# congliuUvA/Clifford-Group-Equivariant-Simplicial-Message-Passing-Networks

Hardware: AMD Instinct MI355X
Metric: simplicial edges/sec (fwd+bwd) on Cl(3,0) 8-ch multivectors; % HBM roofline (higher is better)
Workload: dtype f32; 1 GPU; S1: EGCL layer fwd+bwd, Cl(1, 1, 1), 8 channels, 10000 nodes, 100000 edges/GPU x 1 GPU, aggr=mean, edge_attr 6ch, node_attr 3ch; aggregation=float atomics, launch=hip-graph replay

## Files before the change

### clifford-group-equivariant-simplicial-message-passing-networks_amd/csmpn_hip/native.py

```python
from __future__ import annotations

import ctypes as C
import os

_HERE = os.path.dirname(os.path.abspath(__file__))
LIB_PATH = os.environ.get("CSMPN_LIB") or os.path.join(_HERE, "libcsmpn_hip.so")

ABI_VERSION = 2
MAX_BLOCKS = 4
FLAG_WEIGHTS_PACKED = 1
FLAG_NO_VALIDATE = 2
FLAG_DETERMINISTIC = 4
FLAG_SAVE_STATE = 8
ERR_UNSUPPORTED, ERR_INVALID, ERR_HIP = 1, 2, 3
LAYER_MVSILU, LAYER_MVNORM, LAYER_MVLAYERNORM, LAYER_WGP = 0, 1, 2, 3

EXPORTS = (
    "csmpn_metric_supported",
    "csmpn_algebra_tables",
    "csmpn_geometric_product_forward",
    "csmpn_geometric_product_backward",
    "csmpn_cemlp_workspace_bytes",
    "csmpn_cemlp_saved_floats_per_row",
    "csmpn_cemlp_saved_floats",
    "csmpn_cemlp_forward",
    "csmpn_cemlp_backward",
    "csmpn_mvlinear_forward",
    "csmpn_mvlinear_backward",
    "csmpn_mvlinear_backward_det_bytes",
    "csmpn_mvlinear_backward_det",
    "csmpn_mvsilu_forward",
    "csmpn_mvsilu_backward",
    "csmpn_mvnorm_forward",
    "csmpn_mvnorm_backward",
    "csmpn_mvlayernorm_forward",
    "csmpn_mvlayernorm_backward",
    "csmpn_wgp_forward",
    "csmpn_wgp_backward",
    "csmpn_small_layer_det_bytes",
    "csmpn_mvsilu_backward_det",
    "csmpn_mvnorm_backward_det",
    "csmpn_mvlayernorm_forward_det",
    "csmpn_mvlayernorm_backward_det",
    "csmpn_wgp_backward_det",
    "csmpn_csr_workspace_bytes",
    "csmpn_csr_build",
    "csmpn_csr_source_order",
    "csmpn_segment_reduce",
    "csmpn_egcl_edge_forward",
    "csmpn_egcl_edge_backward",
    "csmpn_egcl_node_forward",
    "csmpn_egcl_node_backward",
    "csmpn_egcl_backward",
    "csmpn_simplex_rows",
    "csmpn_simplex_tables_workspace_bytes",
    "csmpn_simplex_tables",
    "csmpn_rips_lift_workspace_bytes",
    "csmpn_rips_lift",
    "csmpn_knn_lift_workspace_bytes",
    "csmpn_knn_lift",
    "csmpn_embed_cemlp_forward",
    "csmpn_embed_cemlp_backward",
    "csmpn_type_attr_forward",
    "csmpn_type_attr_backward",
    "csmpn_type_attr_backward_det_bytes",
    "csmpn_type_attr_backward_det",
    "csmpn_readout_mse_forward",
    "csmpn_readout_mse_backward",
    "csmpn_readout_traj_forward",
    "csmpn_readout_traj_backward",
    "csmpn_last_error",
    "csmpn_last_kernel",
    "csmpn_abi_version",
    "csmpn_build_target",
)

PARAM_FIELDS = ("lin_w", "lin_b", "silu_a", "silu_b", "gp_w", "norm_a", "right_w", "left_w", "left_b", "ln_a")


class BlockParams(C.Structure):
    _fields_ = [
        ("in_features", C.c_int32),
        ("out_features", C.c_int32),
        ("lin_subspaces", C.c_int32),
        ("reserved", C.c_int32),
    ] + [(name, C.c_void_p) for name in PARAM_FIELDS]


class BlockGrads(C.Structure):
    _fields_ = [(name, C.c_void_p) for name in PARAM_FIELDS]


class VertexBlock(C.Structure):
    _fields_ = [("data", C.c_void_p), ("channels", C.c_int32), ("grade", C.c_int32)]


class NativeLibraryMissing(RuntimeError):
    pass


def _load():
    if not os.path.exists(LIB_PATH):
        raise NativeLibraryMissing(
            f"{LIB_PATH} not found. This package has no CPU/eager fallback: build the HIP "
            f"library first (python -c 'import __graft_entry__ as g; g.build()' or "
            f"make -C {os.path.join(os.path.dirname(_HERE), 'csrc')})."
        )
    lib = C.CDLL(LIB_PATH)
    lib.csmpn_abi_version.restype = C.c_int
    if lib.csmpn_abi_version() != ABI_VERSION:
        raise NativeLibraryMissing(f"{LIB_PATH} has ABI version {lib.csmpn_abi_version()}, this package binds version "
                                   f"{ABI_VERSION}: rebuild it (make -C {os.path.join(os.path.dirname(_HERE), 'csrc')})")
    vp, i32, i64, sz, u32 = C.c_void_p, C.c_int32, C.c_int64, C.c_size_t, C.c_uint32
    fp = C.POINTER(C.c_float)
    bp, bg = C.POINTER(BlockParams), C.POINTER(BlockGrads)

    def sig(name, res, args):
        fn = getattr(lib, name)
        fn.restype = res
        fn.argtypes = args

    sig("csmpn_metric_supported", C.c_int, [fp, C.c_int])
    sig("csmpn_algebra_tables", C.c_int, [fp, C.c_int, vp, vp, vp, vp, vp, vp])
    sig("csmpn_geometric_product_forward", C.c_int, [fp, C.c_int, vp, vp, vp, i64, vp])
    sig("csmpn_geometric_product_backward", C.c_int, [fp, C.c_int, vp, vp, vp, vp, vp, i64, vp])
    sig("csmpn_cemlp_workspace_bytes", sz, [C.c_int, bp, C.c_int])
    sig("csmpn_cemlp_saved_floats_per_row", sz, [C.c_int, bp, C.c_int])
    sig("csmpn_cemlp_saved_floats", sz, [C.c_int, bp, C.c_int, i64, u32])
    sig("csmpn_cemlp_forward", C.c_int, [fp, C.c_int, bp, C.c_int, vp, i64, vp, vp, vp, sz, u32, vp])
    sig("csmpn_cemlp_backward", C.c_int, [fp, C.c_int, bp, bg, C.c_int, vp, vp, i64, vp, vp, vp, sz, u32, vp])
    sig("csmpn_mvlinear_forward", C.c_int, [C.c_int, vp, vp, vp, i64, i32, i32, i32, vp, vp])
    sig("csmpn_mvlinear_backward", C.c_int, [C.c_int, vp, vp, vp, i64, i32, i32, i32, vp, vp, vp, vp])
    sig("csmpn_mvlinear_backward_det_bytes", sz, [C.c_int, i64, i32, i32, i32])
    sig("csmpn_mvlinear_backward_det", C.c_int, [C.c_int, vp, vp, vp, i64, i32, i32, i32, vp, vp, vp, vp, sz, vp])
    sig("csmpn_mvsilu_forward", C.c_int, [fp, C.c_int, vp, vp, vp, i64, i32, vp, vp])
    sig("csmpn_mvsilu_backward", C.c_int, [fp, C.c_int, vp, vp, vp, vp, i64, i32, vp, vp, vp, vp])
    sig("csmpn_mvnorm_forward", C.c_int, [fp, C.c_int, vp, vp, i64, i32, vp, vp])
    sig("csmpn_mvnorm_backward", C.c_int, [fp, C.c_int, vp, vp, vp, i64, i32, vp, vp, vp])
    sig("csmpn_mvlayernorm_forward", C.c_int, [fp, C.c_int, vp, vp, i64, i32, vp, vp])
    sig("csmpn_mvlayernorm_backward", C.c_int, [fp, C.c_int, vp, vp, vp, i64, i32, vp, vp, vp])
    sig("csmpn_wgp_forward", C.c_int, [fp, C.c_int, vp, vp, vp, i64, i32, vp, vp])
    sig("csmpn_wgp_backward", C.c_int, [fp, C.c_int, vp, vp, vp, vp, i64, i32, vp, vp, vp, vp])
    sig("csmpn_small_layer_det_bytes", sz, [C.c_int, C.c_int, i64, i32])
    sig("csmpn_mvsilu_backward_det", C.c_int, [fp, C.c_int, vp, vp, vp, vp, i64, i32, vp, vp, vp, vp, sz, vp])
    sig("csmpn_mvnorm_backward_det", C.c_int, [fp, C.c_int, vp, vp, vp, i64, i32, vp, vp, vp, sz, vp])
    sig("csmpn_mvlayernorm_forward_det", C.c_int, [fp, C.c_int, vp, vp, i64, i32, vp, vp])
    sig("csmpn_mvlayernorm_backward_det", C.c_int, [fp, C.c_int, vp, vp, vp, i64, i32, vp, vp, vp, sz, vp])
    sig("csmpn_wgp_backward_det", C.c_int, [fp, C.c_int, vp, vp, vp, vp, i64, i32, vp, vp, vp, vp, sz, vp])
    sig("csmpn_csr_workspace_bytes", sz, [i64, i64])
    sig("csmpn_csr_build", C.c_int, [vp, i64, i64, vp, vp, vp, vp, vp, vp, sz, u32, vp])
    sig("csmpn_csr_source_order", C.c_int, [vp, i64, i64, vp, vp, vp, sz, vp])
    sig("csmpn_segment_reduce", C.c_int, [vp, i64, i64, vp, vp, vp, vp, vp, i32, vp])
    sig("csmpn_egcl_edge_forward", C.c_int,
        [fp, C.c_int, bp, C.c_int, vp, i32, vp, i32, vp, vp, vp, i64, i64, vp, vp, vp, sz, u32, vp])
    sig("csmpn_egcl_edge_backward", C.c_int,
        [fp, C.c_int, bp, bg, C.c_int, vp, i32, vp, i32, vp, vp, vp, i64, i64, vp, vp, vp, vp, vp, sz, u32, vp])
    sig("csmpn_egcl_node_forward", C.c_int,
        [fp, C.c_int, bp, C.c_int, vp, i32, vp, i32, vp, i32, vp, i32, i32, i64, vp, vp, vp, sz, u32, vp])
    sig("csmpn_egcl_node_backward", C.c_int,
        [fp, C.c_int, bp, bg, C.c_int, vp, i32, vp, i32, vp, i32, vp, i32, i32, i64, vp, vp, vp, vp, vp, vp, sz, u32, vp])
    sig("csmpn_egcl_backward", C.c_int,
        [fp, C.c_int, bp, bg, C.c_int, bp, bg, C.c_int, vp, i32, vp, i32, vp, i32, vp, i32, vp, vp, vp, vp, i32, i32, i64, i64,
         vp, vp, vp, vp, vp, vp, vp, vp, sz, u32, vp, vp, sz, u32, vp])
    sig("csmpn_simplex_rows", C.c_int, [C.c_int, C.POINTER(VertexBlock), C.c_int, vp, i64, i32, i64, vp, vp])
    sig("csmpn_simplex_tables_workspace_bytes", sz, [i64, i32])
    sig("csmpn_simplex_tables", C.c_int, [vp, i32, vp, vp, vp, i64, i64, i32, vp, vp, vp, vp, vp, vp, vp, vp, vp, sz, vp])
    sig("csmpn_rips_lift_workspace_bytes", sz, [i64, i32, i32])
    sig("csmpn_rips_lift", C.c_int, [vp, i32, i64, i32, C.c_double, i32, vp, i64, vp, i32, vp, vp, vp, vp, vp, vp, vp, vp, vp, vp, sz, vp])
    sig("csmpn_knn_lift_workspace_bytes", sz, [i64, i32, i32])
    sig("csmpn_knn_lift", C.c_int, [vp, i32, i64, i32, i32, i32, vp, i64, vp, i32, vp, vp, vp, vp, vp, vp, vp, vp, vp, vp, sz, vp])
    sig("csmpn_embed_cemlp_forward", C.c_int, [fp, C.c_int, bp, C.c_int, vp, i64, i32, vp, i32, i32, i64, vp, vp, vp, sz, u32, vp])
    sig("csmpn_embed_cemlp_backward", C.c_int, [fp, C.c_int, bp, bg, C.c_int, vp, i64, i32, vp, i32, i32, i64, vp, vp, vp, sz, u32, vp])
    sig("csmpn_type_attr_forward", C.c_int, [C.c_int, vp, i32, i32, vp, i64, vp, vp, i64, vp, vp, vp])
    sig("csmpn_type_attr_backward", C.c_int, [C.c_int, i32, i32, vp, i64, vp, vp, i64, vp, vp, vp, vp])
    sig("csmpn_type_attr_backward_det_bytes", sz, [i32, i32, i64, i64])
    sig("csmpn_type_attr_backward_det", C.c_int, [C.c_int, i32, i32, vp, i64, vp, vp, i64, vp, vp, vp, vp, sz, vp])
    sig("csmpn_readout_mse_forward", C.c_int, [C.c_int, vp, vp, i32, vp, i64, i32, vp, i64, vp, vp, vp, vp, vp])
    sig("csmpn_readout_mse_backward", C.c_int, [C.c_int, vp, i32, i64, i32, vp, i64, vp, vp, vp])
    sig("csmpn_readout_traj_forward", C.c_int, [C.c_int, vp, i32, vp, i64, vp, i32, i32, vp, vp, vp, vp, i64, vp, vp, vp, vp])
    sig("csmpn_readout_traj_backward", C.c_int,
        [C.c_int, vp, i32, i64, vp, vp, i64, vp, i32, i32, vp, vp, vp, vp, vp, vp, vp, vp, vp, vp, vp])
    sig("csmpn_last_error", C.c_char_p, [])
    sig("csmpn_last_kernel", C.c_char_p, [])
    sig("csmpn_abi_version", C.c_int, [])
    sig("csmpn_build_target", C.c_char_p, [])
    return lib


_lib = None


def lib():
    global _lib
    if _lib is None:
        _lib = _load()
    return _lib


class CsmpnError(RuntimeError):
    pass


def check(rc: int):
    if rc != 0:
        raise CsmpnError(f"csmpn_hip error {rc}: {lib().csmpn_last_error().decode()}")


def metric_array(metric):
    arr = (C.c_float * len(metric))(*[float(m) for m in metric])
    return arr
```

### clifford-group-equivariant-simplicial-message-passing-networks_amd/csmpn_hip/ops.py

```python
from __future__ import annotations

import ctypes as C
import os
import warnings
from typing import List, Optional, Sequence

import torch

from . import native
from .native import BlockGrads, BlockParams, PARAM_FIELDS, check

NP = len(PARAM_FIELDS)


def _stream(device) -> int:
    return torch.cuda.current_stream(device).cuda_stream


def _on_device_of(arg_index):
    import functools

    def deco(fn):
        @functools.wraps(fn)
        def wrapped(*args, **kwargs):
# ... 292 lines not shown
def _det_call(call, flags):
    det = deterministic_request()
    rc = call(flags | (native.FLAG_DETERMINISTIC if det else 0))
    if det == "soft" and _soft_fallback(rc):
        rc = call(flags)
    check(rc)


_DET_LAUNCHES = 0


def det_launches() -> int:
    return _DET_LAUNCHES


def _count_det():
    global _DET_LAUNCHES
    _DET_LAUNCHES += 1


def _det_scratch(nbytes, device):
    _count_det()
    return torch.empty(max(int(nbytes), 16), dtype=torch.uint8, device=device)


def _small_det_scratch(op, metric, x):
    return _det_scratch(native.lib().csmpn_small_layer_det_bytes(op, len(metric), x.shape[0], x.shape[1]), x.device)


def _warn_soft_slice():
    global _warned_soft_det
    if not _warned_soft_det:
        _warned_soft_det = True
        warnings.warn("csmpn_hip: torch.use_deterministic_algorithms(True) is set, but this launch covers a slice of "
                      "the adjacency (graph-segment step): using float atomics (ops.set_deterministic(True) makes "
                      "this an error)")


def segment_reduce(rows, out, add=None, sub=None, accumulate=True):
    ap, ao = add if add is not None else (None, None)
    sp, so = sub if sub is not None else (None, None)
    check(native.lib().csmpn_segment_reduce(rows.data_ptr(), rows[0].numel(), out.shape[0], _ptr(ap), _ptr(ao),
                                            _ptr(sp), _ptr(so), out.data_ptr(), 1 if accumulate else 0,
                                            _stream(out.device)))
    return out


class Csr:

    __slots__ = ("perm", "src", "dst", "deg", "row_ptr", "n_edges", "n_nodes", "build_ms", "_src_order", "_ws")

    def source_order(self):
        if self._src_order is None:
            dev = self.src.device
            order = torch.empty(max(self.n_edges, 1), dtype=torch.int32, device=dev)
            rp = torch.empty(self.n_nodes + 1, dtype=torch.int32, device=dev)
            ws = torch.empty(int(native.lib().csmpn_csr_workspace_bytes(self.n_edges, self.n_nodes)),
                             dtype=torch.uint8, device=dev)
            with torch.cuda.device(dev):
                check(native.lib().csmpn_csr_source_order(self.src.data_ptr(), self.n_edges, self.n_nodes,
                                                          order.data_ptr(), rp.data_ptr(), ws.data_ptr(), ws.numel(),
                                                          _stream(dev)))
            self._src_order = (rp, order)
        return self._src_order

    def __init__(self, edge_index: torch.Tensor, n_nodes: int):
        if not edge_index.is_cuda:
            raise RuntimeError("edge_index must live on the GPU (no CPU fallback)")
        if edge_index.dtype != torch.int64 or edge_index.dim() != 2 or edge_index.shape[0] != 2:
            raise RuntimeError("edge_index must be int64 [2, E]")
        ei = edge_index.contiguous()
        dev = ei.device
        E = ei.shape[1]
        i32 = dict(dtype=torch.int32, device=dev)
        self.n_edges, self.n_nodes = E, n_nodes
        self._src_order = None
        self._ws = None
        self.perm = torch.empty(max(E, 1), **i32)
        self.src = torch.empty(max(E, 1), **i32)
        self.dst = torch.empty(max(E, 1), **i32)
        self.deg = torch.empty(n_nodes, **i32)
        self.row_ptr = torch.empty(n_nodes + 1, **i32)
        ws = torch.empty(int(native.lib().csmpn_csr_workspace_bytes(E, n_nodes)), dtype=torch.uint8, device=dev)
        with torch.cuda.device(dev):
            t0, t1 = torch.cuda.Event(enable_timing=True), torch.cuda.Event(enable_timing=True)
            t0.record()
            check(native.lib().csmpn_csr_build(ei.data_ptr(), E, n_nodes, self.perm.data_ptr(), self.src.data_ptr(),
                                               self.dst.data_ptr(), self.deg.data_ptr(), self.row_ptr.data_ptr(),
                                               ws.data_ptr(), ws.numel(), 0, _stream(dev)))
            t1.record()
            t1.synchronize()
            self.build_ms = t0.elapsed_time(t1)


    def rebuild_(self, edge_index: torch.Tensor) -> "Csr":
        if not edge_index.is_cuda or edge_index.device != self.src.device:
            raise RuntimeError("edge_index must live on the device of the CSR (no CPU fallback)")
        if edge_index.dtype != torch.int64 or tuple(edge_index.shape) != (2, self.n_edges) or not edge_index.is_contiguous():
            raise RuntimeError(f"Csr.rebuild_: edge_index must be contiguous int64 [2, {self.n_edges}] (the size it was built for)")
        dev = self.src.device
        lib = native.lib()
        if self._ws is None:
            self._ws = torch.empty(int(lib.csmpn_csr_workspace_bytes(self.n_edges, self.n_nodes)), dtype=torch.uint8, device=dev)
        ws = self._ws
        with torch.cuda.device(dev):
            check(lib.csmpn_csr_build(edge_index.data_ptr(), self.n_edges, self.n_nodes, self.perm.data_ptr(),
                                      self.src.data_ptr(), self.dst.data_ptr(), self.deg.data_ptr(), self.row_ptr.data_ptr(),
                                      ws.data_ptr(), ws.numel(), native.FLAG_NO_VALIDATE, _stream(dev)))
            if self._src_order is not None:
                rp, order = self._src_order
                check(lib.csmpn_csr_source_order(self.src.data_ptr(), self.n_edges, self.n_nodes, order.data_ptr(),
                                                 rp.data_ptr(), ws.data_ptr(), ws.numel(), _stream(dev)))
        try:
            edge_index._csmpn_csr = (edge_index._version, self)
        except Exception:
            pass
        return self


class CsrSlice:

    __slots__ = ("perm", "src", "dst", "n_edges", "n_nodes")

    def __init__(self, csr: Csr, lo: int, hi: int):
        self.perm, self.src, self.dst = csr.perm[lo:hi], csr.src[lo:hi], csr.dst[lo:hi]
        self.n_edges, self.n_nodes = hi - lo, csr.n_nodes


def get_csr(edge_index: torch.Tensor, n_nodes: int) -> Csr:
    cached = getattr(edge_index, "_csmpn_csr", None)
    if cached is not None and cached[0] == edge_index._version and cached[1].n_nodes == n_nodes:
        return cached[1]
    csr = Csr(edge_index, n_nodes)
    try:
        edge_index._csmpn_csr = (edge_index._version, csr)
    except Exception:
        pass
    return csr




class EgclSpec:

    def __init__(self, edge: CemlpBinding, node: CemlpBinding, channels: int, out_channels: int,
                 edge_attr_channels: int, node_attr_channels: int, aggr: str, residual: bool):
        if aggr not in ("mean", "sum", "add"):
            raise native.CsmpnError(f"aggr={aggr!r} not supported by the HIP path (mean | sum | add)")
        self.edge, self.node = edge, node
        self.C, self.O = channels, out_channels
        self.A, self.T = edge_attr_channels, node_attr_channels
        self.mean = 1 if aggr == "mean" else 0
        self.residual = 1 if residual else 0


class HipBackend:

    @staticmethod
    def build_csr(edge_index, n_nodes):
        return get_csr(edge_index, n_nodes)

    @staticmethod
    @_on_device_of(2)
    def edge_forward(spec, csr, h, edge_attr, pe, save=True, agg=None, saved=None):
        e = spec.edge
        e.bind(pe)
        N, D = h.shape[0], e.D
        if agg is None:
            agg = torch.zeros(N, spec.O, D, dtype=torch.float32, device=h.device)
        ws = e.workspace(h.device)
        st_flag = 0
        if saved is None and save:
            saved = e.new_saved(csr.n_edges, h.device, _SAVE_STATE)
            if _SAVE_STATE and saved is not None:
                st_flag = native.FLAG_SAVE_STATE
                saved.csmpn_save_state = True
        det = deterministic_request()
        if det and not isinstance(csr, Csr):
            if det == "hard":
                raise native.CsmpnError("deterministic aggregation needs the whole adjacency (no sliced launches: "
                                        "set CSMPN_SPLIT_FWD=0)")
            _warn_soft_slice()
            det = None
        if det:
            rows = torch.empty(max(csr.n_edges, 1), spec.O, D, dtype=torch.float32, device=h.device)
            rc = native.lib().csmpn_egcl_edge_forward(
                e.metric_arr, e.n, e.params, e.nblk, h.data_ptr(), spec.C, _ptr(edge_attr), spec.A,
                csr.perm.data_ptr(), csr.src.data_ptr(), csr.dst.data_ptr(), csr.n_edges, N, rows.data_ptr(),
                _ptr(saved), ws.data_ptr(), ws.numel(), native.FLAG_DETERMINISTIC | st_flag, _stream(h.device))
            if not (det == "soft" and _soft_fallback(rc)):
                check(rc)
                segment_reduce(rows, agg, add=(csr.row_ptr, None))
                return agg, (ws, saved)
        check(native.lib().csmpn_egcl_edge_forward(
            e.metric_arr, e.n, e.params, e.nblk, h.data_ptr(), spec.C, _ptr(edge_attr), spec.A,
            csr.perm.data_ptr(), csr.src.data_ptr(), csr.dst.data_ptr(), csr.n_edges, N, agg.data_ptr(),
            _ptr(saved), ws.data_ptr(), ws.numel(), st_flag, _stream(h.device)))
        return agg, (ws, saved)

    @staticmethod
    @_on_device_of(2)
    def node_forward(spec, deg, h, agg, node_attr, pn, save=True):
        nd = spec.node
        nd.bind(pn)
        N, D = h.shape[0], nd.D
        out = torch.empty(N, nd.out_features, D, dtype=torch.float32, device=h.device)
        ws = nd.workspace(h.device)
        saved = nd.new_saved(N, h.device, _SAVE_STATE) if save else None
        st_flag = 0
        if _SAVE_STATE and saved is not None:
            st_flag = native.FLAG_SAVE_STATE
            saved.csmpn_save_state = True

        def call(flags):
            return native.lib().csmpn_egcl_node_forward(
                nd.metric_arr, nd.n, nd.params, nd.nblk, h.data_ptr(), spec.C, agg.data_ptr(), spec.O,
                _ptr(node_attr), spec.T, deg.data_ptr(), spec.mean, spec.residual, N, out.data_ptr(),
                _ptr(saved), ws.data_ptr(), ws.numel(), flags, _stream(h.device))

        det = deterministic_request()
        rc = call((native.FLAG_DETERMINISTIC if det else 0) | st_flag)
        if det == "soft" and _soft_fallback(rc):
            rc = call(st_flag)
        check(rc)
        return out, (ws, saved)

    @staticmethod
    @_on_device_of(2)
    def node_backward(spec, deg, h, agg, node_attr, pn, gout, want_gna, state=None, gflat=None, fused_into=None):
        nd = spec.node
        nd.bind(pn)
        N, D, dev = h.shape[0], nd.D, h.device
        _flat, views = nd.new_grads(pn, dev, gflat, fused_into=fused_into)
        gh = torch.empty_like(h)
        g_agg = torch.empty(N, spec.O, D, dtype=torch.float32, device=dev)
        g_na = torch.empty_like(node_attr) if (node_attr is not None and want_gna) else None
        ws, saved = state if state is not None else (nd.workspace(dev), None)
        flags = native.FLAG_WEIGHTS_PACKED if state is not None else 0
        if getattr(saved, "csmpn_save_state", False):
            flags |= native.FLAG_SAVE_STATE

        def call(fl):
            return native.lib().csmpn_egcl_node_backward(
                nd.metric_arr, nd.n, nd.params, nd.grads, nd.nblk, h.data_ptr(), spec.C, agg.data_ptr(), spec.O,
                _ptr(node_attr), spec.T, deg.data_ptr(), spec.mean, spec.residual, N, gout.data_ptr(),
                gh.data_ptr(), g_agg.data_ptr(), _ptr(g_na), _ptr(saved), ws.data_ptr(), ws.numel(), fl, _stream(dev))

        det = deterministic_request()
        rc = call(flags | (native.FLAG_DETERMINISTIC if det else 0))
        if det == "soft" and _soft_fallback(rc):
            rc = call(flags)
        check(rc)
        return gh, g_agg, g_na, views

    @staticmethod
    @_on_device_of(2)
    def edge_backward(spec, csr, h, edge_attr, pe, g_agg, gh, want_gea, state=None, gflat=None, fused_into=None):
        e = spec.edge
        e.bind(pe)
        N, dev = h.shape[0], h.device
        _flat, views = e.new_grads(pe, dev, gflat, fused_into=fused_into)
        g_ea = torch.empty_like(edge_attr) if (edge_attr is not None and want_gea) else None
        ws, saved = state if state is not None else (e.workspace(dev), None)
        flags = native.FLAG_WEIGHTS_PACKED if state is not None else 0
        if getattr(saved, "csmpn_save_state", False):
            flags |= native.FLAG_SAVE_STATE
        det = deterministic_request()
        if det and not isinstance(csr, Csr):
            if det == "hard":
                raise native.CsmpnError("deterministic aggregation needs the whole adjacency (no sliced launches)")
            _warn_soft_slice()
            det = None
        if det:
            rows = torch.empty(max(csr.n_edges, 1), spec.C, e.D, dtype=torch.float32, device=dev)
            rc = native.lib().csmpn_egcl_edge_backward(
                e.metric_arr, e.n, e.params, e.grads, e.nblk, h.data_ptr(), spec.C, _ptr(edge_attr), spec.A,
                csr.perm.data_ptr(), csr.src.data_ptr(), csr.dst.data_ptr(), csr.n_edges, N, g_agg.data_ptr(),
                rows.data_ptr(), _ptr(g_ea), _ptr(saved), ws.data_ptr(), ws.numel(),
                flags | native.FLAG_DETERMINISTIC, _stream(dev))
            if not (det == "soft" and _soft_fallback(rc)):
                check(rc)
                segment_reduce(rows, gh, add=(csr.row_ptr, None), sub=csr.source_order())
                return g_ea, views
        check(native.lib().csmpn_egcl_edge_backward(
            e.metric_arr, e.n, e.params, e.grads, e.nblk, h.data_ptr(), spec.C, _ptr(edge_attr), spec.A,
            csr.perm.data_ptr(), csr.src.data_ptr(), csr.dst.data_ptr(), csr.n_edges, N, g_agg.data_ptr(),
            gh.data_ptr(), _ptr(g_ea), _ptr(saved), ws.data_ptr(), ws.numel(), flags, _stream(dev)))
        return g_ea, views

    @staticmethod
    @_on_device_of(2)
    def layer_backward(spec, csr, h, agg, edge_attr, node_attr, pe, pn, gout, want_gea, want_gna, state_e=None, state_n=None,
                       gflat_e=None, gflat_n=None, fused_e=None, fused_n=None):
        e, nd = spec.edge, spec.node
        e.bind(pe)
        nd.bind(pn)
        N, D, dev = h.shape[0], nd.D, h.device
        _fe, views_e = e.new_grads(pe, dev, gflat_e, fused_into=fused_e)
        _fn, views_n = nd.new_grads(pn, dev, gflat_n, fused_into=fused_n)
        gh = torch.empty_like(h)
        g_agg = torch.empty(N, spec.O, D, dtype=torch.float32, device=dev)
        g_na = torch.empty_like(node_attr) if (node_attr is not None and want_gna) else None
        g_ea = torch.empty_like(edge_attr) if (edge_attr is not None and want_gea) else None

        def stage(binding, state):
            ws, saved = state if state is not None else (binding.workspace(dev), None)
            flags = native.FLAG_WEIGHTS_PACKED if state is not None else 0
            if getattr(saved, "csmpn_save_state", False):
                flags |= native.FLAG_SAVE_STATE
            return ws, saved, flags

        ws_e, saved_e, fl_e = stage(e, state_e)
        ws_n, saved_n, fl_n = stage(nd, state_n)
        check(native.lib().csmpn_egcl_backward(
            e.metric_arr, e.n, e.params, e.grads, e.nblk, nd.params, nd.grads, nd.nblk, h.data_ptr(), spec.C,
            agg.data_ptr(), spec.O, _ptr(edge_attr), spec.A, _ptr(node_attr), spec.T, csr.perm.data_ptr(),
            csr.src.data_ptr(), csr.dst.data_ptr(), csr.deg.data_ptr(), spec.mean, spec.residual, csr.n_edges, N,
            gout.data_ptr(), gh.data_ptr(), g_agg.data_ptr(), _ptr(g_ea), _ptr(g_na), None, _ptr(saved_e),
            ws_e.data_ptr(), ws_e.numel(), fl_e, _ptr(saved_n), ws_n.data_ptr(), ws_n.numel(), fl_n, _stream(dev)))
        return gh, g_ea, g_na, views_e, views_n


_SAVE_STATE = os.environ.get("CSMPN_SAVE_STATE", "1") not in ("0", "")


def _check_egcl_inputs(spec, csr, h, edge_attr, node_attr, n_edges):
    D = spec.edge.D
    if h.dim() != 3 or h.shape[1] != spec.C or h.shape[2] != D:
        raise RuntimeError(f"h must be [N, {spec.C}, {D}], got {tuple(h.shape)}")
    if (edge_attr is None) != (spec.A == 0) or (node_attr is None) != (spec.T == 0):
        raise RuntimeError("edge_attr/node_attr presence does not match edge_attr_features/node_attr_features")
    if edge_attr is not None and tuple(edge_attr.shape) != (n_edges, spec.A, D):
        raise RuntimeError(f"edge_attr must be [{n_edges}, {spec.A}, {D}], got {tuple(edge_attr.shape)}")
    if node_attr is not None and tuple(node_attr.shape) != (h.shape[0], spec.T, D):
        raise RuntimeError(f"node_attr must be [{h.shape[0]}, {spec.T}, {D}], got {tuple(node_attr.shape)}")


class _EgclFn(torch.autograd.Function):
    @staticmethod
    def forward(ctx, h, edge_attr, node_attr, spec: EgclSpec, csr: Csr, *params):
        _require_device(h, "EGCL input h")
        _check_egcl_inputs(spec, csr, h, edge_attr, node_attr, csr.n_edges)
        h = h.contiguous()
        if edge_attr is not None:
            _require_device(edge_attr, "edge_attr")
            edge_attr = edge_attr.contiguous()
        if node_attr is not None:
            _require_device(node_attr, "node_attr")
            node_attr = node_attr.contiguous()
        ne = spec.edge.nblk * NP
        pe, pn = params[:ne], params[ne:]
        spec.edge.bind(pe); spec.node.bind(pn)
        n_agg = h.shape[0] * spec.O * spec.edge.D
        ctx.param_refs = params
        fuse = _fusable(params, h.device)
        n_ge, n_gn = (spec.edge.grad_floats(pe), spec.node.grad_floats(pn)) if (any(ctx.needs_input_grad) and not fuse) else (0, 0)
        zeros = torch.zeros(n_agg + n_ge + n_gn, dtype=torch.float32, device=h.device)
        agg = zeros[:n_agg].view(h.shape[0], spec.O, spec.edge.D)
        ctx.gflats = (zeros[n_agg:n_agg + n_ge], zeros[n_agg + n_ge:]) if n_ge else None
        agg, st_e = HipBackend.edge_forward(spec, csr, h, edge_attr, pe, agg=agg)
        out, st_n = HipBackend.node_forward(spec, csr.deg, h, agg, node_attr, pn)
        ctx.spec, ctx.csr, ctx.st_e, ctx.st_n = spec, csr, st_e, st_n
        ctx.has_ea, ctx.has_na = edge_attr is not None, node_attr is not None
        ctx.mask = [p is not None for p in params]
        saved = [h, agg]
        if ctx.has_ea:
            saved.append(edge_attr)
        if ctx.has_na:
            saved.append(node_attr)
        ctx.save_for_backward(*saved, *[p for p in params if p is not None])
        return out

    @staticmethod
    def backward(ctx, gout):
        spec, csr = ctx.spec, ctx.csr
        saved = list(ctx.saved_tensors)
        h, agg = saved[0], saved[1]
        pos = 2
        edge_attr = node_attr = None
        if ctx.has_ea:
            edge_attr = saved[pos]; pos += 1
        if ctx.has_na:
            node_attr = saved[pos]; pos += 1
        it = iter(saved[pos:])
        params = [next(it) if m else None for m in ctx.mask]
        ne = spec.edge.nblk * NP
        pe, pn = params[:ne], params[ne:]
        gout = gout.contiguous()
        gfe, gfn = ctx.gflats if ctx.gflats is not None else (None, None)
        ctx.gflats = None
        refs = ctx.param_refs
        fuse = _fusable(refs, h.device)
        if isinstance(csr, Csr) and not deterministic_request():
            gh, g_ea, g_na, views_e, views_n = HipBackend.layer_backward(
                spec, csr, h, agg, edge_attr, node_attr, pe, pn, gout, ctx.needs_input_grad[1], ctx.needs_input_grad[2],
                ctx.st_e, ctx.st_n, gfe, gfn, refs[:ne] if fuse else None, refs[ne:] if fuse else None)
            return (gh, g_ea, g_na, None, None, *views_e, *views_n)
        gh, g_agg, g_na, views_n = HipBackend.node_backward(spec, csr.deg, h, agg, node_attr, pn, gout,
                                                            ctx.needs_input_grad[2], ctx.st_n, gfn,
                                                            fused_into=refs[ne:] if fuse else None)
        g_ea, views_e = HipBackend.edge_backward(spec, csr, h, edge_attr, pe, g_agg, gh, ctx.needs_input_grad[1],
                                                 ctx.st_e, gfe, fused_into=refs[:ne] if fuse else None)
        return (gh, g_ea, g_na, None, None, *views_e, *views_n)


def egcl_apply(h, edge_attr, node_attr, spec: EgclSpec, csr: Csr, params):
    return _EgclFn.apply(h, edge_attr, node_attr, spec, csr, *params)




class _GpFn(torch.autograd.Function):
    @staticmethod
    @_on_device_of(1)
    def forward(ctx, a, b, metric):
        _require_device(a, "geometric_product operand")
        _require_device(b, "geometric_product operand")
        shape = torch.broadcast_shapes(a.shape, b.shape)
        a2 = a.expand(shape).contiguous()
        b2 = b.expand(shape).contiguous()
        n = len(metric)
        D = 1 << n
        rows = a2.numel() // D
        out = torch.empty_like(a2)
        check(native.lib().csmpn_geometric_product_forward(native.metric_array(metric), n, a2.data_ptr(),
                                                           b2.data_ptr(), out.data_ptr(), rows, _stream(a.device)))
        ctx.save_for_backward(a2, b2)
        ctx.metric, ctx.shapes = metric, (a.shape, b.shape)
        return out

    @staticmethod
    @_on_device_of(1)
    def backward(ctx, gout):
        a2, b2 = ctx.saved_tensors
        metric = ctx.metric
        n = len(metric)
        D = 1 << n
        gout = gout.contiguous()
        ga, gb = torch.zeros_like(a2), torch.zeros_like(b2)
        check(native.lib().csmpn_geometric_product_backward(native.metric_array(metric), n, a2.data_ptr(),
                                                            b2.data_ptr(), gout.data_ptr(), ga.data_ptr(),
                                                            gb.data_ptr(), a2.numel() // D, _stream(a2.device)))
        sa, sb = ctx.shapes
        return ga.sum_to_size(sa), gb.sum_to_size(sb), None




class _MVLinearFn(torch.autograd.Function):

    @staticmethod
    @_on_device_of(1)
    def forward(ctx, x, weight, bias, n):
        _require_device(x, "MVLinear input")
        for name, t in (("weight", weight), ("bias", bias)):
            if t is not None and (t.device != x.device or t.dtype != torch.float32):
                raise RuntimeError(f"MVLinear {name} must be float32 on {x.device}, got {t.dtype} on {t.device}")
        x = x.contiguous()
        w = weight.contiguous()
        b = bias.contiguous() if bias is not None else None
        rows, I, D = x.shape
        O = w.shape[0]
        if D != (1 << n) or w.shape[1] != I:
            raise RuntimeError(f"MVLinear: input {tuple(x.shape)} does not match weight {tuple(w.shape)} (n={n})")
        y = torch.empty(rows, O, D, dtype=torch.float32, device=x.device)
        check(native.lib().csmpn_mvlinear_forward(n, x.data_ptr(), w.data_ptr(), _ptr(b), rows, I, O,
                                                  1 if w.dim() == 3 else 0, y.data_ptr(), _stream(x.device)))
        ctx.save_for_backward(x, w)
        ctx.n, ctx.has_bias = n, bias is not None
        ctx.param_refs = (weight if weight.is_contiguous() else None, bias if (bias is None or bias.is_contiguous()) else False)
        return y

    @staticmethod
    @_on_device_of(1)
    def backward(ctx, gy):
        x, w = ctx.saved_tensors
        gy = gy.contiguous()
        rows, I, D = x.shape
        O = w.shape[0]
        gx = torch.empty_like(x) if ctx.needs_input_grad[0] else None
        need_w, need_b = ctx.needs_input_grad[1], ctx.has_bias and ctx.needs_input_grad[2]
        pw, pb = ctx.param_refs
        sub = 1 if w.dim() == 3 else 0

        def run(gw_ptr, gb_ptr):
            if deterministic_request() and (gw_ptr is not None or gb_ptr is not None):
                ws = _det_scratch(native.lib().csmpn_mvlinear_backward_det_bytes(ctx.n, rows, I, O, sub), x.device)
                check(native.lib().csmpn_mvlinear_backward_det(ctx.n, x.data_ptr(), w.data_ptr(), gy.data_ptr(), rows, I, O, sub,
                                                               _ptr(gx), gw_ptr, gb_ptr, ws.data_ptr(), ws.numel(),
                                                               _stream(x.device)))
            else:
                check(native.lib().csmpn_mvlinear_backward(ctx.n, x.data_ptr(), w.data_ptr(), gy.data_ptr(), rows, I, O, sub,
                                                           _ptr(gx), gw_ptr, gb_ptr, _stream(x.device)))

        if (pw is not None and pb is not False and (need_w or need_b)
                and _fusable([pw if need_w else None, pb if need_b else None], x.device)
                and (not need_b or pb.grad.numel() == O)):
            run(pw.grad.data_ptr() if need_w else None, pb.grad.data_ptr() if need_b else None)
            return gx, None, None, None
        gw = torch.zeros_like(w) if need_w else None
        gb = torch.zeros(1, O, 1, dtype=torch.float32, device=x.device) if need_b else None
        run(_ptr(gw), _ptr(gb))
        return gx, gw, gb, None



_SMALL_LAUNCHES = 0


def small_layer_launches() -> int:
    return _SMALL_LAUNCHES


def _small_args(x, what, params):
    _require_device(x, f"{what} input")
    if x.dim() != 3:
        raise RuntimeError(f"{what}: the HIP path takes [rows, channels, D] inputs, got {tuple(x.shape)}")
    for t in params:
        if t.device != x.device or t.dtype != torch.float32:
            raise RuntimeError(f"{what} parameters must be float32 on {x.device}, got {t.dtype} on {t.device}")
    return x.contiguous()


def _count():
    global _SMALL_LAUNCHES
    _SMALL_LAUNCHES += 1


class _MVSiLUFn(torch.autograd.Function):

    @staticmethod
    @_on_device_of(1)
    def forward(ctx, x, a, b, metric):
        x = _small_args(x, "MVSiLU", (a, b))
        a2, b2 = a.contiguous(), b.contiguous()
        y = torch.empty_like(x)
        check(native.lib().csmpn_mvsilu_forward(native.metric_array(metric), len(metric), x.data_ptr(), a2.data_ptr(),
                                                b2.data_ptr(), x.shape[0], x.shape[1], y.data_ptr(), _stream(x.device)))
        _count()
        ctx.save_for_backward(x, a2, b2)
        ctx.metric = metric
        return y

    @staticmethod
    @_on_device_of(1)
    def backward(ctx, gy):
        x, a, b = ctx.saved_tensors
        gy = gy.contiguous()
        gx, ga, gb = torch.empty_like(x), torch.zeros_like(a), torch.zeros_like(b)
# ... 472 lines not shown
```

### clifford-group-equivariant-simplicial-message-passing-networks_amd/csrc/capi.hip

```cpp
#include <mutex>
#include <hip/hip_runtime.h>

#include <cstdarg>
#include <cstdio>
#include <cstdlib>
#include <cstring>
#include <vector>

#include "plan.hpp"

using namespace csmpn;

thread_local char g_csmpn_err[512] = "";

int csmpn_fail(int code, const char* fmt, ...) {
    va_list ap;
    va_start(ap, fmt);
    vsnprintf(g_csmpn_err, sizeof(g_csmpn_err), fmt, ap);
    va_end(ap);
    return code;
}


namespace csmpn {
// ... 102 lines not shown

size_t csmpn_cemlp_saved_floats(int n, const csmpn_block_params* blocks, int n_blocks, int64_t rows, uint32_t flags) {
    if (rows <= 0 || !blocks || n_blocks < 1 || n_blocks > CSMPN_MAX_BLOCKS || n < 1 || n > 8) return 0;
    return saved_layout(n, blocks, n_blocks, rows, flags).total;
}

size_t csmpn_cemlp_saved_floats_per_row(int n, const csmpn_block_params* blocks, int n_blocks) {
    if (!blocks || n_blocks < 1 || n_blocks > CSMPN_MAX_BLOCKS || n < 1 || n > 8) return 0;
    return saved_layout(n, blocks, n_blocks, -1, CSMPN_FLAG_SAVE_STATE).total;
}

size_t csmpn_cemlp_workspace_bytes(int n, const csmpn_block_params* blocks, int n_blocks) {
    if (!blocks || n_blocks < 1 || n_blocks > CSMPN_MAX_BLOCKS || n < 1 || n > 8) return 0;
    const size_t tail = family_tail_bytes(n, blocks, n_blocks), det = det_slice_bytes(n, blocks, n_blocks);
    return plan_front_bytes(n, blocks, n_blocks) + (tail > det ? tail : det) + kTailSlack;
}

int csmpn_cemlp_forward(const float* metric, int n, const csmpn_block_params* blocks, int n_blocks, const float* x,
                        int64_t rows, float* y, float* save_inputs, void* workspace, size_t workspace_bytes, uint32_t flags, void* stream) {
    const AlgId id = alg_id(metric, n);
    if (id == ALG_NONE) return fail(CSMPN_ERR_UNSUPPORTED, "metric not supported by the HIP path");
    Plan plan;
    int rc = make_plan(id, blocks, nullptr, n_blocks, workspace, workspace_bytes, false, 0, false, rows, plan,
                       (flags & CSMPN_FLAG_DETERMINISTIC) != 0);
    if (rc) return rc;
    const bool need_pack = !(flags & CSMPN_FLAG_WEIGHTS_PACKED);
    RowIO io;
    memset(&io, 0, sizeof(io));
    io.rows = rows; io.nseg = 1;
    io.seg[0].a = x; io.seg[0].ch = blocks[0].in_features; io.seg[0].off = 0;
    io.y = y; io.save = save_inputs;
    io.save_state = ((flags & CSMPN_FLAG_SAVE_STATE) && pq_plain_shape(n, blocks, n_blocks)) ? 1 : 0;
    return run_rows(plan, MODE_PLAIN, false, io, (hipStream_t)stream, need_pack);
}

int csmpn_cemlp_backward(const float* metric, int n, const csmpn_block_params* blocks, const csmpn_block_grads* grads,
                         int n_blocks, const float* x, const float* gy, int64_t rows, float* gx, const float* saved_inputs, void* workspace,
                         size_t workspace_bytes, uint32_t flags, void* stream) {
    const AlgId id = alg_id(metric, n);
    if (id == ALG_NONE) return fail(CSMPN_ERR_UNSUPPORTED, "metric not supported by the HIP path");
    Plan plan;
    int rc = make_plan(id, blocks, grads, n_blocks, workspace, workspace_bytes, true, 0, saved_inputs != nullptr, rows, plan,
                       (flags & CSMPN_FLAG_DETERMINISTIC) != 0);
    if (rc) return rc;
    const bool need_pack = true;
    RowIO io;
    memset(&io, 0, sizeof(io));
    io.rows = rows; io.nseg = 1;
    io.seg[0].a = x; io.seg[0].ch = blocks[0].in_features; io.seg[0].off = 0;
    io.gy = gy; io.gx[0] = gx; io.saved = saved_inputs;
    io.row_store = (flags & CSMPN_FLAG_DETERMINISTIC) ? 1 : 0;
    io.save_state = ((flags & CSMPN_FLAG_SAVE_STATE) && pq_plain_shape(n, blocks, n_blocks)) ? 1 : 0;
    const bool tables_ready = io.save_state && (flags & CSMPN_FLAG_WEIGHTS_PACKED) != 0;
    return run_rows(plan, MODE_PLAIN, true, io, (hipStream_t)stream, need_pack, tables_ready);
}

__global__ void index_range_kernel(const int* __restrict__ idx, long n, int hi, int* __restrict__ flag) {
    const long i = (long)blockIdx.x * blockDim.x + threadIdx.x;
    if (i < n && (idx[i] < 0 || idx[i] >= hi)) atomicOr(flag, 1);
}
__device__ int g_range_flag;
static std::mutex g_range_mutex;

static int check_index_range(const int32_t* idx, int64_t n, int64_t hi, hipStream_t st, const char* what) {
    if (n <= 0) return CSMPN_OK;
    std::lock_guard<std::mutex> lock(g_range_mutex);
    int* flag = nullptr;
    hipError_t e = hipGetSymbolAddress(reinterpret_cast<void**>(&flag), HIP_SYMBOL(g_range_flag));
    if (e == hipSuccess) e = hipMemsetAsync(flag, 0, sizeof(int), st);
    if (e != hipSuccess) return fail(CSMPN_ERR_HIP, "%s validation: %s", what, hipGetErrorString(e));
    hipLaunchKernelGGL(index_range_kernel, dim3((unsigned)((n + 255) / 256)), dim3(256), 0, st, idx, (long)n,
                       (int)(hi > 0x7fffffff ? 0x7fffffff : hi), flag);
    int host_flag = 0;
    e = hipMemcpyAsync(&host_flag, flag, sizeof(int), hipMemcpyDeviceToHost, st);
    if (e == hipSuccess) e = hipStreamSynchronize(st);
    if (e != hipSuccess) return fail(CSMPN_ERR_HIP, "%s validation: %s", what, hipGetErrorString(e));
    if (host_flag) return fail(CSMPN_ERR_INVALID, "%s has entries outside [0, %lld)", what, (long long)hi);
    return CSMPN_OK;
}

static int embed_io(const AlgId id, const csmpn_block_params* blocks, const float* vertex_feat, int64_t n_vertex_rows, int32_t kpv,
                    const int32_t* verts, int32_t nv, int32_t n_orders, int64_t n_rows, uint32_t flags, hipStream_t st, RowIO& io) {
    if (id != ALG_N5 && id != ALG_N5M) return fail(CSMPN_ERR_UNSUPPORTED, "fused embedding: Cl(5,0) / Cl(4,1) only");
    if (n_orders != 1 && n_orders != 2 && n_orders != 6) return fail(CSMPN_ERR_UNSUPPORTED, "fused embedding: 1, 2 or 6 vertex orders");
    if (!vertex_feat || !verts || kpv < 1 || nv < 1 || nv * kpv != blocks[0].in_features || nv * kpv > 8)
        return fail(CSMPN_ERR_UNSUPPORTED, "fused embedding: verts_per_row * channels_per_vertex must equal in_features (<= 8)");
    if (n_rows % n_orders) return fail(CSMPN_ERR_INVALID, "fused embedding: n_rows %ld is not a multiple of n_orders %d", (long)n_rows, n_orders);
    if (n_vertex_rows < 1 || n_vertex_rows > 0x7fffffff)
        return fail(CSMPN_ERR_INVALID, "fused embedding: n_vertex_rows %lld not in [1, 2^31)", (long long)n_vertex_rows);
    if (!(flags & CSMPN_FLAG_NO_VALIDATE)) {
        const int rc = check_index_range(verts, n_rows * nv, n_vertex_rows, st, "fused embedding: verts");
        if (rc) return rc;
    }
    memset(&io, 0, sizeof(io));
    io.rows = n_rows; io.nseg = 1;
    io.seg[0].a = vertex_feat; io.seg[0].ch = blocks[0].in_features; io.seg[0].off = 0;
    io.emb_verts = verts; io.emb_nperm = n_orders; io.emb_nv = nv; io.emb_k = kpv; io.emb_nrows = (int)n_vertex_rows;
    return CSMPN_OK;
}

int csmpn_embed_cemlp_forward(const float* metric, int n, const csmpn_block_params* blocks, int n_blocks, const float* vertex_feat,
                              int64_t n_vertex_rows, int32_t channels_per_vertex, const int32_t* verts, int32_t verts_per_row, int32_t n_orders,
                              int64_t n_rows, float* out, float* save_inputs, void* workspace, size_t workspace_bytes,
                              uint32_t flags, void* stream) {
    const AlgId id = alg_id(metric, n);
    if (id == ALG_NONE) return fail(CSMPN_ERR_UNSUPPORTED, "metric not supported by the HIP path");
    RowIO io;
    int rc = embed_io(id, blocks, vertex_feat, n_vertex_rows, channels_per_vertex, verts, verts_per_row, n_orders, n_rows, flags,
                      (hipStream_t)stream, io);
    if (rc) return rc;
    Plan plan;
    if ((rc = make_plan(id, blocks, nullptr, n_blocks, workspace, workspace_bytes, false, 0, false, n_rows, plan))) return rc;
    io.y = out; io.save = save_inputs;
    if (!plw_serves(plan, MODE_PLAIN, false, io))
        return fail(CSMPN_ERR_UNSUPPORTED, "fused embedding: shape not served by the wide parity-lane kernels");
    io.save_state = (flags & CSMPN_FLAG_SAVE_STATE) ? 1 : 0;
    return run_rows(plan, MODE_PLAIN, false, io, (hipStream_t)stream, false);
}

int csmpn_embed_cemlp_backward(const float* metric, int n, const csmpn_block_params* blocks, const csmpn_block_grads* grads,
                               int n_blocks, const float* vertex_feat, int64_t n_vertex_rows, int32_t channels_per_vertex,
                               const int32_t* verts, int32_t verts_per_row, int32_t n_orders, int64_t n_rows, const float* g_out,
                               const float* saved_inputs, void* workspace, size_t workspace_bytes, uint32_t flags, void* stream) {
    const AlgId id = alg_id(metric, n);
    if (id == ALG_NONE) return fail(CSMPN_ERR_UNSUPPORTED, "metric not supported by the HIP path");
    RowIO io;
    int rc = embed_io(id, blocks, vertex_feat, n_vertex_rows, channels_per_vertex, verts, verts_per_row, n_orders, n_rows, flags,
                      (hipStream_t)stream, io);
    if (rc) return rc;
    Plan plan;
    if ((rc = make_plan(id, blocks, grads, n_blocks, workspace, workspace_bytes, true, 0, saved_inputs != nullptr, n_rows, plan))) return rc;
    io.gy = g_out; io.saved = saved_inputs;
    if (!plw_serves(plan, MODE_PLAIN, true, io))
        return fail(CSMPN_ERR_UNSUPPORTED, "fused embedding: shape not served by the wide parity-lane kernels (two blocks need saved inputs)");
    io.save_state = (flags & CSMPN_FLAG_SAVE_STATE) ? 1 : 0;
    return run_rows(plan, MODE_PLAIN, true, io, (hipStream_t)stream, false);
}

static int edge_io(const csmpn_block_params* blocks, const float* h, int channels, const float* edge_attr, int attr_channels,
                   const int32_t* perm, const int32_t* src_sorted, const int32_t* dst_sorted, int64_t E, uint32_t flags, RowIO& io) {
    if (attr_channels > 0 && !edge_attr && E > 0) return fail(CSMPN_ERR_INVALID, "edge_attr is null");
    if (channels + attr_channels != blocks[0].in_features)
        return fail(CSMPN_ERR_INVALID, "edge model in_features %d != %d + %d", blocks[0].in_features, channels, attr_channels);
    memset(&io, 0, sizeof(io));
    io.rows = E; io.nseg = attr_channels > 0 ? 2 : 1;
    io.seg[0].a = h; io.seg[0].ia = dst_sorted; io.seg[0].b = h; io.seg[0].ib = src_sorted; io.seg[0].ch = channels;
    io.seg[1].a = edge_attr; io.seg[1].ia = perm; io.seg[1].ch = attr_channels; io.seg[1].off = channels;
    io.dst = dst_sorted; io.src = src_sorted; io.perm = perm;
    io.row_store = (flags & CSMPN_FLAG_DETERMINISTIC) ? 1 : 0;
    io.save_state = (flags & CSMPN_FLAG_SAVE_STATE) ? 1 : 0;
    return CSMPN_OK;
}

int csmpn_egcl_edge_forward(const float* metric, int n, const csmpn_block_params* blocks, int n_blocks, const float* h,
                            int32_t channels, const float* edge_attr, int32_t attr_channels, const int32_t* perm,
                            const int32_t* src_sorted, const int32_t* dst_sorted, int64_t E, int64_t N, float* agg,
                            float* save_inputs, void* workspace, size_t workspace_bytes, uint32_t flags, void* stream) {
    const AlgId id = alg_id(metric, n);
    if (id == ALG_NONE) return fail(CSMPN_ERR_UNSUPPORTED, "metric not supported by the HIP path");
    RowIO io;
    int rc = edge_io(blocks, h, channels, edge_attr, attr_channels, perm, src_sorted, dst_sorted, E, flags, io);
    if (rc) return rc;
    Plan plan;
    if ((rc = make_plan(id, blocks, nullptr, n_blocks, workspace, workspace_bytes, false, blocks[n_blocks - 1].out_features << n, false,
                        E, plan, (flags & CSMPN_FLAG_DETERMINISTIC) != 0))) return rc;
    const bool need_pack = !(flags & CSMPN_FLAG_WEIGHTS_PACKED);
    io.agg = agg; io.save = save_inputs;
    io.gather_rows = N;
    return run_rows(plan, MODE_EDGE, false, io, (hipStream_t)stream, need_pack);
}

static int edge_backward(const float* metric, int n, const csmpn_block_params* blocks,
                         const csmpn_block_grads* grads, int n_blocks, const float* h, int32_t channels,
                         const float* edge_attr, int32_t attr_channels, const int32_t* perm,
                         const int32_t* src_sorted, const int32_t* dst_sorted, int64_t E, int64_t N,
                         const float* g_agg, float* gh, float* g_edge_attr, const float* saved_inputs, void* workspace,
                         size_t workspace_bytes, uint32_t flags, void* stream, SliceSet* deferred) {
    const AlgId id = alg_id(metric, n);
    if (id == ALG_NONE) return fail(CSMPN_ERR_UNSUPPORTED, "metric not supported by the HIP path");
    RowIO io;
    int rc = edge_io(blocks, h, channels, edge_attr, attr_channels, perm, src_sorted, dst_sorted, E, flags, io);
    if (rc) return rc;
    Plan plan;
    if ((rc = make_plan(id, blocks, grads, n_blocks, workspace, workspace_bytes, true, 0, saved_inputs != nullptr, E, plan,
                        (flags & CSMPN_FLAG_DETERMINISTIC) != 0))) return rc;
    const bool need_pack = true;
    io.gy = g_agg; io.gx[0] = gh; io.gx[1] = g_edge_attr; io.saved = saved_inputs;
    io.gather_rows = N;
    return run_rows(plan, MODE_EDGE, true, io, (hipStream_t)stream, need_pack, (flags & CSMPN_FLAG_WEIGHTS_PACKED) != 0, deferred);
}

int csmpn_egcl_edge_backward(const float* metric, int n, const csmpn_block_params* blocks,
                             const csmpn_block_grads* grads, int n_blocks, const float* h, int32_t channels,
                             const float* edge_attr, int32_t attr_channels, const int32_t* perm,
                             const int32_t* src_sorted, const int32_t* dst_sorted, int64_t E, int64_t N,
                             const float* g_agg, float* gh, float* g_edge_attr, const float* saved_inputs, void* workspace,
                             size_t workspace_bytes, uint32_t flags, void* stream) {
    return edge_backward(metric, n, blocks, grads, n_blocks, h, channels, edge_attr, attr_channels, perm, src_sorted, dst_sorted, E, N,
                         g_agg, gh, g_edge_attr, saved_inputs, workspace, workspace_bytes, flags, stream, nullptr);
}

static int node_io(const csmpn_block_params* blocks, int n_blocks, const float* h, int channels, const float* agg,
                   int agg_channels, const float* node_attr, int attr_channels, const int32_t* in_degree,
                   int mean_aggr, int residual, int64_t N, RowIO& io) {
    if (attr_channels > 0 && !node_attr) return fail(CSMPN_ERR_INVALID, "node_attr is null");
    if (channels + agg_channels + attr_channels != blocks[0].in_features)
        return fail(CSMPN_ERR_INVALID, "node model in_features %d != %d + %d + %d", blocks[0].in_features, channels,
                    agg_channels, attr_channels);
    if (residual && blocks[n_blocks - 1].out_features != channels)
        return fail(CSMPN_ERR_INVALID, "residual needs out_features == channels");
    if (mean_aggr && !in_degree) return fail(CSMPN_ERR_INVALID, "in_degree is null");
    memset(&io, 0, sizeof(io));
    io.rows = N; io.nseg = attr_channels > 0 ? 3 : 2;
    io.seg[0].a = h; io.seg[0].ch = channels; io.seg[0].off = 0;
    io.seg[1].a = agg; io.seg[1].ch = agg_channels; io.seg[1].off = channels;
    io.seg[1].deg = mean_aggr ? in_degree : nullptr;
    io.seg[2].a = node_attr; io.seg[2].ch = attr_channels; io.seg[2].off = channels + agg_channels;
    return CSMPN_OK;
}

int csmpn_egcl_node_forward(const float* metric, int n, const csmpn_block_params* blocks, int n_blocks, const float* h,
                            int32_t channels, const float* agg, int32_t agg_channels, const float* node_attr,
                            int32_t attr_channels, const int32_t* in_degree, int32_t mean_aggr, int32_t residual,
                            int64_t N, float* out, float* save_inputs, void* workspace, size_t workspace_bytes, uint32_t flags, void* stream) {
    const AlgId id = alg_id(metric, n);
    if (id == ALG_NONE) return fail(CSMPN_ERR_UNSUPPORTED, "metric not supported by the HIP path");
    RowIO io;
    int rc = node_io(blocks, n_blocks, h, channels, agg, agg_channels, node_attr, attr_channels, in_degree, mean_aggr,
                     residual, N, io);
    if (rc) return rc;
    Plan plan;
    if ((rc = make_plan(id, blocks, nullptr, n_blocks, workspace, workspace_bytes, false, 0, false, N, plan,
                        (flags & CSMPN_FLAG_DETERMINISTIC) != 0))) return rc;
    const bool need_pack = !(flags & CSMPN_FLAG_WEIGHTS_PACKED);
    io.y = out; io.resid = residual ? h : nullptr; io.save = save_inputs;
    io.row_store = (flags & CSMPN_FLAG_DETERMINISTIC) ? 1 : 0;
    io.save_state = (flags & CSMPN_FLAG_SAVE_STATE) ? 1 : 0;
    return run_rows(plan, MODE_NODE, false, io, (hipStream_t)stream, need_pack);
}

static int node_backward(const float* metric, int n, const csmpn_block_params* blocks,
                         const csmpn_block_grads* grads, int n_blocks, const float* h, int32_t channels,
                         const float* agg, int32_t agg_channels, const float* node_attr, int32_t attr_channels,
                         const int32_t* in_degree, int32_t mean_aggr, int32_t residual, int64_t N,
                         const float* g_out, float* gh, float* g_agg, float* g_node_attr, const float* saved_inputs, void* workspace,
                         size_t workspace_bytes, uint32_t flags, void* stream, SliceSet* deferred) {
    const AlgId id = alg_id(metric, n);
    if (id == ALG_NONE) return fail(CSMPN_ERR_UNSUPPORTED, "metric not supported by the HIP path");
    RowIO io;
    int rc = node_io(blocks, n_blocks, h, channels, agg, agg_channels, node_attr, attr_channels, in_degree, mean_aggr,
                     residual, N, io);
    if (rc) return rc;
    Plan plan;
    if ((rc = make_plan(id, blocks, grads, n_blocks, workspace, workspace_bytes, true, 0, saved_inputs != nullptr, N, plan,
                        (flags & CSMPN_FLAG_DETERMINISTIC) != 0))) return rc;
    const bool need_pack = true;
    io.gy = g_out; io.gx[0] = gh; io.gx[1] = g_agg; io.gx[2] = g_node_attr;
    io.resid_bwd = residual ? 1 : 0; io.saved = saved_inputs;
    io.row_store = (flags & CSMPN_FLAG_DETERMINISTIC) ? 1 : 0;
    io.save_state = (flags & CSMPN_FLAG_SAVE_STATE) ? 1 : 0;
    return run_rows(plan, MODE_NODE, true, io, (hipStream_t)stream, need_pack, (flags & CSMPN_FLAG_WEIGHTS_PACKED) != 0, deferred);
}

int csmpn_egcl_node_backward(const float* metric, int n, const csmpn_block_params* blocks,
                             const csmpn_block_grads* grads, int n_blocks, const float* h, int32_t channels,
                             const float* agg, int32_t agg_channels, const float* node_attr, int32_t attr_channels,
                             const int32_t* in_degree, int32_t mean_aggr, int32_t residual, int64_t N,
                             const float* g_out, float* gh, float* g_agg, float* g_node_attr, const float* saved_inputs, void* workspace,
                             size_t workspace_bytes, uint32_t flags, void* stream) {
    return node_backward(metric, n, blocks, grads, n_blocks, h, channels, agg, agg_channels, node_attr, attr_channels, in_degree, mean_aggr,
                         residual, N, g_out, gh, g_agg, g_node_attr, saved_inputs, workspace, workspace_bytes, flags, stream, nullptr);
}

int csmpn_egcl_backward(const float* metric, int n, const csmpn_block_params* edge_blocks, const csmpn_block_grads* edge_grads,
                        int n_edge_blocks, const csmpn_block_params* node_blocks, const csmpn_block_grads* node_grads,
                        int n_node_blocks, const float* h, int32_t channels, const float* agg, int32_t agg_channels,
                        const float* edge_attr, int32_t edge_attr_channels, const float* node_attr, int32_t node_attr_channels,
                        const int32_t* perm, const int32_t* src_sorted, const int32_t* dst_sorted, const int32_t* in_degree,
                        int32_t mean_aggr, int32_t residual, int64_t E, int64_t N, const float* g_out, float* gh, float* g_agg,
                        float* g_edge_attr, float* g_node_attr, float* g_edge_rows, const float* edge_saved, void* edge_workspace,
                        size_t edge_workspace_bytes, uint32_t edge_flags, const float* node_saved, void* node_workspace,
                        size_t node_workspace_bytes, uint32_t node_flags, void* stream) {
    const bool det = ((edge_flags | node_flags) & CSMPN_FLAG_DETERMINISTIC) != 0;
    if ((edge_flags & CSMPN_FLAG_DETERMINISTIC) && !g_edge_rows)
        return fail(CSMPN_ERR_INVALID, "CSMPN_FLAG_DETERMINISTIC: g_edge_rows ([E, C, D], csmpn_egcl_edge_backward's gh) is null");
    const char *we = static_cast<const char*>(edge_workspace), *wn = static_cast<const char*>(node_workspace);
    const bool apart = we && wn && (we + edge_workspace_bytes <= wn || wn + node_workspace_bytes <= we);
    SliceSet node_set, edge_set;
    node_set.unit = edge_set.unit = nullptr;
    const bool defer = !det && apart;
    int rc = node_backward(metric, n, node_blocks, node_grads, n_node_blocks, h, channels, agg, agg_channels, node_attr,
                           node_attr_channels, in_degree, mean_aggr, residual, N, g_out, gh, g_agg, g_node_attr, node_saved,
                           node_workspace, node_workspace_bytes, node_flags, stream, defer ? &node_set : nullptr);
    if (rc) return rc;
    rc = edge_backward(metric, n, edge_blocks, edge_grads, n_edge_blocks, h, channels, edge_attr, edge_attr_channels, perm, src_sorted,
                       dst_sorted, E, N, g_agg, (edge_flags & CSMPN_FLAG_DETERMINISTIC) ? g_edge_rows : gh, g_edge_attr, edge_saved,
                       edge_workspace, edge_workspace_bytes, edge_flags, stream, node_set.unit ? &edge_set : nullptr);
    if (node_set.unit) {
        const SliceSet* const other = (!rc && edge_set.unit == node_set.unit) ? &edge_set : nullptr;
        HIP_TRY(node_set.unit->sum_slices(node_set, other, (hipStream_t)stream));
        if (!rc && edge_set.unit && !other) HIP_TRY(edge_set.unit->sum_slices(edge_set, nullptr, (hipStream_t)stream));
    }
    return rc;
}

}
```

### clifford-group-equivariant-simplicial-message-passing-networks_amd/csrc/cemlp_cl.hpp

```cpp
#pragma once
#include "cemlp_lane.hpp"

namespace csmpn {

constexpr int kClWaves = 4;
constexpr int kClSliceCap = 512;
constexpr int kClParStride = 36;

#define CL_LDS_ORDER() do { asm volatile("" ::: "memory"); __builtin_amdgcn_wave_barrier(); asm volatile("" ::: "memory"); } while (0)

typedef unsigned cl_u4 __attribute__((ext_vector_type(4)));
constexpr unsigned kClNoStore = 0xFF000000u;
constexpr int kClStream = 2;
struct ClBuf {
    __amdgpu_buffer_rsrc_t r;
    CSMPN_DEV ClBuf() : r(__builtin_amdgcn_make_buffer_rsrc(nullptr, 0, 0, 0x00020000)) {}
    CSMPN_DEV ClBuf(const void* base, size_t bytes)
        : r(__builtin_amdgcn_make_buffer_rsrc(const_cast<void*>(base), 0, base ? (int)(unsigned)bytes : 0, 0x00020000)) {}
    template <int AUX = 0>
    CSMPN_DEV f4 ld4(unsigned off) const { return __builtin_bit_cast(f4, __builtin_amdgcn_raw_buffer_load_b128(r, (int)off, 0, AUX)); }
    CSMPN_DEV int ldi(unsigned off) const { return (int)__builtin_amdgcn_raw_buffer_load_b32(r, (int)off, 0, 0); }
    template <int AUX = 0>
    CSMPN_DEV void st4(unsigned off, f4 v) const { __builtin_amdgcn_raw_buffer_store_b128(__builtin_bit_cast(cl_u4, v), r, (int)off, 0, AUX); }
    CSMPN_DEV void st8(unsigned off, const float (&x)[8]) const {
// ... 69 lines not shown
            "v_fmac_f32_dpp %2, %10, %17 row_ror:%20 row_mask:0xf bank_mask:0xf\n\t"
            "v_fmac_f32_dpp %3, %11, %17 row_ror:%20 row_mask:0xf bank_mask:0xf\n\t"
            "v_fmac_f32_dpp %4, %12, %18 row_ror:%20 row_mask:0xf bank_mask:0xf\n\t"
            "v_fmac_f32_dpp %5, %13, %18 row_ror:%20 row_mask:0xf bank_mask:0xf\n\t"
            "v_fmac_f32_dpp %6, %14, %18 row_ror:%20 row_mask:0xf bank_mask:0xf\n\t"
            "v_fmac_f32_dpp %7, %15, %19 row_ror:%20 row_mask:0xf bank_mask:0xf"
            : "+v"(acc[0]), "+v"(acc[1]), "+v"(acc[2]), "+v"(acc[3]), "+v"(acc[4]), "+v"(acc[5]), "+v"(acc[6]), "+v"(acc[7])
            : "v"(x[0]), "v"(x[1]), "v"(x[2]), "v"(x[3]), "v"(x[4]), "v"(x[5]), "v"(x[6]), "v"(x[7]),
              "v"(w.x), "v"(w.y), "v"(w.z), "v"(w.w), "n"(ROT));
    }
}

template <int NK>
CSMPN_DEV void cl_pin(f4 (&w)[NK]) {
    if constexpr (NK == 8) asm volatile("" : "+v"(w[0]), "+v"(w[1]), "+v"(w[2]), "+v"(w[3]), "+v"(w[4]), "+v"(w[5]), "+v"(w[6]), "+v"(w[7]));
    else if constexpr (NK == 4) asm volatile("" : "+v"(w[0]), "+v"(w[1]), "+v"(w[2]), "+v"(w[3]));
    else if constexpr (NK == 2) asm volatile("" : "+v"(w[0]), "+v"(w[1]));
    else static_assert(NK == 1 || NK == 2 || NK == 4 || NK == 8, "batch size");
}
template <int C, int NROT, int TOFF, int BATCH = 4>
CSMPN_DEV void cl_mix(float (&acc)[8], const float (&x)[8], const float* ldsw) {
    static_assert(NROT % BATCH == 0, "whole batches");
    constexpr int NB = NROT / BATCH;
    f4 w[BATCH];
#pragma unroll
    for (int i = 0; i < BATCH; ++i) w[i] = ld4(ldsw + (TOFF + 4 * C * i));
    cl_pin<BATCH>(w);
    static_for<0, NB>([&](auto b) {
        f4 wn[BATCH];
        if constexpr (b + 1 < NB) {
#pragma unroll
            for (int i = 0; i < BATCH; ++i) wn[i] = ld4(ldsw + (TOFF + 4 * C * (BATCH * (b + 1) + i)));
        }
        static_for<0, BATCH>([&](auto i) { cl_fmac8<ClMap<C>::ROTL * (BATCH * b + i)>(acc, x, w[i]); });
        if constexpr (b + 1 < NB) {
            cl_pin<BATCH>(wn);
#pragma unroll
            for (int i = 0; i < BATCH; ++i) w[i] = wn[i];
        }
    });
}

constexpr int cl_pow2_ge(int w) { int p = 1; while (p < w) p <<= 1; return p; }

template <int C, int MODE, int NA, int K, bool BWD>
struct ClTab {
    static constexpr int NSEG = MODE == MODE_EDGE ? 1 : (MODE == MODE_NODE ? 2 : 0);
    static_assert(MODE == MODE_EDGE || MODE == MODE_NODE, "edge or node program");
    static constexpr int NP = K > 0 ? 1 : NSEG + (NA > 0 ? 1 : 0);
    static constexpr int width(int p) { return (K > 0 || p < NSEG) ? C : NA; }
    static constexpr int period(int p) { return (K > 0 || p < NSEG) ? C : cl_pow2_ge(NA); }
    static constexpr int coff(int p) { return C * p; }
    static constexpr int I = K > 0 ? C : NSEG * C + NA;
    static_assert(NA <= C, "attribute segment wider than the layer");
    static constexpr int W1(int p) { int o = 0; for (int q = 0; q < p; ++q) o += 4 * C * period(q); return o; }
    static constexpr int WR = W1(NP), WL = WR + 4 * C * C;
    static constexpr int fwd_end = WL + 4 * C * C;
    static constexpr int W1T(int p) { return fwd_end + 4 * C * C * p; }
    static constexpr int WRT = W1T(NP), WLT = WRT + 4 * C * C;
    static constexpr int par = BWD ? WLT + 4 * C * C : fwd_end;
    static constexpr int total = par + C * kClParStride;
    static constexpr int n_entries = par / 4;
};

constexpr unsigned kClStateTile = 2048, kClStatePiece = 1024;
template <int C>
CSMPN_DEV unsigned cl_state_lane(int r, int c) { return 16u * (unsigned)(r * C + c); }
struct ClFwd {
    float y[8], gate[4], R[8], invden[4], s[8];
    float qs, nl, invMn;
};

CSMPN_DEV float cl_smooth_abs_sqrt(float q) { return sqrt_pos(sqrt_pos(__builtin_fmaf(q, q, kSmooth))); }

template <class ALG, int C, class TB, bool BWD>
struct ClStage {
    static constexpr int G = ALG::G, P = ALG::P, NP = TB::NP;
    static_assert(G == 4, "the weight of one (o, c) pair is one 16-byte vector of 4 grades");
    static_assert(16 + P <= kClParStride && P % 4 == 0, "parameter stride; path weights as 16-byte vectors");
    static_assert(C * C == 64, "a piece is one wave's worth of entries");
    static_assert(kClWaves >= 3, "three waves share the per-channel parameters");
    static_assert(C * P / 4 <= 64, "one wave deals out the path weights, a 16-byte vector per lane");
    static_assert(16 + P == kClParStride, "a channel's parameter row has no padding behind the path weights: every float of it is staged");
    static constexpr int NQ = BWD ? 2 * NP + 4 : NP + 2, NSLOT = (NQ + kClWaves - 1) / kClWaves;
    struct Piece {
        const float* base;
        unsigned bytes;
        int e0, n;
        int stride, coff;
        int pm, width;
        bool transposed;
    };
    template <int Q>
    static CSMPN_DEV Piece piece(const DevBlock& B) {
        static_assert(Q >= 0 && Q < NQ, "piece index");
        constexpr bool T = Q >= NP + 2;
        constexpr int q = T ? Q - (NP + 2) : Q;
        if constexpr (q < NP) {
            return Piece{B.W1, (unsigned)(C * TB::I * G * 4), (T ? TB::W1T(q) : TB::W1(q)) / 4, T ? C * C : TB::period(q) * C, TB::I * G * 4,
                         TB::coff(q) * G * 4, TB::period(q) - 1, TB::width(q), T};
        } else {
            constexpr int e0 = (q == NP ? (T ? TB::WRT : TB::WR) : (T ? TB::WLT : TB::WL)) / 4;
            return Piece{q == NP ? B.WR : B.WL, (unsigned)(C * C * G * 4), e0, C * C, C * G * 4, 0, C - 1, C, T};
        }
    }
    f4 v[NSLOT], pw, psa, psb, pan;
    float pb1, pbL, pla;
    int dst[NSLOT];
    __device__ void load(const DevBlock& B, int wave, int lane, int dir) {
        const int o = lane % C, k = lane / C, t = o + dir * k, t7 = t & (C - 1);
        static_for<0, NSLOT>([&](auto s) {
            Piece d{B.W1, 0u, 0, 0, 0, 0, 0, 0, false};
            static_for<0, kClWaves>([&](auto j) {
                constexpr int Q = kClWaves * decltype(s)::value + decltype(j)::value;
                if constexpr (Q < NQ) {
                    if (wave == j) d = piece<Q>(B);
                }
            });
            const int row = d.transposed ? t7 : o, col = (d.transposed ? o : t) & d.pm;
            const bool in_piece = lane < d.n;
            const unsigned off = in_piece && col < d.width ? (unsigned)(row * d.stride + d.coff + col * (G * 4)) : kClNoStore;
            v[s] = ClBuf(d.base, d.bytes).ld4(off);
            dst[s] = in_piece ? d.e0 + lane : -1;
        });
        constexpr int NW = C * P / 4;
        const unsigned ow = wave == 0 && lane < NW ? 16u * lane : kClNoStore;
        const unsigned ov = wave == 1 && lane < C ? 16u * lane : kClNoStore;
        const unsigned os = wave == 2 && lane < C ? 4u * lane : kClNoStore;
        pw = ClBuf(B.w, C * P * 4).ld4(ow);
        psa = ClBuf(B.sa, C * G * 4).ld4(ov);
        psb = ClBuf(B.sb, C * G * 4).ld4(ov);
        pan = ClBuf(B.an, C * G * 4).ld4(ov);
        pb1 = __builtin_bit_cast(float, ClBuf(B.has_b1 ? B.b1 : nullptr, C * 4).ldi(os));
        pbL = __builtin_bit_cast(float, ClBuf(B.bL, C * 4).ldi(os));
        pla = __builtin_bit_cast(float, ClBuf(B.la, C * 4).ldi(os));
    }
    __device__ void store(float* base, int wave, int lane) {
#pragma unroll
        for (int s = 0; s < NSLOT; ++s) {
            if (dst[s] >= 0) st4(base + 4 * dst[s], v[s]);
        }
        float* par = base + TB::par;
        constexpr int NW = C * P / 4;
        if (wave == 0 && lane < NW) st4(par + (lane / (P / 4)) * kClParStride + 16 + 4 * (lane % (P / 4)), pw);
        if (wave == 1 && lane < C) {
            float* p = par + lane * kClParStride;
            st4(p + 4, psa);
            st4(p + 8, psb);
            st4(p + 12, f4{sigmoidf(pan.x), sigmoidf(pan.y), sigmoidf(pan.z), sigmoidf(pan.w)});
        }
        if (wave == 2 && lane < C) st4(par + lane * kClParStride, f4{pb1, pbL, pla, 0.f});
    }
};

template <class ALG>
CSMPN_DEV void cl_weighted_gp(float (&out)[8], const float (&z)[8], const float (&r)[8], const float* wp) {
    constexpr int P = ALG::P;
    f4 wv[(P + 3) / 4];
#pragma unroll
    for (int q = 0; q < (P + 3) / 4; ++q) wv[q] = ld4(wp + 4 * q);
    static_for<0, P>([&](auto p) {
        constexpr int gi = ALG::t.path_g[p][0], gj = ALG::t.path_g[p][1], gk = ALG::t.path_g[p][2];
        constexpr int i0 = ALG::gstart(gi), ni = ALG::gsize(gi);
        constexpr int j0 = ALG::gstart(gj), nj = ALG::gsize(gj);
        constexpr int k0 = ALG::gstart(gk), nk = ALG::gsize(gk);
        const float w = wv[p / 4][p % 4];
        float tmp[nj];
#pragma unroll
        for (int t = 0; t < nj; ++t) tmp[t] = 0.f;
        static_for<0, ni>([&](auto ii) {
            static_for<0, nk>([&](auto kk) {
                constexpr int i = i0 + ii, k = k0 + kk;
                constexpr int j = ALG::t.out[i][k];
                if constexpr (j >= j0 && j < j0 + nj) {
                    constexpr float sg = float(ALG::t.sign[i][k]);
                    tmp[j - j0] += (sg * z[i]) * r[k];
                }
            });
        });
#pragma unroll
        for (int t = 0; t < nj; ++t) out[j0 + t] = __builtin_fmaf(w, tmp[t], out[j0 + t]);
    });
}

template <class ALG, int C, class TB, int BATCH>
CSMPN_DEV void cl_block_tail(const float* ldsw, const float* ldsp, ClFwd& S, float (&out)[8], ClStamp& stamp, int sid, bool have_s = false) {
    constexpr int D = ALG::D, G = ALG::G;
    static_assert(D == 8 && G == 4, "Cl(3,0)-shaped algebra");
    const f4 p0 = ld4(ldsp + TB::par);
    const f4 sa = ld4(ldsp + (TB::par + 4)), sb = ld4(ldsp + (TB::par + 8));
    S.y[0] += p0.x;
    float z[D];
    static_for<0, G>([&](auto g) {
        constexpr int d0 = ALG::gstart(g), nd = ALG::gsize(g);
        float u;
        if constexpr (g == 0) {
            u = S.y[0];
        } else {
            u = 0.f;
            static_for<0, nd>([&](auto t) {
                constexpr int d = d0 + decltype(t)::value;
                u += qsf<ALG, d> * S.y[d] * S.y[d];
            });
        }
        S.gate[g] = sigmoidf(__builtin_fmaf(sa[int(g)], u, sb[int(g)]));
#pragma unroll
        for (int t = 0; t < nd; ++t) z[d0 + t] = S.gate[g] * S.y[d0 + t];
    });
    stamp(sid);
    float L[D];
#pragma unroll
    for (int d = 0; d < D; ++d) { S.R[d] = 0.f; L[d] = 0.f; }
    cl_mix<C, C, TB::WR, BATCH>(S.R, z, ldsw);
    if (have_s) {
        const f4 sg = ld4(ldsp + (TB::par + 12));
        static_for<0, G>([&](auto g) {
            constexpr int d0 = ALG::gstart(g), nd = ALG::gsize(g);
            float qq = 0.f;
            static_for<0, nd>([&](auto t) {
                constexpr int d = d0 + decltype(t)::value;
                qq += qsf<ALG, d> * S.R[d] * S.R[d];
            });
            const float m = __builtin_fmaf(sg[int(g)], cl_smooth_abs_sqrt(qq) - 1.0f, 1.0f);
            S.invden[g] = fast_rcp(m + kEps);
        });
        float qs = 0.f;
        static_for<0, D>([&](auto dd) {
            constexpr int d = decltype(dd)::value;
            qs += qsf<ALG, d> * S.s[d] * S.s[d];
        });
        S.qs = qs;
        S.nl = cl_smooth_abs_sqrt(qs);
        S.invMn = fast_rcp(__builtin_fmaf(cl_chan_sum<C>(S.nl), 1.0f / float(C), kEps));
        return;
    }
    cl_mix<C, C, TB::WL, BATCH>(L, z, ldsw);
    stamp(sid + 1);
    L[0] += p0.y;
    const f4 sg = ld4(ldsp + (TB::par + 12));
    float r[D];
    static_for<0, G>([&](auto g) {
        constexpr int d0 = ALG::gstart(g), nd = ALG::gsize(g);
        float qq = 0.f;
        static_for<0, nd>([&](auto t) {
            constexpr int d = d0 + decltype(t)::value;
            qq += qsf<ALG, d> * S.R[d] * S.R[d];
        });
        const float m = __builtin_fmaf(sg[int(g)], cl_smooth_abs_sqrt(qq) - 1.0f, 1.0f);
        S.invden[g] = fast_rcp(m + kEps);
#pragma unroll
        for (int t = 0; t < nd; ++t) r[d0 + t] = S.R[d0 + t] * S.invden[g];
    });
    stamp(sid + 2);
    cl_weighted_gp<ALG>(L, z, r, ldsp + (TB::par + 16));
    stamp(sid + 3);
#pragma unroll
    for (int d = 0; d < D; ++d) S.s[d] = L[d] * kInvSqrt2;
    float qs = 0.f;
    static_for<0, D>([&](auto dd) {
        constexpr int d = decltype(dd)::value;
        qs += qsf<ALG, d> * S.s[d] * S.s[d];
    });
    S.qs = qs;
    S.nl = cl_smooth_abs_sqrt(qs);
    S.invMn = fast_rcp(__builtin_fmaf(cl_chan_sum<C>(S.nl), 1.0f / float(C), kEps));
    const float k = p0.z * S.invMn;
#pragma unroll
    for (int d = 0; d < D; ++d) out[d] = k * S.s[d];
    stamp(sid + 4);
}


template <class ALG>
struct ClRed {
    static constexpr int G = ALG::G, P = ALG::P;
    static constexpr int i_la = 0, i_bL = 1, i_w = 2, i_an = 2 + P, i_sa = 2 + P + G, i_b1 = 2 + P + 3 * G, n = 3 + 3 * G + P;
};
template <class ALG, int C, int I>
struct ClPart {
    static constexpr int G = ALG::G, P = ALG::P;
    static constexpr int pWR = C * I * G, pWL = pWR + C * C * G, pS = pWL + C * C * G;
    static constexpr int qb1 = 0, qsa = qb1 + C, qsb = qsa + C * G, qw = qsb + C * G, qan = qw + C * P, qbL = qan + C * G, qla = qbL + C;
    static constexpr int m_small = C * (3 + 3 * G + P);
    static constexpr int total = pS + m_small;
    using RM = ClRed<ALG>;
    static constexpr int off(int idx) {
        if (idx == RM::i_la) return qla;
        if (idx == RM::i_bL) return qbL;
        if (idx < RM::i_an) return qw + (idx - RM::i_w);
        if (idx < RM::i_sa) return qan + (idx - RM::i_an);
        if (idx < RM::i_b1) return ((idx - RM::i_sa) & 1 ? qsb : qsa) + (idx - RM::i_sa) / 2;
        return qb1;
    }
    static constexpr int stride(int idx) {
        if (idx == RM::i_la || idx == RM::i_bL) return 1;
        if (idx < RM::i_an) return P;
        if (idx < RM::i_b1) return G;
        return 1;
    }
};

template <int N>
struct ClSums {
    static constexpr int kGroups = (N + 3) / 4;
    static constexpr int floats_per_wg = kGroups * 4 * 64 * kClWaves;
    float* base;
// ... 188 lines not shown
            acc += val[rr];
        });
        flush(cur, acc);
        if constexpr (SUB) {
            static_for<0, RPW>([&](auto rr) { flush(__builtin_amdgcn_readlane(t_sub, MP::lane_of_row(rr)), -val[rr]); });
        }
    });
}

template <class ALG, int C, int MODE, int NA>
struct ClIn {
    static constexpr int D = ALG::D, RB = C * D * 4, AB = NA * D * 4;
    ClBuf a, b, at;
    ClBuf i0, i1, i2;
    unsigned rows;
    unsigned lo, la;
    bool in_attr;
    const float* attr;
    CSMPN_DEV ClIn(const RowIO& io, int c) {
        rows = (unsigned)io.rows;
        lo = (unsigned)c * (D * 4);
        const int ca = c & (cl_pow2_ge(NA > 0 ? NA : 1) - 1);
        la = (unsigned)(ca < NA ? ca : NA - 1) * (D * 4);
        in_attr = c < NA;
        const size_t rb = (size_t)rows * RB, ib = (size_t)rows * 4;
        if constexpr (MODE == MODE_EDGE) {
            const size_t tb = (size_t)io.gather_rows * RB;
            a = ClBuf(io.seg[0].a, tb); b = ClBuf(io.seg[0].b, tb);
            i0 = ClBuf(io.seg[0].ia, ib); i1 = ClBuf(io.seg[0].ib, ib);
            if constexpr (NA > 0) { attr = io.seg[1].a; i2 = ClBuf(io.seg[1].ia, ib); }
        } else {
            attr = nullptr;
            a = ClBuf(io.seg[0].a, rb); b = ClBuf(io.seg[1].a, rb);
            i0 = ClBuf(io.seg[1].deg, ib);
            if constexpr (NA > 0) at = ClBuf(io.seg[2].a, (size_t)rows * AB);
        }
    }
    CSMPN_DEV unsigned row_off(unsigned row) const { return row * RB + lo; }
};

template <int C, int MODE>
struct ClTile {
    unsigned row, lrow;
    bool valid;
    int i_dst, i_src, i_perm, deg;
    CSMPN_DEV float scale() const { return 1.0f / float(deg > 1 ? deg : 1); }
    template <class ALG, int NA>
    CSMPN_DEV void load(const ClIn<ALG, C, MODE, NA>& in, unsigned tile, int r) {
        row = tile * ClMap<C>::RPW + r;
        valid = row < in.rows;
        lrow = valid ? row : 0;
        i_dst = i_src = i_perm = 0;
        deg = 1;
        if constexpr (MODE == MODE_EDGE) {
            i_dst = in.i0.ldi(4 * lrow);
            i_src = in.i1.ldi(4 * lrow);
            if constexpr (NA > 0) i_perm = in.i2.ldi(4 * lrow);
        }
        if constexpr (MODE == MODE_NODE) deg = in.i0.ldi(4 * lrow);
    }
};

template <class ALG, int C, int MODE, int NA>
struct ClRaw {
    static constexpr int NSEG = MODE == MODE_EDGE ? 2 : 2;
    using IN = ClIn<ALG, C, MODE, NA>;
    f4 v[2 * (NSEG + (NA > 0 ? 1 : 0))];
    CSMPN_DEV void issue(const IN& in, const ClTile<C, MODE>& T) {
        unsigned o0, o1, o2 = 0;
        if constexpr (MODE == MODE_EDGE) {
            o0 = (unsigned)T.i_dst * IN::RB + in.lo;
            o1 = (unsigned)T.i_src * IN::RB + in.lo;
        } else {
            o0 = o1 = in.row_off(T.lrow);
            if constexpr (NA > 0) o2 = T.lrow * IN::AB + in.la;
        }
        v[0] = in.a.ld4(o0); v[1] = in.a.ld4(o0 + 16);
        v[2] = in.b.ld4(o1); v[3] = in.b.ld4(o1 + 16);
        if constexpr (NA > 0 && MODE == MODE_EDGE) {
            const float* p2 = in.attr + ((size_t)(unsigned)T.i_perm * (IN::AB / 4) + in.la / 4);
            v[4] = ld4(p2); v[5] = ld4(p2 + 4);
        } else if constexpr (NA > 0) {
            v[4] = in.at.ld4(o2); v[5] = in.at.ld4(o2 + 16);
        }
    }
    CSMPN_DEV void pin() {
        if constexpr (NA > 0) asm volatile("" : "+v"(v[0]), "+v"(v[1]), "+v"(v[2]), "+v"(v[3]), "+v"(v[4]), "+v"(v[5]));
        else asm volatile("" : "+v"(v[0]), "+v"(v[1]), "+v"(v[2]), "+v"(v[3]));
    }
    template <class TB>
    CSMPN_DEV void finish(float (&x)[TB::NP][8], const ClTile<C, MODE>& T) const {
        auto unpack = [&](float (&t)[8], const f4& a, const f4& b) {
            t[0] = a.x; t[1] = a.y; t[2] = a.z; t[3] = a.w; t[4] = b.x; t[5] = b.y; t[6] = b.z; t[7] = b.w;
        };
        if constexpr (MODE == MODE_EDGE) {
            const f4 a = v[0] - v[2], b = v[1] - v[3];
            unpack(x[0], a, b);
            if constexpr (NA > 0) unpack(x[1], v[4], v[5]);
        } else {
            unpack(x[0], v[0], v[1]);
            const float sc_ = T.scale();
            unpack(x[1], v[2] * sc_, v[3] * sc_);
            if constexpr (NA > 0) unpack(x[2], v[4], v[5]);
        }
    }
};

template <int C>
CSMPN_DEV int cl_probe_dir(int c) {
    const int probe = cl_dpp_i<0x120 + ClMap<C>::ROTL>(c);
    return (((probe - c) & (C - 1)) == 1) ? 1 : -1;
}

template <class ALG, int C, int MODE, int NBLK, int NA>
__global__ void __launch_bounds__(64 * kClWaves, 4) cemlp_cl_fwd_kernel(const DevCemlp C_arg, const RowIO io_arg) {
    CSMPN_KERNEL_ARGS(Cd);
    using MP = ClMap<C>;
    using T0 = ClTab<C, MODE, NA, 0, false>;
    using T1 = ClTab<C, MODE, NA, 1, false>;
    constexpr int D = ALG::D, ROW = C * D, RPW = MP::RPW, SS = ROW + 4;
    static_assert(NBLK == 1 || NBLK == 2, "one or two blocks");
    constexpr int tab_floats = T0::total + (NBLK > 1 ? T1::total : 0);
    constexpr int kBatch = 4;
    extern __shared__ __attribute__((aligned(16))) float smem[];
    float* lds = smem;
    const int wave = __builtin_amdgcn_readfirstlane(threadIdx.x >> 6), lane = threadIdx.x & 63;
    const int c = MP::chan(lane), r = MP::row(lane);
    float* sc = lds + tab_floats + wave * (RPW * SS);
    ClStamp stamp(0);
    using IN = ClIn<ALG, C, MODE, NA>;
    constexpr int RB = IN::RB;
    const IN in(io, c);
    const float* ldsw0 = lds + 4 * c;
    const float* ldsp0 = lds + kClParStride * c;
    const float* ldsw1 = ldsw0 + T0::total;
    const float* ldsp1 = ldsp0 + T0::total;

    const unsigned ntiles = (in.rows + RPW - 1) / RPW;
    const unsigned tstride = gridDim.x * kClWaves;
    const bool save_s = NBLK > 1 && io.save_state != 0 && io.save != nullptr;
    const size_t row_bytes = (size_t)in.rows * RB, state_bytes = state_rows(io.rows) * (size_t)RB;
    const ClBuf b_save(io.save, row_bytes);
    const ClBuf b_s0(save_s ? io.save + state_region<ROW, ROW>(io.rows, 0, 0) : nullptr, state_bytes);
    const ClBuf b_s1(save_s ? io.save + state_region<ROW, ROW>(io.rows, 0, 1) : nullptr, state_bytes);
    const ClBuf b_out(MODE == MODE_EDGE ? (io.row_store ? io.agg : nullptr) : io.y, row_bytes);
    const ClBuf b_res(MODE == MODE_NODE ? io.resid : nullptr, row_bytes);
    const unsigned st_lane = cl_state_lane<C>(r, c);
    const unsigned tile0 = blockIdx.x * kClWaves + wave;
    ClTile<C, MODE> T, Tn;
    T.load(in, tile0, r);
    ClRaw<ALG, C, MODE, NA> raw;
    raw.issue(in, T);
    Tn.load(in, tile0 + tstride, r);
    {
        const int dir = cl_probe_dir<C>(c);
        ClStage<ALG, C, T0, false> st0;
        ClStage<ALG, C, T1, false> st1;
        st0.load(Cd.b[0], wave, lane, dir);
        if constexpr (NBLK > 1) st1.load(Cd.b[1], wave, lane, dir);
        st0.store(lds, wave, lane);
        if constexpr (NBLK > 1) st1.store(lds + T0::total, wave, lane);
    }
    __syncthreads();
    stamp(0);
    for (unsigned tile = tile0; tile < ntiles; tile += tstride) {
        raw.pin();
        stamp(1);
        f4 res0, res1;
        if constexpr (MODE == MODE_NODE) {
            if (io.resid) {
                const unsigned o = in.row_off(T.lrow);
                res0 = b_res.ld4(o); res1 = b_res.ld4(o + 16);
            }
        }
        const unsigned st_off = T.valid ? tile * kClStateTile + st_lane : kClNoStore;
        float out[D], in1[D];
        {
            float x[T0::NP][D];
            raw.template finish<T0>(x, T);
            ClFwd S;
#pragma unroll
            for (int d = 0; d < D; ++d) S.y[d] = 0.f;
            static_for<0, T0::NP>([&](auto p) { cl_mix<C, T0::period(p), T0::W1(p), kBatch>(S.y, x[p], ldsw0); });
            stamp(2);
            cl_block_tail<ALG, C, T0, kBatch>(ldsw0, ldsp0, S, out, stamp, 3);
            if (save_s) {
                b_s0.template st4<kClStream>(st_off, f4{S.s[0], S.s[1], S.s[2], S.s[3]});
                b_s0.template st4<kClStream>(st_off + kClStatePiece, f4{S.s[4], S.s[5], S.s[6], S.s[7]});
            }
        }
        if constexpr (NBLK > 1) {
#pragma unroll
            for (int d = 0; d < D; ++d) in1[d] = out[d];
            ClFwd S;
#pragma unroll
            for (int d = 0; d < D; ++d) S.y[d] = 0.f;
            cl_mix<C, C, T1::W1(0), kBatch>(S.y, in1, ldsw1);
            stamp(8);
            cl_block_tail<ALG, C, T1, kBatch>(ldsw1, ldsp1, S, out, stamp, 9);
            if (save_s) {
                b_s1.template st4<kClStream>(st_off, f4{S.s[0], S.s[1], S.s[2], S.s[3]});
                b_s1.template st4<kClStream>(st_off + kClStatePiece, f4{S.s[4], S.s[5], S.s[6], S.s[7]});
            }
        }
        const ClTile<C, MODE> Tc = T;
        T = Tn;
        raw.issue(in, T);
        Tn.load(in, tile + 2 * tstride, r);
        const unsigned o_row = in.row_off(Tc.row);
        if constexpr (NBLK > 1) {
            if (io.save) b_save.st8(o_row, in1);
        }
        if constexpr (MODE == MODE_EDGE) {
            if (io.row_store) {
                b_out.st8(o_row, out);
            } else {
                CL_LDS_ORDER();
                cl_st8(sc + r * SS + c * D, out);
                CL_LDS_ORDER();
                cl_scatter<C, ROW, false>(sc, Tc.valid ? Tc.i_dst : -1, -1, io.agg, lane);
            }
        } else {
            if (io.resid) {
                const float res[D] = {res0.x, res0.y, res0.z, res0.w, res1.x, res1.y, res1.z, res1.w};
#pragma unroll
                for (int d = 0; d < D; ++d) out[d] += res[d];
            }
            b_out.st8(o_row, out);
        }
        stamp(14);
    }
    stamp.flush(io.stamps, lane);
}
template <class ALG, int C, int MODE, int NBLK, int NA>
constexpr size_t cl_fwd_lds_bytes() {
    return sizeof(float) * (ClTab<C, MODE, NA, 0, false>::total + (NBLK > 1 ? ClTab<C, MODE, NA, 1, false>::total : 0) +
                            (MODE == MODE_EDGE ? kClWaves * ClMap<C>::RPW * (C * ALG::D + 4) : 0));
}

struct ClCarry { f4 a, b; };
template <class ALG, int C, int MODE, int NA>
struct ClBwdIn : ClIn<ALG, C, MODE, NA> {
    using IN = ClIn<ALG, C, MODE, NA>;
    static constexpr int ROW = C * ALG::D;
    ClBuf gy, st0, st1;
    unsigned st_lane, st_row0;
    CSMPN_DEV ClBwdIn(const RowIO& io, int c, int r) : IN(io, c) {
        const size_t rb = (size_t)this->rows * IN::RB, sb = state_rows(io.rows) * (size_t)IN::RB;
        gy = ClBuf(io.gy, MODE == MODE_EDGE ? (size_t)io.gather_rows * IN::RB : rb);
        st0 = ClBuf(io.saved + state_region<ROW, ROW>(io.rows, 0, 0), io.save_state ? sb : 0);
        st1 = ClBuf(io.saved + state_region<ROW, ROW>(io.rows, 0, 1), io.save_state ? sb : 0);
        st_lane = cl_state_lane<C>(r, c);
        st_row0 = cl_state_lane<C>(0, c);
    }
    CSMPN_DEV unsigned gy_off(const ClTile<C, MODE>& T) const {
        if constexpr (MODE == MODE_EDGE) return T.valid ? (unsigned)T.i_dst * IN::RB + this->lo : kClNoStore;
        else return this->row_off(T.row);
    }
    template <int K>
    CSMPN_DEV const ClBuf& state() const { if constexpr (K == 0) return st0; else return st1; }
    CSMPN_DEV unsigned state_off(const ClTile<C, MODE>& T) const {
        return T.valid ? (T.row / ClMap<C>::RPW) * kClStateTile + st_lane : st_row0;
    }
};
template <class ALG, int C, int MODE, int NBLK, int NA, bool SAVES>
struct ClBwdReq {
    f4 g0, g1, s0, s1, t0, t1;
    ClRaw<ALG, C, MODE, NA> raw;
    template <int K>
    CSMPN_DEV void request(const RowIO& io, const ClBwdIn<ALG, C, MODE, NA>& in, const ClTile<C, MODE>& Tl) {
        if constexpr (K == NBLK - 1) {
            const unsigned o = in.gy_off(Tl);
            g0 = in.gy.ld4(o); g1 = in.gy.ld4(o + 16);
        }
        if constexpr (K == 0) {
            raw.issue(in, Tl);
        } else {
            const ClBuf saved(io.saved, (size_t)in.rows * ClBwdIn<ALG, C, MODE, NA>::RB);
            const unsigned o = in.row_off(Tl.lrow);
            s0 = saved.ld4(o); s1 = saved.ld4(o + 16);
        }
        if constexpr (SAVES) {
            const unsigned o = in.state_off(Tl);
            t0 = in.template state<K>().template ld4<kClStream>(o);
            t1 = in.template state<K>().template ld4<kClStream>(o + kClStatePiece);
        }
    }
    CSMPN_DEV void arrived0() {
        raw.pin();
        if constexpr (SAVES) asm volatile("" : "+v"(t0), "+v"(t1));
    }
};
template <class ALG, int C, int MODE, int NBLK, int NA, int K, bool SAVES, bool SINGLE>
CSMPN_DEV ClCarry cl_bwd_block(const RowIO& io, const ClBwdIn<ALG, C, MODE, NA>& in, float* tab, float* work, const ClTile<C, MODE>& T0,
                               ClBwdReq<ALG, C, MODE, NBLK, NA, SAVES>& cur,
                               ClBwdReq<ALG, C, MODE, NBLK, NA, SAVES>& next, const ClCarry carry_in, ClStamp& stamp) {
    constexpr bool single = SINGLE, have_pre = SINGLE || K == NBLK - 1;
    f4 carry_a = carry_in.a, carry_b = carry_in.b;
    using MP = ClMap<C>;
    using TB = ClTab<C, MODE, NA, K, true>;
    using PT = ClPart<ALG, C, TB::I>;
    using RM = ClRed<ALG>;
    constexpr int D = ALG::D, G = ALG::G, ROW = C * D, RPW = MP::RPW, SS = ROW + 4, NP = TB::NP;
    static_assert(K >= 0 && K < NBLK && NBLK <= 2, "block index");
    constexpr bool kLast = K == NBLK - 1;
    constexpr int img_max = NBLK > 1 && ClPart<ALG, C, C>::total > ClPart<ALG, C, ClTab<C, MODE, NA, 0, true>::I>::total
                                ? ClPart<ALG, C, C>::total : ClPart<ALG, C, ClTab<C, MODE, NA, 0, true>::I>::total;
// ... 160 lines not shown
            if (io.gx[1]) {
                float gx[D];
#pragma unroll
                for (int d = 0; d < D; ++d) gx[d] = 0.f;
                cl_mix<C, C, TB::W1T(1)>(gx, gy, ldsw);
#pragma unroll
                for (int d = 0; d < D; ++d) gx[d] *= Tc.scale();
                b_gx1.st8(o_row, gx);
            }
            if constexpr (NA > 0) {
                if (io.gx[2]) {
                    float gx[D];
#pragma unroll
                    for (int d = 0; d < D; ++d) gx[d] = 0.f;
                    cl_mix<C, C, TB::W1T(2)>(gx, gy, ldsw);
                    b_gx2.st8(in.in_attr ? Tc.row * IN::AB + in.lo : kClNoStore, gx);
                }
            }
        }
        stamp(16);
        if constexpr (single) break;
    }
    if constexpr (K > 0 && single) next.template request<K - 1>(io, in, T0);

    {
        float* img = sc;
        const int j = lane & 15, q = lane >> 4;
        constexpr int NM = NP + 2;
        f4 lo[NM], hi[NM];
        auto pair_tile = [&](const f4 (&acc)[G], int m) {
            if constexpr (C == 8) {
#pragma unroll
                for (int g = 0; g < G; ++g) {
                    lo[m][g] = acc[g][0] + dpp_mov<0xB1>(acc[g][1]);
                    hi[m][g] = acc[g][2] + dpp_mov<0xB1>(acc[g][3]);
                }
            }
        };
        auto put_tile = [&](const f4 (&acc)[G], int m, int base, int I, int coff, int width) {
            if constexpr (C == 8) {
                const int cc = j >> 1;
                if ((j & 1) == 0 && cc < width) {
                    float* p0 = img + base + ((2 * q) * I + coff + cc) * G;
                    st4(p0, lo[m]);
                    st4(p0 + I * G, hi[m]);
                }
            } else {
                if (j < width) {
#pragma unroll
                    for (int v = 0; v < 4; ++v) {
                        float* p0 = img + base + ((4 * q + v) * I + coff + j) * G;
                        st4(p0, f4{acc[0][v], acc[1][v], acc[2][v], acc[3][v]});
                    }
                }
            }
        };
        static_for<0, NP>([&](auto p) { pair_tile(accW1[p], p); });
        pair_tile(accR, NP);
        pair_tile(accL, NP + 1);
        if constexpr (C == 8) {
#pragma unroll
            for (int m = 0; m < NM; ++m) asm volatile("" : "+v"(lo[m]), "+v"(hi[m]) : : "memory");
        }
        static_for<0, NP>([&](auto p) { put_tile(accW1[p], p, 0, TB::I, TB::coff(p), TB::width(p)); });
        put_tile(accR, NP, PT::pWR, C, 0, C);
        put_tile(accL, NP + 1, PT::pWL, C, 0, C);
        stamp(21);
        __syncthreads();
        stamp(22);
        float* part = io.rl_partials + (K == 0 ? 0 : (size_t)kClSliceCap * ClPart<ALG, C, ClTab<C, MODE, NA, 0, true>::I>::total) +
                      (size_t)blockIdx.x * PT::total;
        constexpr int KG = ClSums<RM::n>::kGroups, GS = 4 * 64 * kClWaves, HR = RPW / 2;
        static_assert(2 * C * KG <= 64 * kClWaves, "one pair of owner threads per (channel, group of four sums)");
        const int par = threadIdx.x & 1, own = threadIdx.x >> 1, oc = own % C, og = own / C;
        f4 s = f4{0.f, 0.f, 0.f, 0.f};
        if (own < C * KG) {
            const float* src = work + kClWaves * scratch + og * GS + 4 * (MP::lane_of_row(par) + oc * MP::ROTL);
            f4 v[kClWaves * HR];
#pragma unroll
            for (int w = 0; w < kClWaves; ++w) {
#pragma unroll
                for (int rh = 0; rh < HR; ++rh) v[w * HR + rh] = ld4(src + 4 * (w * 64 + MP::lane_of_row(2 * rh)));
            }
            s = v[0];
#pragma unroll
            for (int i = 1; i < kClWaves * HR; ++i) s += v[i];
#pragma unroll
            for (int i = 0; i < 4; ++i) s[i] += dpp_mov<0xB1>(s[i]);
        }
        if constexpr (K == 1 && single) next.arrived0();
        if (own < C * KG) {
#pragma unroll
            for (int i = 0; i < 2; ++i) {
                const int idx = 4 * og + 2 * par + i;
                const float val = par ? s[2 + i] : s[i];
                if (idx < RM::n) part[PT::pS + PT::off(idx) + oc * PT::stride(idx)] = val;
            }
        }
        const float* img0 = work;
        static_assert(PT::pS % 4 == 0, "matrix part of the slice");
        for (int e = 4 * threadIdx.x; e < PT::pS; e += 4 * 64 * kClWaves) {
            f4 v = ld4(img0 + e);
#pragma unroll
            for (int w = 1; w < kClWaves; ++w) v += ld4(img0 + w * scratch + e);
            st4(part + e, v);
        }
    }
    stamp(17);
    return ClCarry{carry_a, carry_b};
}
template <class ALG, int C, int MODE, int NBLK, int NA>
constexpr size_t cl_bwd_lds_bytes() {
    using TB0 = ClTab<C, MODE, NA, 0, true>;
    using TB1 = ClTab<C, MODE, NA, 1, true>;
    constexpr int tile = ClMap<C>::RPW * (C * ALG::D + 4);
    int img = ClPart<ALG, C, TB0::I>::total;
    if (NBLK > 1 && ClPart<ALG, C, C>::total > img) img = ClPart<ALG, C, C>::total;
    return sizeof(float) * (TB0::total + (NBLK > 1 ? TB1::total : 0) + kClWaves * (tile > img ? tile : img) +
                            ClSums<ClRed<ALG>::n>::floats_per_wg);
}
template <class ALG, int C, int MODE, int NBLK, int NA, bool SAVES, bool SINGLE>
CSMPN_DEV void cl_bwd_blocks(const RowIO& io, const ClBwdIn<ALG, C, MODE, NA>& in, float* smem, const ClTile<C, MODE>& T0, ClBwdReq<ALG, C, MODE, NBLK, NA, SAVES>& req,
                             ClStamp& stamp) {
    using TB0 = ClTab<C, MODE, NA, 0, true>;
    using TB1 = ClTab<C, MODE, NA, 1, true>;
    constexpr int tabs = TB0::total + (NBLK > 1 ? TB1::total : 0);
    ClCarry carry{f4{0.f, 0.f, 0.f, 0.f}, f4{0.f, 0.f, 0.f, 0.f}};
    if constexpr (NBLK > 1) {
        ClBwdReq<ALG, C, MODE, NBLK, NA, SAVES> req0;
        carry = cl_bwd_block<ALG, C, MODE, NBLK, NA, 1, SAVES, SINGLE>(io, in, smem + TB0::total, smem + tabs, T0, req, req0, carry, stamp);
        if constexpr (!SINGLE) asm volatile("s_waitcnt vmcnt(0)" ::: "memory");
        stamp(18);
        __syncthreads();
        stamp(19);
        cl_bwd_block<ALG, C, MODE, NBLK, NA, 0, SAVES, SINGLE>(io, in, smem, smem + tabs, T0, req0, req, carry, stamp);
    } else {
        cl_bwd_block<ALG, C, MODE, NBLK, NA, 0, SAVES, SINGLE>(io, in, smem, smem + tabs, T0, req, req, carry, stamp);
    }
}
template <class ALG, int C, int MODE, int NBLK, int NA, bool SAVES = false>
__global__ void __launch_bounds__(64 * kClWaves, 2) cemlp_cl_bwd_kernel(const DevCemlp C_arg, const RowIO io_arg) {
    CSMPN_KERNEL_ARGS(Cd);
    extern __shared__ __attribute__((aligned(16))) float smem[];
    ClStamp stamp(0);
    using TB0 = ClTab<C, MODE, NA, 0, true>;
    using TB1 = ClTab<C, MODE, NA, 1, true>;
    constexpr int tabs = TB0::total + (NBLK > 1 ? TB1::total : 0);
    const int lane = threadIdx.x & 63;
    const ClBwdIn<ALG, C, MODE, NA> in(io, ClMap<C>::chan(lane), ClMap<C>::row(lane));
    ClTile<C, MODE> T0;
    ClBwdReq<ALG, C, MODE, NBLK, NA, SAVES> req;
    T0.load(in, blockIdx.x * kClWaves + __builtin_amdgcn_readfirstlane(threadIdx.x >> 6), ClMap<C>::row(lane));
    req.template request<NBLK - 1>(io, in, T0);
    {
        const int wave = __builtin_amdgcn_readfirstlane(threadIdx.x >> 6);
        const int dir = cl_probe_dir<C>(ClMap<C>::chan(lane));
        ClStage<ALG, C, TB0, true> st0;
        ClStage<ALG, C, TB1, true> st1;
        st0.load(Cd.b[0], wave, lane, dir);
        if constexpr (NBLK > 1) st1.load(Cd.b[1], wave, lane, dir);
        st0.store(smem, wave, lane);
        if constexpr (NBLK > 1) st1.store(smem + TB0::total, wave, lane);
    }
    __syncthreads();
    stamp(0);
    const unsigned ntiles = (in.rows + ClMap<C>::RPW - 1) / ClMap<C>::RPW;
    if (ntiles <= gridDim.x * kClWaves) cl_bwd_blocks<ALG, C, MODE, NBLK, NA, SAVES, true>(io, in, smem, T0, req, stamp);
    else cl_bwd_blocks<ALG, C, MODE, NBLK, NA, SAVES, false>(io, in, smem, T0, req, stamp);
    stamp.flush(io.stamps, threadIdx.x & 63);
}

template <class ALG, int C, int I0, int NBLK>
CSMPN_DEV void cl_reduce_group(const DevCemlp& Cd, const float* part, int nslices, int slice_cap, int group, float (*red)[17]) {
    constexpr int G = ALG::G;
    using P0 = ClPart<ALG, C, I0>;
    using P1 = ClPart<ALG, C, C>;
    constexpr int total = P0::total + (NBLK > 1 ? P1::total : 0);
    const int j = threadIdx.x & 15, w = threadIdx.x >> 4;
    int e = group * 16 + j;
    const bool live = e < total;
    if (!live) e = 0;
    const int k = (NBLK > 1 && e >= P0::total) ? 1 : 0;
    const int len = k == 0 ? P0::total : P1::total;
    const float* p = part + (k == 0 ? 0 : (size_t)slice_cap * P0::total);
    if (k == 1) e -= P0::total;
    float s = 0.f;
    for (int s0 = w; s0 < nslices; s0 += 256) {
        float v[16];
#pragma unroll
        for (int i = 0; i < 16; ++i) {
            const int sl = s0 + 16 * i;
            v[i] = sl < nslices ? p[(size_t)sl * len + e] : 0.f;
        }
#pragma unroll
        for (int i = 0; i < 16; ++i) s += v[i];
    }
    red[w][j] = s;
    __syncthreads();
    if (w != 0 || !live) return;
#pragma unroll
    for (int i = 1; i < 16; ++i) s += red[i][j];
    const DevBlock& B = Cd.b[k];
    const int I = k == 0 ? I0 : C;
    int f = e;
    float* dst = nullptr;
    const int nW1 = C * I * G, nWC = C * C * G;
    if (f < nW1) dst = B.gW1 + f;
    else if ((f -= nW1) < nWC) dst = B.gWR + f;
    else if ((f -= nWC) < nWC) dst = B.gWL + f;
    else {
        f -= nWC;
        if (f < P0::qsa) dst = B.has_b1 ? B.gb1 + f : nullptr;
        else if (f < P0::qsb) dst = B.gsa + (f - P0::qsa);
        else if (f < P0::qw) dst = B.gsb + (f - P0::qsb);
        else if (f < P0::qan) dst = B.gw + (f - P0::qw);
        else if (f < P0::qbL) dst = B.gan + (f - P0::qan);
        else if (f < P0::qla) dst = B.gbL + (f - P0::qbL);
        else dst = B.gla + (f - P0::qla);
    }
    if (dst) *dst += s;
}
template <class ALG, int C, int I0, int NBLK>
constexpr int cl_reduce_groups() { return (ClPart<ALG, C, I0>::total + (NBLK > 1 ? ClPart<ALG, C, C>::total : 0) + 15) / 16; }
template <class ALG, int C, int I0, int NBLK>
__global__ void __launch_bounds__(256) cl_reduce_kernel(const DevCemlp Cd, const float* part, int nslices, int slice_cap) {
    __shared__ float red[16][17];
    cl_reduce_group<ALG, C, I0, NBLK>(Cd, part, nslices, slice_cap, blockIdx.x, red);
}
template <class ALG, int C, int I0A, int NBLKA, int I0B, int NBLKB>
__global__ void __launch_bounds__(256) cl_reduce2_kernel(const DevCemlp CdA, const float* partA, int nslicesA, const DevCemlp CdB,
                                                         const float* partB, int nslicesB, int slice_cap) {
    __shared__ float red[16][17];
    constexpr int groupsA = cl_reduce_groups<ALG, C, I0A, NBLKA>();
    if ((int)blockIdx.x < groupsA) cl_reduce_group<ALG, C, I0A, NBLKA>(CdA, partA, nslicesA, slice_cap, blockIdx.x, red);
    else cl_reduce_group<ALG, C, I0B, NBLKB>(CdB, partB, nslicesB, slice_cap, (int)blockIdx.x - groupsA, red);
}

}
```

### clifford-group-equivariant-simplicial-message-passing-networks_amd/csrc/dispatch.hip

```cpp
#include <atomic>
#include <cstdio>

#include "plan.hpp"

namespace csmpn {
namespace {

struct SizeKey { int n, nblk, ch, i0; bool uniform; };
SizeKey size_key(int n, const csmpn_block_params* blocks, int nblk) {
    SizeKey k{n, nblk, nblk > 0 ? blocks[0].out_features : 0, nblk > 0 ? blocks[0].in_features : 0, nblk > 0};
    for (int j = 1; j < nblk; ++j)
        if (blocks[j].out_features != k.ch || blocks[j].in_features != k.ch) k.uniform = false;
    return k;
}
LaneShape shape_of(int mode, const SizeKey& k) {
    return LaneShape{mode, k.nblk, k.ch, mode == MODE_EDGE ? k.i0 - k.ch : (mode == MODE_NODE ? k.i0 - 2 * k.ch : k.i0)};
}
constexpr int kModes[] = {MODE_EDGE, MODE_NODE, MODE_PLAIN};
bool n3_shape(const SizeKey& k) { return k.n == 3 && k.nblk <= 2 && k.uniform; }
bool d32_shape(const SizeKey& k) { return k.n == 5 && k.nblk <= 2 && k.uniform && k.ch >= 8 && k.ch <= 32; }
bool egcl_slices(const LaneUnit& u, const SizeKey& k) {
    return u.slice_floats(shape_of(MODE_EDGE, k)) || u.slice_floats(shape_of(MODE_NODE, k));
}

struct TailNeed {
    size_t table_bytes, slice_bytes, pad, align, slack;
    size_t bytes() const { return table_bytes + slice_bytes; }
    size_t asks() const { return bytes() + slack; }
};
TailNeed padded(size_t table_bytes, size_t slice_bytes, bool exact) {
    return TailNeed{table_bytes, slice_bytes, kTailPad, kTailAlign, exact ? kAdmitSlack : kBoundSlack};
}
float* carve(const Plan& plan, const TailNeed& t, float** tabs) {
    if (!t.table_bytes) return reinterpret_cast<float*>(tail_region(plan, t.slice_bytes + t.pad, t.align));
    char* const tb = tail_region(plan, t.table_bytes + t.pad, t.align);
    *tabs = reinterpret_cast<float*>(tb);
    return reinterpret_cast<float*>(tb - t.slice_bytes);
}

struct SavedNeed { bool claimed; size_t handover_ch, state_ch; };

struct StageShape {
    bool ok;
    int ch, na, i0, nblk;
    bool uniform_width;
    bool all_w1_sub;
};
StageShape stage_shape(const DevCemlp& C, const SizeKey& k, int mode, const RowIO& io) {
    StageShape S{true, k.ch, k.i0, k.i0, k.nblk, k.uniform, true};
    const int ch = S.ch;
    for (int j = 0; j < C.nblk; ++j)
        if (!C.b[j].w1_sub) S.all_w1_sub = false;
    if (mode == MODE_EDGE) {
        S.na = io.nseg > 1 ? io.seg[1].ch : 0;
        if (io.seg[0].ch != ch || S.i0 != ch + S.na) S.ok = false;
    } else if (mode == MODE_NODE) {
        S.na = io.nseg > 2 ? io.seg[2].ch : 0;
        if (io.seg[0].ch != ch || io.seg[1].ch != ch || S.i0 != 2 * ch + S.na) S.ok = false;
    }
    return S;
}

struct Launch {
    const Plan& plan;
    const AlgOps& A;
    int mode;
    bool bwd, tables_ready;
    SizeKey key;
    StageShape S;
    float* handover;
};
LaneShape lane_shape(const Launch& x) { return LaneShape{x.mode, x.S.nblk, x.S.ch, x.S.na}; }
bool egcl(const Launch& x) { return x.mode != MODE_PLAIN && x.S.ok; }
bool two_uniform_blocks(const Launch& x) { return x.S.nblk == 2 && x.S.uniform_width && x.S.all_w1_sub; }
bool fits(const Plan& plan, size_t bytes) { return plan.workspace && plan.workspace_bytes >= bytes; }
unsigned capped(long groups, long cap) { return (unsigned)(groups < cap ? groups : cap); }

enum DebugFields { kChannelsAttr, kChannelsI0, kI0 };
struct Family {
    const char* name;
    DebugFields debug_fields;
    bool (*eligible)(const Launch& x, const RowIO& io);
    unsigned (*grid)(const Launch& x, long rows);
    const LaneUnit* (*unit)(const AlgOps* A);
    TailNeed (*tail)(const LaneUnit* u, const LaneShape& s, bool bwd);
    float* RowIO::*slices;
    const char* too_small;
    bool (*reserves)(const SizeKey& k);
    SavedNeed (*saved)(const SizeKey& k);
    int handover_blocks;
    void (*kernel_label)(const Launch& x, const RowIO& io);
};

bool pq_on() { return !sw().no_pq && !sw().no_cm; }
bool pq_eligible(const Launch& x, const RowIO& io) {
    const StageShape& S = x.S;
    if (!pq_on() || x.plan.id != ALG_N3) return false;
    if (S.nblk != 2 && !(S.nblk == 1 && x.mode == MODE_PLAIN)) return false;
    if (S.ch != 32 || !S.uniform_width || !S.all_w1_sub || !S.ok) return false;
    if (x.mode == MODE_PLAIN && (io.nseg != 1 || io.emb_nperm != 0 || io.seg[0].ch != S.i0)) return false;
    if (!cemlp_pq_n3().table_floats(lane_shape(x))) return false;
    return !x.bwd || (io.saved && io.save_state);
}
unsigned pq_grid(const Launch&, long rows) {
    return capped((rows + 15) / 16, kPqGridCap);
}
TailNeed pq_tail(const LaneUnit* u, const LaneShape& s, bool) {
    const size_t tf = u->table_floats(s);
    return tf ? padded(tf * sizeof(float), u->slice_floats(s) * sizeof(float) * kPqGridCap, true) : TailNeed{};
}
SavedNeed pq_saved(const SizeKey& k) {
    if (!pq_on() || sw().no_cm_bwd || !n3_shape(k) || k.ch != 32 || !cemlp_pq_n3().table_floats(shape_of(MODE_PLAIN, k))) return {};
    return {true, 0, (size_t)3 * k.nblk * 32};
}
void pq_label(const Launch& x, const RowIO&) {
    note_kernel("csmpn::cemlp_pq_%s_kernel<%s, ...> (mode %d, %d channels, %d %s channels, %d block%s)", x.bwd ? "bwd" : "fwd", x.A.name,
                x.mode, x.S.ch, x.S.na, x.mode == MODE_PLAIN ? "input" : "attribute", x.S.nblk, x.S.nblk > 1 ? "s" : "");
}

bool pg_eligible(const Launch& x, const RowIO& io) {
    const StageShape& S = x.S;
    if (sw().no_pg || !x.A.pg || !two_uniform_blocks(x) || S.ch <= 16 || S.ch > 32 || !egcl(x)) return false;
    if (!x.A.pg->table_floats(lane_shape(x))) return false;
    return !x.bwd || (io.saved && io.save_state);
}
unsigned pg_grid(const Launch&, long rows) { return capped((rows + 15) / 16, kPgGridCap); }
TailNeed pg_tail(const LaneUnit* u, const LaneShape& s, bool) {
    return padded(u ? u->table_floats(s) * sizeof(float) : pg_tables_bytes(s.channels), pg_part_bytes(s.channels), u != nullptr);
}
bool pg_reserves(const SizeKey& k) { return d32_shape(k) && k.ch > 16; }
SavedNeed pg_saved(const SizeKey& k) { return pg_reserves(k) && k.nblk == 2 ? SavedNeed{true, (size_t)k.ch, 3 * 2 * 32} : SavedNeed{}; }
void pg_label(const Launch& x, const RowIO&) {
    note_kernel("csmpn::cemlp_pg_%s_kernel<%s, ...> (mode %d, %d channels, %d attribute channels)", x.bwd ? "bwd" : "fwd", x.A.name, x.mode,
                x.S.ch, x.S.na);
}

bool plw_eligible(const Launch& x, const RowIO& io) {
    const StageShape& S = x.S;
    if (sw().no_plw || !x.A.plw || S.nblk < 1 || S.nblk > 2) return false;
    if ((S.ch <= 8 && !(S.ch == 8 && sw().plw8)) || S.ch > 32 || !S.uniform_width || !S.all_w1_sub || !S.ok) return false;
    if (x.mode == MODE_PLAIN && (S.na < 1 || S.na > 8 || io.nseg != 1)) return false;
    if (!x.A.plw->table_floats(lane_shape(x))) return false;
    return !(x.bwd && S.nblk > 1 && !io.saved);
}
unsigned plw_grid(const Launch& x, long rows) {
    const long per_cu = 4 / ((x.S.ch + 7) / 8) > 0 ? 4 / ((x.S.ch + 7) / 8) : 1;
    return capped((rows + 3) / 4, (x.bwd ? kPlwMaxGroups : 2 * kPlwMaxGroups) * per_cu);
}
TailNeed plw_tail(const LaneUnit* u, const LaneShape& s, bool) {
    return padded(u ? u->table_floats(s) * sizeof(float) : plw_tables_bytes(s.channels), plw_part_bytes(s.channels), u != nullptr);
}
bool plw_reserves(const SizeKey& k) { return d32_shape(k); }
SavedNeed plw_saved(const SizeKey& k) {
    return d32_shape(k) && k.nblk == 2 ? SavedNeed{true, (size_t)k.ch, (size_t)3 * 2 * ((k.ch + 7) / 8 * 8)} : SavedNeed{};
}
void plw_label(const Launch& x, const RowIO&) {
    note_kernel("csmpn::cemlp_plw_%s_kernel<%s, ...> (mode %d, %d channels, %d attribute channels, %d blocks)", x.bwd ? "bwd" : "fwd",
                x.A.name, x.mode, x.S.ch, x.S.na, x.S.nblk);
}

bool pl_eligible(const Launch& x, const RowIO& io) {
    if (sw().no_pl || !x.A.pl || !two_uniform_blocks(x) || x.S.ch != 8 || !egcl(x)) return false;
    if (x.bwd && !io.saved) return false;
    return serves(*x.A.pl, lane_shape(x));
}
unsigned pl_grid(const Launch& x, long rows) {
    const long tiles = (rows + 3) / 4;
    return capped((tiles + 3) / 4, x.bwd ? kPlMaxBwdGroups : 512);
}
TailNeed pl_tail(const LaneUnit* u, const LaneShape&, bool bwd) { return bwd ? padded(0, pl_part_bytes(), u != nullptr) : TailNeed{}; }
bool pl_reserves(const SizeKey& k) { return d32_shape(k) && k.nblk == 2 && k.ch == 8; }
void pl_label(const Launch& x, const RowIO& io) {
    note_kernel("csmpn::cemlp_pl_kernel<%s, %d, %d, %d, %s, %s>", x.A.name, x.mode, x.S.nblk, x.S.i0, x.bwd ? "true" : "false",
                x.bwd && io.save_state ? "true" : "false");
}

bool cl_eligible(const Launch& x, const RowIO& io) {
    const StageShape& S = x.S;
    if (sw().no_cl || x.plan.id != ALG_N3 || !two_uniform_blocks(x) || !egcl(x)) return false;
    if (x.bwd && !io.saved) return false;
    if (!serves(cemlp_cl_n3(), lane_shape(x))) return false;
    const int row_floats = S.ch * x.A.D;
    if (!cl_array_fits(io.rows + 16, row_floats)) return false;
    return x.mode != MODE_EDGE || (io.gather_rows > 0 && cl_array_fits(io.gather_rows, row_floats));
}
unsigned cl_grid(const Launch& x, long rows) {
    const long rows_per_wave = 64 / x.S.ch;
    const long tiles = (rows + rows_per_wave - 1) / rows_per_wave;
    long cap = x.bwd ? kClMaxBwdGroups : kClMaxFwdGroups;
    const long cap_f = sw().cl_cap_fwd, cap_b = sw().cl_cap_bwd;
    if (!x.bwd && cap_f > 0 && cap_f < 4096) cap = cap_f;
    if (x.bwd && cap_b > 0 && cap_b < cap) cap = cap_b;
    return capped((tiles + 3) / 4, cap);
}
TailNeed cl_tail(const LaneUnit* u, const LaneShape& s, bool bwd) {
    return bwd ? TailNeed{0, u->slice_floats(s) * sizeof(float) * kClMaxBwdGroups, 0, 16, 0} : TailNeed{};
}
SavedNeed cl_saved(const SizeKey& k) {
    return n3_shape(k) && k.nblk == 2 && egcl_slices(cemlp_cl_n3(), k) ? SavedNeed{true, (size_t)k.ch, (size_t)2 * k.ch} : SavedNeed{};
}
void cl_label(const Launch& x, const RowIO& io) {
    note_kernel("csmpn::cemlp_cl_%s_kernel<%s, %d, %d, %d, %d%s>", x.bwd ? "bwd" : "fwd", x.A.name, x.S.ch, x.mode, x.S.nblk, x.S.na,
                !x.bwd ? "" : (io.save_state ? ", true" : ", false"));
}

SavedNeed cm_saved(const SizeKey& k) {
    if (sw().no_cm_bwd || !n3_shape(k) || k.nblk != 2 || !egcl_slices(cemlp_cm_n3(), k)) return {};
    return {true, (size_t)k.ch, k.ch == 32 ? (size_t)3 * 2 * 32 : 0};
}
bool cm_eligible(const Launch& x, const RowIO& io) {
    if (sw().no_cm || x.plan.id != ALG_N3 || !two_uniform_blocks(x) || !egcl(x)) return false;
    if (x.bwd && !io.saved) return false;
    if (!serves(cemlp_cm_n3(), lane_shape(x))) return false;
    return !x.bwd || cm_saved(x.key).claimed;
}
unsigned cm_grid(const Launch& x, long rows) {
    const long tiles = (rows + 15) / 16;
    const long cap = x.bwd ? kCmMaxBwdGroups : (x.S.ch == 16 ? kCmMaxFwdGroups : 256);
    const long per_group = !x.bwd ? 4 : (x.S.ch == 32 ? 2 : 4);
    return capped((tiles + per_group - 1) / per_group, cap);
}
void cm_label(const Launch& x, const RowIO& io) {
    note_kernel("csmpn::cemlp_%s_kernel<%s, %d, %d, %d, %d%s>", !x.bwd ? "cm_fwd" : (x.S.ch == 32 ? "cmp" : "cmb"), x.A.name, x.S.ch, x.mode,
                x.S.nblk, x.S.na, x.bwd && x.S.ch == 32 ? (io.save_state && x.S.nblk > 1 ? ", true" : ", false") : "");
}

const Family kFamilies[] = {
    {"pq", kChannelsAttr, pq_eligible, pq_grid, [](const AlgOps*) { return &cemlp_pq_n3(); }, pq_tail, &RowIO::slices, nullptr, n3_shape,
     pq_saved, 1, pq_label},
    {"pg", kChannelsAttr, pg_eligible, pg_grid, [](const AlgOps* A) { return A ? A->pg : nullptr; }, pg_tail, &RowIO::slices, nullptr,
     pg_reserves, pg_saved, 1, pg_label},
    {"plw", kChannelsAttr, plw_eligible, plw_grid, [](const AlgOps* A) { return A ? A->plw : nullptr; }, plw_tail, &RowIO::slices, nullptr,
     plw_reserves, plw_saved, 2, plw_label},
    {"pl", kI0, pl_eligible, pl_grid, [](const AlgOps* A) { return A ? A->pl : nullptr; }, pl_tail, &RowIO::slices,
     "workspace too small for the parity-lane backward", pl_reserves, nullptr, 0, pl_label},
    {"cl", kChannelsI0, cl_eligible, cl_grid, [](const AlgOps*) { return &cemlp_cl_n3(); }, cl_tail, &RowIO::rl_partials, nullptr, n3_shape,
     cl_saved, 1, cl_label},
    {"cm", kChannelsI0, cm_eligible, cm_grid, [](const AlgOps*) { return &cemlp_cm_n3(); }, cl_tail, &RowIO::rl_partials, nullptr, n3_shape,
     cm_saved, 1, cm_label},
};

SavedNeed family_saved(const SizeKey& k) {
    for (const Family& F : kFamilies) {
        const SavedNeed s = F.saved ? F.saved(k) : SavedNeed{};
        if (s.claimed) return s;
    }
    return {};
}
}

size_t family_tail_bytes(int n, const csmpn_block_params* blocks, int nblk) {
    const SizeKey k = size_key(n, blocks, nblk);
    size_t best = 0;
    for (const Family& F : kFamilies)
        for (int mode : kModes) {
            const size_t b = F.reserves(k) ? F.tail(F.unit(nullptr), shape_of(mode, k), true).asks() : 0;
            best = b > best ? b : best;
        }
    return best;
}

bool pq_plain_shape(int n, const csmpn_block_params* blocks, int nblk) { return nblk >= 1 && pq_saved(size_key(n, blocks, nblk)).claimed; }

bool general_phased_shape(int n, const csmpn_block_params* blocks, int nblk) {
    if (n > 3 || nblk < 2 || nblk > CSMPN_MAX_BLOCKS) return false;
    for (int k = 0; k < nblk; ++k)
        if (blocks[k].out_features > 64) return false;
    return !family_saved(size_key(n, blocks, nblk)).handover_ch;
}

SavedLayout saved_layout(int n, const csmpn_block_params* blocks, int nblk, int64_t rows, uint32_t flags) {
    SavedLayout L{};
    for (int k = 0; k + 1 < nblk; ++k) L.inputs_ch += (size_t)blocks[k].out_features;
    const SavedNeed s = family_saved(size_key(n, blocks, nblk));
    if (s.handover_ch) L.handover_ch = s.handover_ch;
    else if (general_phased_shape(n, blocks, nblk) && (rows < 0 || rows >= sw().phased_min_rows || s.claimed)) L.handover_ch = L.inputs_ch;
    if (rows < 0 || (flags & CSMPN_FLAG_SAVE_STATE)) L.state_ch = s.state_ch;
    if (rows < 0) {
        L.total = (L.inputs_ch + L.handover_ch + L.state_ch) << n;
        return L;
    }
    const size_t state_rows = (size_t)((rows + 15) & ~(int64_t)15);
    L.handover_off = (L.inputs_ch * (size_t)rows) << n;
    L.state_off = ((L.inputs_ch + L.handover_ch) * (size_t)rows) << n;
    L.total = L.state_off + ((L.state_ch * state_rows) << n);
    return L;
}

namespace {
void debug_line(const Family& F, const Launch& x, unsigned grid, long rows) {
    char shape[64];
    if (F.debug_fields == kI0) snprintf(shape, sizeof(shape), "i0=%d", x.S.i0);
    else snprintf(shape, sizeof(shape), "channels=%d %s=%d", x.S.ch, F.debug_fields == kChannelsAttr ? "attr" : "i0",
                  F.debug_fields == kChannelsAttr ? x.S.na : x.S.i0);
    fprintf(stderr, "[csmpn] %s mode=%d bwd=%d %s grid=%u rows=%ld\n", F.name, x.mode, (int)x.bwd, shape, grid, rows);
}

Launch make_launch(const Plan& plan, int mode, bool bwd, bool tables_ready, const RowIO& io, float* handover) {
    const AlgOps& A = alg_ops(plan.id);
    const SizeKey k = size_key(A.n, plan.blocks, plan.C.nblk);
    return Launch{plan, A, mode, bwd, tables_ready, k, stage_shape(plan.C, k, mode, io), handover};
}
}

bool plw_serves(const Plan& plan, int mode, bool bwd, const RowIO& io) {
    const Launch x = make_launch(plan, mode, bwd, false, io, nullptr);
    return plw_eligible(x, io) && fits(plan, plw_tail(x.A.plw, lane_shape(x), bwd).asks());
}

int run_rows(const Plan& plan, int mode, bool bwd, const RowIO& io_in, hipStream_t st, bool need_pack, bool tables_ready,
             SliceSet* deferred) {
    if (deferred) deferred->unit = nullptr;
    if (io_in.rows <= 0) return CSMPN_OK;
    const AlgOps& A = alg_ops(plan.id);
    RowIO io = io_in;
    io.stamps = g_stamps;
    const SavedLayout SL = saved_layout(A.n, plan.blocks, plan.C.nblk, io.rows, io.save_state ? CSMPN_FLAG_SAVE_STATE : 0);
    if (!SL.state_ch) io.save_state = 0;
    float* const handover = io.saved ? const_cast<float*>(io.saved) + SL.handover_off : nullptr;
    const Launch x = make_launch(plan, mode, bwd, tables_ready, io, handover);
    for (const Family& F : kFamilies) {
        if (!F.eligible(x, io)) continue;
        const LaneUnit* const unit = F.unit(&A);
        const TailNeed t = F.tail(unit, lane_shape(x), bwd);
        if (t.bytes() && !fits(plan, t.asks())) {
            if (!F.too_small) continue;
            return fail(CSMPN_ERR_INVALID, "%s", F.too_small);
        }
        const unsigned grid = F.grid(x, io.rows);
        float* tabs = nullptr;
        if (t.bytes()) io.*F.slices = carve(plan, t, &tabs);
        if (bwd && F.handover_blocks && x.S.nblk >= F.handover_blocks) io.handover = handover;
        if (sw().debug) debug_line(F, x, grid, io.rows);
        bool handled = false;
        io.defer_sum = (bwd && deferred && unit->sum_slices && io.rl_partials) ? 1 : 0;
        HIP_TRY(unit->launch(lane_shape(x), bwd, !(bwd && tables_ready), grid, st, plan.C, io, tabs, &handled));
        if (handled) {
            if (io.defer_sum) *deferred = SliceSet{unit, lane_shape(x), plan.C, io.rl_partials, grid};
            F.kernel_label(x, io);
            return CSMPN_OK;
        }
    }
    if (A.D == 32 && bwd && mode != MODE_PLAIN && io.rows >= 4096 && !sw().quiet) {
        static std::atomic<bool> warned{false};
        if (!warned.exchange(true))
            fprintf(stderr, "[csmpn] note: Cl(5,0) / Cl(4,1) layer with %d channels runs on the general row-tile kernels (slow path: "
                            "their backward spills registers). The parity-lane kernels serve two-block EGCL layers of 8, 16, 24, 28 "
                            "or 32 channels. (CSMPN_QUIET=1 silences this note.)\n", plan.C.b[0].O);
    }
    if (io.row_store && !plan.det_general)
        return fail(CSMPN_ERR_UNSUPPORTED,
                    "CSMPN_FLAG_DETERMINISTIC: this shape is served neither by the lane kernels (Cl(3,0) 8 / 16 channels, "
                    "Cl(5,0) / Cl(4,1) 8 / 16 / 24 / 28 / 32 channels; two blocks with saved block inputs) nor by the deterministic "
                    "form of the general kernels (n <= 3, tiles and gradient mirror resident in LDS)");
    DetSlices det{nullptr, 0, kDetGroups};
    if (bwd && (io.row_store || (!sw().no_sliced && (plan.id == ALG_N2 || plan.id == ALG_N3) && !plan.ps && plan.var != VAR_GLOBAL && !plan.wide))) {
        const int rc = det_slices(plan, io.row_store != 0, det);
        if (rc) return rc;
    }
    if (bwd && plan.C.phased) io.handover = handover;
    if (need_pack) {
        const int rcp = run_pack(plan, st);
        if (rcp) return rcp;
    }
    const long R = 16 * plan.H;
    const long ntiles = (io.rows + R - 1) / R;
    DevCemlp Cd = plan.C;
    unsigned threads = plan.threads;
    size_t lds_bytes = plan.lds_bytes;
    if (plan.var != VAR_GLOBAL && Cd.RT > 1 && !bwd) {
        long rt = (ntiles + 255) / 256;
        if (rt < 1) rt = 1;
        if (rt < Cd.RT) {
            lds_bytes -= (size_t)(Cd.RT - rt) * Cd.tile_floats * 4;
            Cd.RT = (int)rt;
            threads = (unsigned)(Cd.RT * Cd.MT * 64);
        }
    }
    long grid = (ntiles + Cd.RT - 1) / Cd.RT;
    if (grid > (long)plan.grid_cap) grid = plan.grid_cap;
    if (det.base && grid > det.groups) grid = det.groups;
    if (sw().debug && plan.wide)
        fprintf(stderr, "[csmpn] wide mode=%d bwd=%d CT=%d MT=%d threads=%u lds=%zu grid=%ld tile_floats=%d rows=%ld\n", mode, (int)bwd,
                Cd.CT, Cd.MT, threads, lds_bytes, grid, Cd.tile_floats, io.rows);
    else if (sw().debug)
        fprintf(stderr, "[csmpn] mode=%d bwd=%d var=%d ps=%d share=%d phased=%d H=%d MT=%d RT=%d threads=%u lds=%zu grid=%ld tile_floats=%d mirror=%d rows=%ld\n",
                mode, (int)bwd, plan.var, (int)plan.ps, Cd.share_inz, (int)(bwd && Cd.phased), plan.H, Cd.MT, Cd.RT, threads, lds_bytes, grid,
                Cd.tile_floats, Cd.mirror_floats, io.rows);
    if (det.base) {
        const int rc = det_launch_begin(plan, det, grid, Cd, st);
        if (rc) return rc;
    }
    const char* const dir = bwd ? "true" : "false";
    if (plan.wide) {
        HIP_TRY(A.launch_cemlp_wide(mode, bwd, (unsigned)grid, threads, lds_bytes, st, Cd, io));
        note_kernel("csmpn::cemlp_wide_kernel<%s, %d, %s> (%d channel tiles on %d waves, tiles in %s)", A.name, mode, dir, Cd.CT, Cd.MT,
                    Cd.gtiles ? "global scratch" : "LDS");
    } else if (plan.ps) {
        HIP_TRY(A.launch_cemlp_ps(mode, bwd, (unsigned)grid, threads, lds_bytes, st, Cd, io));
        note_kernel("csmpn::cemlp_ps_kernel<%s, %d, %s>", A.name, mode, dir);
    } else {
        HIP_TRY(A.launch_cemlp(mode, plan.var, plan.H, bwd, (unsigned)grid, threads, lds_bytes, st, Cd, io));
        note_kernel("csmpn::cemlp_kernel<%s, %d, %d, %d, %s>", A.name, mode, plan.var, plan.H, dir);
    }
    return det.base ? det_reduce(plan, det, grid, st) : CSMPN_OK;
}

}
```

### clifford-group-equivariant-simplicial-message-passing-networks_amd/csrc/launch.hpp

```cpp
#pragma once
#include <hip/hip_runtime.h>

#include "cemlp_device.hpp"

namespace csmpn {
constexpr int kMaxLdsBytes = 160 * 1024;

#define CSMPN_DECLARE_ALG(tag)                                                                                  \
    bool has_h2_##tag();                                                                                        \
    bool has_ps_##tag();                                                                                        \
    hipError_t launch_cemlp_ps_##tag(int mode, bool bwd, unsigned grid, unsigned block, size_t lds,            \
                                     hipStream_t st, const DevCemlp& C, const RowIO& io);                      \
    hipError_t launch_cemlp_##tag(int mode, int var, int h, bool bwd, unsigned grid, unsigned block, size_t lds,   \
                                  hipStream_t st, const DevCemlp& C, const RowIO& io);                          \
    hipError_t launch_cemlp_wide_##tag(int mode, bool bwd, unsigned grid, unsigned block, size_t lds, hipStream_t st, \
                                       const DevCemlp& C, const RowIO& io);                                    \
    hipError_t launch_gp_##tag(bool bwd, const float* a, const float* b, const float* gout, float* out,        \
                               float* ga, float* gb, long rows, hipStream_t st);

CSMPN_DECLARE_ALG(n2)
CSMPN_DECLARE_ALG(n3)
CSMPN_DECLARE_ALG(n4)
CSMPN_DECLARE_ALG(n5)
CSMPN_DECLARE_ALG(n5m)
CSMPN_DECLARE_ALG(n4m)

struct LaneShape { int mode, nblk, channels, attr; };
struct LaneUnit;
struct SliceSet {
    const LaneUnit* unit;
    LaneShape shape;
    DevCemlp C;
    const float* part;
    unsigned nslices;
};
struct LaneUnit {
    size_t (*table_floats)(const LaneShape&);
    size_t (*slice_floats)(const LaneShape&);
    hipError_t (*launch)(const LaneShape&, bool bwd, bool pack, unsigned grid, hipStream_t st, const DevCemlp& C, const RowIO& io,
                         float* tabs, bool* handled);
    hipError_t (*sum_slices)(const SliceSet& a, const SliceSet* b, hipStream_t st);
};
inline bool serves(const LaneUnit& u, const LaneShape& s) { return u.table_floats(s) != 0 || u.slice_floats(s) != 0; }
#define CSMPN_DECLARE_LANE_UNIT(family, tag) const LaneUnit& cemlp_##family##_##tag();

constexpr int kClMaxFwdGroups = 1024;
constexpr int kClMaxBwdGroups = 512;
constexpr unsigned long long kClMaxArrayBytes = 0xFF000000ull;
constexpr bool cl_array_fits(long rows, int row_floats) {
    return rows >= 0 && (unsigned long long)rows * (unsigned long long)row_floats * 4ull <= kClMaxArrayBytes;
}
static_assert(cl_array_fits(16711680, 64) && !cl_array_fits(16711681, 64), "8 channels of Cl(3,0): 256-byte rows, 16 711 680 of them");
static_assert(cl_array_fits(0, 64) && !cl_array_fits(-1, 64) && !cl_array_fits(1L << 40, 64), "no wrap in the check itself");
CSMPN_DECLARE_LANE_UNIT(cl, n3)

constexpr int kCmMaxFwdGroups = 768;
constexpr int kCmMaxBwdGroups = 256;
CSMPN_DECLARE_LANE_UNIT(cm, n3)

constexpr int kPlMaxBwdGroups = 256;
CSMPN_DECLARE_LANE_UNIT(pl, n5)
CSMPN_DECLARE_LANE_UNIT(pl, n5m)

constexpr int kPlwMaxGroups = 256;
CSMPN_DECLARE_LANE_UNIT(plw, n5)
CSMPN_DECLARE_LANE_UNIT(plw, n5m)

constexpr int kPgGridCap = 256;
CSMPN_DECLARE_LANE_UNIT(pg, n5)
CSMPN_DECLARE_LANE_UNIT(pg, n5m)

constexpr unsigned kPqGridCap = 768;
CSMPN_DECLARE_LANE_UNIT(pq, n3)

constexpr size_t pl_part_bytes() { return (size_t)(8 * 768 + 2 * 640) * sizeof(float) * 4 * kPlMaxBwdGroups + 256; }
constexpr size_t plw_part_bytes(int ch) {
    const size_t NG = (ch + 7) / 8, nch0 = 2 * NG + 1;
    const size_t image = 8 * NG * (3 + 3 * 6 + 64) + 16;
    const size_t per_cu = 4 / NG > 0 ? 4 / NG : 1;
    const size_t bytes = ((nch0 + 2 * NG) * 12 * 64 * NG + image) * sizeof(float) * kPlwMaxGroups * per_cu + 256;
    return ch == 8 && pl_part_bytes() > bytes ? pl_part_bytes() : bytes;
}
constexpr size_t plw_tables_bytes(int ch) {
    const size_t NG = (ch + 7) / 8, nch0 = 2 * NG + 1;
    return ((2 * NG * nch0 + 4 * NG * NG) + (2 * NG * NG + 4 * NG * NG)) * 384 * sizeof(float);
}
constexpr size_t pg_part_bytes(int ch) { return plw_part_bytes(ch); }
constexpr size_t pg_tables_bytes(int ch) { return plw_tables_bytes(ch) + 65536; }
constexpr size_t pg_tables_overshoot(int ch) { return ch == 24 ? 100352 : 0; }
}
```

### clifford-group-equivariant-simplicial-message-passing-networks_amd/csrc/plan.hpp

```cpp
#pragma once
#include <hip/hip_runtime.h>

#include <cstddef>

#include "../../include/csmpn_hip.h"
#include "capi_common.hpp"
#include "cemlp_kernel.hpp"
#include "launch.hpp"

#define fail csmpn_fail

#define HIP_TRY(expr)                                                                         \
    do {                                                                                      \
        hipError_t e_ = (expr);                                                               \
        if (e_ != hipSuccess) return fail(CSMPN_ERR_HIP, "%s: %s", #expr, hipGetErrorString(e_)); \
    } while (0)

namespace csmpn {

inline int cdiv(int a, int b) { return (a + b - 1) / b; }
inline int rup(int a, int b) { return cdiv(a, b) * b; }

struct Switches {
    bool no_cl;
    bool no_cm;
    bool no_cm_bwd;
    bool no_pl;
    bool no_plw;
    bool plw8;
    bool no_pg;
    bool no_pq;
    bool no_share;
    bool no_phased;
    bool no_sliced;
    bool debug;
    bool quiet;
    int force_ps;
    int force_h;
    int min_lds_tiles;
    long phased_min_rows;
    long cl_cap_fwd, cl_cap_bwd;
};
const Switches& sw();
void note_kernel(const char* fmt, ...);
extern unsigned long long* g_stamps;

enum AlgId { ALG_NONE = -1, ALG_N2, ALG_N3, ALG_N4, ALG_N5, ALG_N5M, ALG_N4M, ALG_COUNT };
AlgId alg_id(const float* metric, int n);

struct AlgOps {
    int n, D, paths;
    bool h2, ps;
    const char* name;
    hipError_t (*launch_cemlp)(int mode, int var, int h, bool bwd, unsigned grid, unsigned block, size_t lds, hipStream_t st,
                               const DevCemlp& C, const RowIO& io);
    hipError_t (*launch_cemlp_ps)(int mode, bool bwd, unsigned grid, unsigned block, size_t lds, hipStream_t st, const DevCemlp& C,
                                  const RowIO& io);
    hipError_t (*launch_cemlp_wide)(int mode, bool bwd, unsigned grid, unsigned block, size_t lds, hipStream_t st, const DevCemlp& C,
                                    const RowIO& io);
    hipError_t (*launch_gp)(bool bwd, const float* a, const float* b, const float* gout, float* out, float* ga, float* gb, long rows,
                            hipStream_t st);
    const LaneUnit *pl, *plw, *pg;
};
const AlgOps& alg_ops(AlgId id);

struct Plan {
    AlgId id;
    const csmpn_block_params* blocks;
    DevCemlp C;
    PackDesc P;
    size_t pack_f4;
    unsigned threads;
    size_t lds_bytes;
    unsigned grid_cap;
    int var;
    int H;
    bool ps;
    bool det_general;
    bool wide;
    void* workspace;
    size_t workspace_bytes;
};
int make_plan(AlgId id, const csmpn_block_params* blocks, const csmpn_block_grads* grads, int nblk, void* workspace,
              size_t workspace_bytes, bool bwd, int stage_rowlen, bool use_saved, long rows, Plan& plan, bool deterministic = false);
int run_pack(const Plan& plan, hipStream_t st);
size_t plan_front_bytes(int n, const csmpn_block_params* blocks, int nblk);

inline char* tail_region(const Plan& plan, size_t bytes, size_t align) {
    return static_cast<char*>(plan.workspace) + ((plan.workspace_bytes - bytes) & ~(align - 1));
}
constexpr size_t kTailPad = 16, kTailAlign = 256;
constexpr size_t kTailSlack = kTailPad + kTailAlign;
constexpr size_t kAdmitSlack = 1024;
constexpr size_t kBoundSlack = kTailAlign;

template <class Block, class F>
inline void for_each_grad_tensor(Block& B, int G, int P, F&& f) {
    f(B.gW1, (B.w1_sub ? G : 1) * B.O * B.I, true); f(B.gWR, G * B.O * B.O, true); f(B.gWL, G * B.O * B.O, true);
    f(B.gb1, B.O, B.has_b1 != 0); f(B.gsa, B.O * G, true); f(B.gsb, B.O * G, true); f(B.gw, B.O * P, true);
    f(B.gan, B.O * G, true); f(B.gbL, B.O, true); f(B.gla, B.O, true);
}
int mirror_total(int G, int P, const csmpn_block_params* blocks, int nblk);

constexpr int kDetGroups = 512;
struct DetSlices {
    float* base;
    int floats;
    int groups;
};
size_t det_slice_bytes(int n, const csmpn_block_params* blocks, int nblk);
int det_slices(const Plan& plan, bool required, DetSlices& S);
int det_launch_begin(const Plan& plan, const DetSlices& S, long grid, DevCemlp& Cd, hipStream_t st);
int det_reduce(const Plan& plan, const DetSlices& S, long grid, hipStream_t st);

struct SavedLayout {
    size_t inputs_ch, handover_ch, state_ch;
    size_t handover_off, state_off, total;
};
SavedLayout saved_layout(int n, const csmpn_block_params* blocks, int nblk, int64_t rows, uint32_t flags);
bool pq_plain_shape(int n, const csmpn_block_params* blocks, int nblk);
bool general_phased_shape(int n, const csmpn_block_params* blocks, int nblk);
size_t family_tail_bytes(int n, const csmpn_block_params* blocks, int nblk);

int run_rows(const Plan& plan, int mode, bool bwd, const RowIO& io_in, hipStream_t st, bool need_pack, bool tables_ready = false,
             SliceSet* deferred = nullptr);
bool plw_serves(const Plan& plan, int mode, bool bwd, const RowIO& io);

}
```

### include/csmpn_hip.h

```cpp
#ifndef CSMPN_HIP_H
#define CSMPN_HIP_H

#include <stddef.h>
#include <stdint.h>

#ifdef __cplusplus
extern "C" {
#endif

#define CSMPN_MAX_BLOCKS 4
#define CSMPN_OK 0
#define CSMPN_ERR_UNSUPPORTED 1
#define CSMPN_ERR_INVALID 2
#define CSMPN_ERR_HIP 3

#define CSMPN_FLAG_NO_VALIDATE 2u
#define CSMPN_FLAG_WEIGHTS_PACKED 1u

#define CSMPN_FLAG_DETERMINISTIC 4u
#define CSMPN_FLAG_SAVE_STATE 8u

typedef struct csmpn_block_params {
    int32_t in_features;
    int32_t out_features;
    int32_t lin_subspaces;
    int32_t reserved;
    const float* lin_w;
    const float* lin_b;
    const float* silu_a;
    const float* silu_b;
    const float* gp_w;
    const float* norm_a;
    const float* right_w;
    const float* left_w;
    const float* left_b;
    const float* ln_a;
} csmpn_block_params;

typedef struct csmpn_block_grads {
    float* lin_w;
    float* lin_b;
    float* silu_a;
    float* silu_b;
    float* gp_w;
    float* norm_a;
    float* right_w;
    float* left_w;
    float* left_b;
    float* ln_a;
} csmpn_block_grads;

int csmpn_metric_supported(const float* metric_host, int n);

int csmpn_algebra_tables(const float* metric_host, int n, float* cayley, int64_t* index_to_bitmap,
                         int64_t* bitmap_to_index, int64_t* grades, int64_t* subspaces, uint8_t* paths);

int csmpn_geometric_product_forward(const float* metric_host, int n, const float* a, const float* b,
                                    float* out, int64_t rows, void* stream);
int csmpn_geometric_product_backward(const float* metric_host, int n, const float* a, const float* b,
                                     const float* gout, float* ga, float* gb, int64_t rows, void* stream);

size_t csmpn_cemlp_workspace_bytes(int n, const csmpn_block_params* blocks, int n_blocks);

size_t csmpn_cemlp_saved_floats_per_row(int n, const csmpn_block_params* blocks, int n_blocks);
size_t csmpn_cemlp_saved_floats(int n, const csmpn_block_params* blocks, int n_blocks, int64_t rows, uint32_t flags);

int csmpn_cemlp_forward(const float* metric_host, int n, const csmpn_block_params* blocks, int n_blocks,
                        const float* x, int64_t rows, float* y, float* save_inputs, void* workspace, size_t workspace_bytes,
                        uint32_t flags, void* stream);

int csmpn_cemlp_backward(const float* metric_host, int n, const csmpn_block_params* blocks,
                         const csmpn_block_grads* grads, int n_blocks, const float* x, const float* gy,
                         int64_t rows, float* gx, const float* saved_inputs, void* workspace, size_t workspace_bytes, uint32_t flags, void* stream);

int csmpn_mvlinear_forward(int n, const float* x, const float* weight, const float* bias, int64_t rows,
                           int32_t in_features, int32_t out_features, int32_t subspaces, float* y, void* stream);
int csmpn_mvlinear_backward(int n, const float* x, const float* weight, const float* gy, int64_t rows,
                            int32_t in_features, int32_t out_features, int32_t subspaces, float* gx, float* g_weight,
                            float* g_bias, void* stream);
size_t csmpn_mvlinear_backward_det_bytes(int n, int64_t rows, int32_t in_features, int32_t out_features, int32_t subspaces);
int csmpn_mvlinear_backward_det(int n, const float* x, const float* weight, const float* gy, int64_t rows,
                                int32_t in_features, int32_t out_features, int32_t subspaces, float* gx, float* g_weight,
                                float* g_bias, void* workspace, size_t workspace_bytes, void* stream);

int csmpn_mvsilu_forward(const float* metric_host, int n, const float* x, const float* a, const float* b, int64_t rows,
                         int32_t channels, float* y, void* stream);
int csmpn_mvsilu_backward(const float* metric_host, int n, const float* x, const float* a, const float* b, const float* gy,
                          int64_t rows, int32_t channels, float* gx, float* g_a, float* g_b, void* stream);
int csmpn_mvnorm_forward(const float* metric_host, int n, const float* x, const float* a, int64_t rows, int32_t channels,
                         float* y, void* stream);
int csmpn_mvnorm_backward(const float* metric_host, int n, const float* x, const float* a, const float* gy, int64_t rows,
                          int32_t channels, float* gx, float* g_a, void* stream);
int csmpn_mvlayernorm_forward(const float* metric_host, int n, const float* x, const float* a, int64_t rows,
                              int32_t channels, float* y, void* stream);
int csmpn_mvlayernorm_backward(const float* metric_host, int n, const float* x, const float* a, const float* gy,
                               int64_t rows, int32_t channels, float* gx, float* g_a, void* stream);
int csmpn_wgp_forward(const float* metric_host, int n, const float* z, const float* r, const float* weight, int64_t rows,
                      int32_t channels, float* y, void* stream);
int csmpn_wgp_backward(const float* metric_host, int n, const float* z, const float* r, const float* weight,
                       const float* gy, int64_t rows, int32_t channels, float* gz, float* gr, float* g_weight, void* stream);

#define CSMPN_LAYER_MVSILU 0
#define CSMPN_LAYER_MVNORM 1
#define CSMPN_LAYER_MVLAYERNORM 2
#define CSMPN_LAYER_WGP 3
size_t csmpn_small_layer_det_bytes(int op, int n, int64_t rows, int32_t channels);
int csmpn_mvsilu_backward_det(const float* metric_host, int n, const float* x, const float* a, const float* b, const float* gy,
                              int64_t rows, int32_t channels, float* gx, float* g_a, float* g_b, void* workspace,
                              size_t workspace_bytes, void* stream);
int csmpn_mvnorm_backward_det(const float* metric_host, int n, const float* x, const float* a, const float* gy, int64_t rows,
                              int32_t channels, float* gx, float* g_a, void* workspace, size_t workspace_bytes, void* stream);
int csmpn_mvlayernorm_forward_det(const float* metric_host, int n, const float* x, const float* a, int64_t rows,
                                  int32_t channels, float* y, void* stream);
int csmpn_mvlayernorm_backward_det(const float* metric_host, int n, const float* x, const float* a, const float* gy,
                                   int64_t rows, int32_t channels, float* gx, float* g_a, void* workspace, size_t workspace_bytes,
                                   void* stream);
int csmpn_wgp_backward_det(const float* metric_host, int n, const float* z, const float* r, const float* weight, const float* gy,
                           int64_t rows, int32_t channels, float* gz, float* gr, float* g_weight, void* workspace,
                           size_t workspace_bytes, void* stream);

size_t csmpn_csr_workspace_bytes(int64_t n_edges, int64_t n_nodes);
int csmpn_csr_build(const int64_t* edge_index, int64_t n_edges, int64_t n_nodes, int32_t* perm,
                    int32_t* src_sorted, int32_t* dst_sorted, int32_t* in_degree, int32_t* row_ptr,
                    void* workspace, size_t workspace_bytes, uint32_t flags, void* stream);

int csmpn_csr_source_order(const int32_t* src_sorted, int64_t n_edges, int64_t n_nodes, int32_t* order,
                           int32_t* row_ptr_src, void* workspace, size_t workspace_bytes, void* stream);

int csmpn_segment_reduce(const float* rows, int64_t row_floats, int64_t n_nodes, const int32_t* add_ptr,
                         const int32_t* add_order, const int32_t* sub_ptr, const int32_t* sub_order, float* out,
                         int32_t accumulate, void* stream);

int csmpn_egcl_edge_forward(const float* metric_host, int n, const csmpn_block_params* blocks, int n_blocks,
                            const float* h, int32_t channels, const float* edge_attr, int32_t attr_channels,
                            const int32_t* perm, const int32_t* src_sorted, const int32_t* dst_sorted,
                            int64_t n_edges, int64_t n_nodes, float* agg, float* save_inputs, void* workspace,
                            size_t workspace_bytes, uint32_t flags, void* stream);

int csmpn_egcl_edge_backward(const float* metric_host, int n, const csmpn_block_params* blocks,
                             const csmpn_block_grads* grads, int n_blocks, const float* h, int32_t channels,
                             const float* edge_attr, int32_t attr_channels, const int32_t* perm,
                             const int32_t* src_sorted, const int32_t* dst_sorted, int64_t n_edges,
                             int64_t n_nodes, const float* g_agg, float* gh, float* g_edge_attr,
                             const float* saved_inputs, void* workspace, size_t workspace_bytes, uint32_t flags, void* stream);

int csmpn_egcl_node_forward(const float* metric_host, int n, const csmpn_block_params* blocks, int n_blocks,
                            const float* h, int32_t channels, const float* agg, int32_t agg_channels,
                            const float* node_attr, int32_t attr_channels, const int32_t* in_degree,
                            int32_t mean_aggr, int32_t residual, int64_t n_nodes, float* out,
                            float* save_inputs, void* workspace, size_t workspace_bytes, uint32_t flags, void* stream);

int csmpn_egcl_node_backward(const float* metric_host, int n, const csmpn_block_params* blocks,
                             const csmpn_block_grads* grads, int n_blocks, const float* h, int32_t channels,
                             const float* agg, int32_t agg_channels, const float* node_attr,
                             int32_t attr_channels, const int32_t* in_degree, int32_t mean_aggr,
                             int32_t residual, int64_t n_nodes, const float* g_out, float* gh, float* g_agg,
                             float* g_node_attr, const float* saved_inputs, void* workspace, size_t workspace_bytes, uint32_t flags, void* stream);

int csmpn_egcl_backward(const float* metric_host, int n, const csmpn_block_params* edge_blocks,
                        const csmpn_block_grads* edge_grads, int n_edge_blocks, const csmpn_block_params* node_blocks,
                        const csmpn_block_grads* node_grads, int n_node_blocks, const float* h, int32_t channels,
                        const float* agg, int32_t agg_channels, const float* edge_attr, int32_t edge_attr_channels,
                        const float* node_attr, int32_t node_attr_channels, const int32_t* perm, const int32_t* src_sorted,
                        const int32_t* dst_sorted, const int32_t* in_degree, int32_t mean_aggr, int32_t residual,
                        int64_t n_edges, int64_t n_nodes, const float* g_out, float* gh, float* g_agg, float* g_edge_attr,
                        float* g_node_attr, float* g_edge_rows, const float* edge_saved_inputs, void* edge_workspace,
                        size_t edge_workspace_bytes, uint32_t edge_flags, const float* node_saved_inputs, void* node_workspace,
                        size_t node_workspace_bytes, uint32_t node_flags, void* stream);

typedef struct csmpn_vertex_block {
    const float* data;
    int32_t channels;
    int32_t grade;
} csmpn_vertex_block;
int csmpn_simplex_rows(int n, const csmpn_vertex_block* blocks, int n_blocks, const int64_t* verts, int64_t n_rows,
                       int32_t verts_per_row, int64_t n_feature_rows, float* out, void* stream);

size_t csmpn_simplex_tables_workspace_bytes(int64_t n_rows, int32_t max_dim);
int csmpn_simplex_tables(const int64_t* x_ind, int32_t x_ind_cols, const int64_t* node_types, const int64_t* x_ind_batch,
                         const int64_t* x_ind_ptr, int64_t n_rows, int64_t n_graphs, int32_t max_dim,
                         const int64_t* n_expected, int64_t* const* rows, int64_t* const* verts, int32_t* const* verts_i32,
                         int64_t* graph_of_vertex, int64_t* vertices_per_graph, int32_t* types_i32, uint32_t* status,
                         void* workspace, size_t workspace_bytes, void* stream);

size_t csmpn_rips_lift_workspace_bytes(int64_t n_graphs, int32_t verts_per_graph, int32_t max_dim);
int csmpn_rips_lift(const float* points, int32_t point_dim, int64_t n_graphs, int32_t verts_per_graph, double dis, int32_t max_dim,
                    const int64_t* capacity_rows, int64_t capacity_edges, int64_t* x_ind, int32_t x_ind_cols, int64_t* node_types,
                    int64_t* batch, int64_t* x_ind_batch, int64_t* ptr, int64_t* x_ind_ptr, int64_t* edge_index, int64_t* edge_types,
                    int64_t* counts, uint32_t* status, void* workspace, size_t workspace_bytes, void* stream);

size_t csmpn_knn_lift_workspace_bytes(int64_t n_graphs, int32_t verts_per_graph, int32_t max_dim);
int csmpn_knn_lift(const float* points, int32_t point_dim, int64_t n_graphs, int32_t verts_per_graph, int32_t k, int32_t max_dim,
                   const int64_t* capacity_rows, int64_t capacity_edges, int64_t* x_ind, int32_t x_ind_cols, int64_t* node_types,
                   int64_t* batch, int64_t* x_ind_batch, int64_t* ptr, int64_t* x_ind_ptr, int64_t* edge_index, int64_t* edge_types,
                   int64_t* counts, uint32_t* status, void* workspace, size_t workspace_bytes, void* stream);

int csmpn_embed_cemlp_forward(const float* metric_host, int n, const csmpn_block_params* blocks, int n_blocks,
                              const float* vertex_feat, int64_t n_vertex_rows, int32_t channels_per_vertex, const int32_t* verts,
                              int32_t verts_per_row, int32_t n_orders, int64_t n_rows, float* out, float* save_inputs,
                              void* workspace, size_t workspace_bytes, uint32_t flags, void* stream);
int csmpn_embed_cemlp_backward(const float* metric_host, int n, const csmpn_block_params* blocks, const csmpn_block_grads* grads,
                               int n_blocks, const float* vertex_feat, int64_t n_vertex_rows, int32_t channels_per_vertex,
                               const int32_t* verts, int32_t verts_per_row, int32_t n_orders, int64_t n_rows, const float* g_out,
                               const float* saved_inputs, void* workspace, size_t workspace_bytes, uint32_t flags, void* stream);

int csmpn_readout_traj_forward(int n, const float* x, int32_t channels, const int32_t* vertex_rows, int64_t n_vertices,
                               const float* weight, int32_t out_channels, int32_t weight_stride, const float* loc, const float* target,
                               const int32_t* target_row, const int32_t* vertex_ptr, int64_t n_graphs, float* pred, float* per_graph,
                               float* per_vertex, void* stream);
int csmpn_readout_traj_backward(int n, const float* x, int32_t channels, int64_t n_rows, const int32_t* vertex_rows,
                                const int32_t* vertex_of_row, int64_t n_vertices, const float* weight, int32_t out_channels,
                                int32_t weight_stride, const float* pred, const float* target, const int32_t* target_row,
                                const int32_t* graph_of_vertex, const int32_t* vertex_ptr, const float* g_per_graph,
                                const float* g_per_vertex, float* gpred_scratch, float* gx, float* g_weight, void* stream);

int csmpn_type_attr_forward(int n, const float* table, int32_t n_types, int32_t k, const int32_t* types, int64_t n_nodes,
                            const int32_t* src, const int32_t* dst, int64_t n_edges, float* node_attr, float* edge_attr, void* stream);
int csmpn_type_attr_backward(int n, int32_t n_types, int32_t k, const int32_t* types, int64_t n_nodes, const int32_t* src,
                             const int32_t* dst, int64_t n_edges, const float* g_node_attr, const float* g_edge_attr, float* g_table,
                             void* stream);
size_t csmpn_type_attr_backward_det_bytes(int32_t n_types, int32_t k, int64_t n_nodes, int64_t n_edges);
int csmpn_type_attr_backward_det(int n, int32_t n_types, int32_t k, const int32_t* types, int64_t n_nodes, const int32_t* src,
                                 const int32_t* dst, int64_t n_edges, const float* g_node_attr, const float* g_edge_attr,
                                 float* g_table, void* workspace, size_t workspace_bytes, void* stream);

int csmpn_readout_mse_forward(int n, const float* x, const float* weight, int32_t weight_stride, const float* bias,
                              int64_t n_rows, int32_t channels, const int32_t* graph_ptr, int64_t n_graphs,
                              const float* target, float* pred, float* loss, float* channel_sums, void* stream);
int csmpn_readout_mse_backward(int n, const float* weight, int32_t weight_stride, int64_t n_rows, int32_t channels,
                               const int32_t* graph_ptr, int64_t n_graphs, const float* coef, float* gx, void* stream);

const char* csmpn_last_error(void);

const char* csmpn_last_kernel(void);

int csmpn_abi_version(void);
const char* csmpn_build_target(void);

#ifdef __cplusplus
}
#endif
#endif
```

Measured before the change: 645.5 million edges/s.

## Precompute per-layer weight images once and fuse zero-fill into one prepare kernel

Adds a combined EGCL forward entry point that first runs a prepare kernel. The kernel builds packed weight/table "images" for the edge and node forward and backward programs in one launch and also zero-fills the aggregation and gradient buffers. The row kernels then load these prebuilt images instead of repacking weights in each launch, and the backward reuses the images saved from the forward. This removes repeated per-kernel weight packing and a separate memset launch. In exchange it adds an extra buffer, a new code path restricted to the S1 shape (Cl(3,0)-sized, 8 channels, 2 blocks), and more API surface.

```diff
diff --git a/clifford-group-equivariant-simplicial-message-passing-networks_amd/csmpn_hip/native.py b/clifford-group-equivariant-simplicial-message-passing-networks_amd/csmpn_hip/native.py
--- a/clifford-group-equivariant-simplicial-message-passing-networks_amd/csmpn_hip/native.py
+++ b/clifford-group-equivariant-simplicial-message-passing-networks_amd/csmpn_hip/native.py
@@ -52,6 +52,9 @@
     "csmpn_egcl_node_forward",
     "csmpn_egcl_node_backward",
     "csmpn_egcl_backward",
+    "csmpn_egcl_image_floats",
+    "csmpn_egcl_forward",
+    "csmpn_egcl_backward_images",
     "csmpn_simplex_rows",
     "csmpn_simplex_tables_workspace_bytes",
     "csmpn_simplex_tables",
@@ -162,6 +165,13 @@
     sig("csmpn_egcl_backward", C.c_int,
         [fp, C.c_int, bp, bg, C.c_int, bp, bg, C.c_int, vp, i32, vp, i32, vp, i32, vp, i32, vp, vp, vp, vp, i32, i32, i64, i64,
          vp, vp, vp, vp, vp, vp, vp, vp, sz, u32, vp, vp, sz, u32, vp])
+    sig("csmpn_egcl_image_floats", sz, [C.c_int, bp, C.c_int, bp, C.c_int, C.POINTER(sz)])
+    sig("csmpn_egcl_forward", C.c_int,
+        [fp, C.c_int, bp, C.c_int, bp, C.c_int, vp, i32, vp, i32, vp, i32, vp, vp, vp, vp, i32, i32, i64, i64, vp, i32, vp,
+         vp, vp, sz, u32, vp, vp, sz, u32, vp, sz, vp, i64, vp])
+    sig("csmpn_egcl_backward_images", C.c_int,
+        [fp, C.c_int, bp, bg, C.c_int, bp, bg, C.c_int, vp, i32, vp, i32, vp, i32, vp, i32, vp, vp, vp, vp, i32, i32, i64, i64,
+         vp, vp, vp, vp, vp, vp, vp, vp, sz, u32, vp, vp, sz, u32, vp, sz, vp])
     sig("csmpn_simplex_rows", C.c_int, [C.c_int, C.POINTER(VertexBlock), C.c_int, vp, i64, i32, i64, vp, vp])
     sig("csmpn_simplex_tables_workspace_bytes", sz, [i64, i32])
     sig("csmpn_simplex_tables", C.c_int, [vp, i32, vp, vp, vp, i64, i64, i32, vp, vp, vp, vp, vp, vp, vp, vp, vp, sz, vp])
diff --git a/clifford-group-equivariant-simplicial-message-passing-networks_amd/csmpn_hip/ops.py b/clifford-group-equivariant-simplicial-message-passing-networks_amd/csmpn_hip/ops.py
--- a/clifford-group-equivariant-simplicial-message-passing-networks_amd/csmpn_hip/ops.py
+++ b/clifford-group-equivariant-simplicial-message-passing-networks_amd/csmpn_hip/ops.py
@@ -468,6 +468,13 @@
         self.A, self.T = edge_attr_channels, node_attr_channels
         self.mean = 1 if aggr == "mean" else 0
         self.residual = 1 if residual else 0
+        self._image_floats = None
+
+    def image_floats(self) -> int:
+        if self._image_floats is None:
+            e, nd = self.edge, self.node
+            self._image_floats = int(native.lib().csmpn_egcl_image_floats(e.n, e.params, e.nblk, nd.params, nd.nblk, None))
+        return self._image_floats
 
 
 class HipBackend:
@@ -606,8 +613,35 @@
 
     @staticmethod
     @_on_device_of(2)
+    def layer_forward(spec, csr, h, edge_attr, node_attr, pe, pn, agg, zero, images):
+        e, nd = spec.edge, spec.node
+        e.bind(pe)
+        nd.bind(pn)
+        N, D, dev = h.shape[0], nd.D, h.device
+        out = torch.empty(N, nd.out_features, D, dtype=torch.float32, device=dev)
+
+        def stage(binding, rows):
+            saved = binding.new_saved(rows, dev, _SAVE_STATE)
+            flag = 0
+            if _SAVE_STATE and saved is not None:
+                flag = native.FLAG_SAVE_STATE
+                saved.csmpn_save_state = True
+            return binding.workspace(dev), saved, flag
+
+        ws_e, saved_e, fl_e = stage(e, csr.n_edges)
+        ws_n, saved_n, fl_n = stage(nd, N)
+        check(native.lib().csmpn_egcl_forward(
+            e.metric_arr, e.n, e.params, e.nblk, nd.params, nd.nblk, h.data_ptr(), spec.C, _ptr(edge_attr), spec.A,
+            _ptr(node_attr), spec.T, csr.perm.data_ptr(), csr.src.data_ptr(), csr.dst.data_ptr(), csr.deg.data_ptr(),
+            spec.mean, spec.residual, csr.n_edges, N, agg.data_ptr(), spec.O, out.data_ptr(), _ptr(saved_e), ws_e.data_ptr(),
+            ws_e.numel(), fl_e, _ptr(saved_n), ws_n.data_ptr(), ws_n.numel(), fl_n, images.data_ptr(), images.numel(),
+            zero.data_ptr(), zero.numel(), _stream(dev)))
+        return out, (ws_e, saved_e), (ws_n, saved_n)
+
+    @staticmethod
+    @_on_device_of(2)
     def layer_backward(spec, csr, h, agg, edge_attr, node_attr, pe, pn, gout, want_gea, want_gna, state_e=None, state_n=None,
-                       gflat_e=None, gflat_n=None, fused_e=None, fused_n=None):
+                       gflat_e=None, gflat_n=None, fused_e=None, fused_n=None, images=None):
         e, nd = spec.edge, spec.node
         e.bind(pe)
         nd.bind(pn)
@@ -628,12 +662,15 @@
 
         ws_e, saved_e, fl_e = stage(e, state_e)
         ws_n, saved_n, fl_n = stage(nd, state_n)
-        check(native.lib().csmpn_egcl_backward(
-            e.metric_arr, e.n, e.params, e.grads, e.nblk, nd.params, nd.grads, nd.nblk, h.data_ptr(), spec.C,
-            agg.data_ptr(), spec.O, _ptr(edge_attr), spec.A, _ptr(node_attr), spec.T, csr.perm.data_ptr(),
-            csr.src.data_ptr(), csr.dst.data_ptr(), csr.deg.data_ptr(), spec.mean, spec.residual, csr.n_edges, N,
-            gout.data_ptr(), gh.data_ptr(), g_agg.data_ptr(), _ptr(g_ea), _ptr(g_na), None, _ptr(saved_e),
-            ws_e.data_ptr(), ws_e.numel(), fl_e, _ptr(saved_n), ws_n.data_ptr(), ws_n.numel(), fl_n, _stream(dev)))
+        args = (e.metric_arr, e.n, e.params, e.grads, e.nblk, nd.params, nd.grads, nd.nblk, h.data_ptr(), spec.C,
+                agg.data_ptr(), spec.O, _ptr(edge_attr), spec.A, _ptr(node_attr), spec.T, csr.perm.data_ptr(),
+                csr.src.data_ptr(), csr.dst.data_ptr(), csr.deg.data_ptr(), spec.mean, spec.residual, csr.n_edges, N,
+                gout.data_ptr(), gh.data_ptr(), g_agg.data_ptr(), _ptr(g_ea), _ptr(g_na), None, _ptr(saved_e),
+                ws_e.data_ptr(), ws_e.numel(), fl_e, _ptr(saved_n), ws_n.data_ptr(), ws_n.numel(), fl_n)
+        if images is not None:
+            check(native.lib().csmpn_egcl_backward_images(*args, images.data_ptr(), images.numel(), _stream(dev)))
+        else:
+            check(native.lib().csmpn_egcl_backward(*args, _stream(dev)))
         return gh, g_ea, g_na, views_e, views_n
 
 
@@ -671,11 +708,21 @@
         ctx.param_refs = params
         fuse = _fusable(params, h.device)
         n_ge, n_gn = (spec.edge.grad_floats(pe), spec.node.grad_floats(pn)) if (any(ctx.needs_input_grad) and not fuse) else (0, 0)
-        zeros = torch.zeros(n_agg + n_ge + n_gn, dtype=torch.float32, device=h.device)
+        n_zero = n_agg + n_ge + n_gn
+        n_img = spec.image_floats() if (isinstance(csr, Csr) and n_zero % 4 == 0 and any(ctx.needs_input_grad)
+                                        and not deterministic_request()) else 0
+        if n_img:
+            flat = torch.empty(n_zero + n_img, dtype=torch.float32, device=h.device)
+            zeros, ctx.images = flat[:n_zero], flat[n_zero:]
+        else:
+            zeros, ctx.images = torch.zeros(n_zero, dtype=torch.float32, device=h.device), None
         agg = zeros[:n_agg].view(h.shape[0], spec.O, spec.edge.D)
         ctx.gflats = (zeros[n_agg:n_agg + n_ge], zeros[n_agg + n_ge:]) if n_ge else None
-        agg, st_e = HipBackend.edge_forward(spec, csr, h, edge_attr, pe, agg=agg)
-        out, st_n = HipBackend.node_forward(spec, csr.deg, h, agg, node_attr, pn)
+        if n_img:
+            out, st_e, st_n = HipBackend.layer_forward(spec, csr, h, edge_attr, node_attr, pe, pn, agg, zeros, ctx.images)
+        else:
+            agg, st_e = HipBackend.edge_forward(spec, csr, h, edge_attr, pe, agg=agg)
+            out, st_n = HipBackend.node_forward(spec, csr.deg, h, agg, node_attr, pn)
         ctx.spec, ctx.csr, ctx.st_e, ctx.st_n = spec, csr, st_e, st_n
         ctx.has_ea, ctx.has_na = edge_attr is not None, node_attr is not None
         ctx.mask = [p is not None for p in params]
@@ -710,7 +757,7 @@
         if isinstance(csr, Csr) and not deterministic_request():
             gh, g_ea, g_na, views_e, views_n = HipBackend.layer_backward(
                 spec, csr, h, agg, edge_attr, node_attr, pe, pn, gout, ctx.needs_input_grad[1], ctx.needs_input_grad[2],
-                ctx.st_e, ctx.st_n, gfe, gfn, refs[:ne] if fuse else None, refs[ne:] if fuse else None)
+                ctx.st_e, ctx.st_n, gfe, gfn, refs[:ne] if fuse else None, refs[ne:] if fuse else None, images=ctx.images)
             return (gh, g_ea, g_na, None, None, *views_e, *views_n)
         gh, g_agg, g_na, views_n = HipBackend.node_backward(spec, csr.deg, h, agg, node_attr, pn, gout,
                                                             ctx.needs_input_grad[2], ctx.st_n, gfn,
diff --git a/clifford-group-equivariant-simplicial-message-passing-networks_amd/csrc/capi.hip b/clifford-group-equivariant-simplicial-message-passing-networks_amd/csrc/capi.hip
--- a/clifford-group-equivariant-simplicial-message-passing-networks_amd/csrc/capi.hip
+++ b/clifford-group-equivariant-simplicial-message-passing-networks_amd/csrc/capi.hip
@@ -278,10 +278,10 @@
     return CSMPN_OK;
 }
 
-int csmpn_egcl_edge_forward(const float* metric, int n, const csmpn_block_params* blocks, int n_blocks, const float* h,
-                            int32_t channels, const float* edge_attr, int32_t attr_channels, const int32_t* perm,
-                            const int32_t* src_sorted, const int32_t* dst_sorted, int64_t E, int64_t N, float* agg,
-                            float* save_inputs, void* workspace, size_t workspace_bytes, uint32_t flags, void* stream) {
+static int edge_forward(const float* metric, int n, const csmpn_block_params* blocks, int n_blocks, const float* h,
+                        int32_t channels, const float* edge_attr, int32_t attr_channels, const int32_t* perm,
+                        const int32_t* src_sorted, const int32_t* dst_sorted, int64_t E, int64_t N, float* agg,
+                        float* save_inputs, void* workspace, size_t workspace_bytes, uint32_t flags, void* stream, const float* tab) {
     const AlgId id = alg_id(metric, n);
     if (id == ALG_NONE) return fail(CSMPN_ERR_UNSUPPORTED, "metric not supported by the HIP path");
     RowIO io;
@@ -293,7 +293,15 @@
     const bool need_pack = !(flags & CSMPN_FLAG_WEIGHTS_PACKED);
     io.agg = agg; io.save = save_inputs;
     io.gather_rows = N;
-    return run_rows(plan, MODE_EDGE, false, io, (hipStream_t)stream, need_pack);
+    return run_rows(plan, MODE_EDGE, false, io, (hipStream_t)stream, need_pack, false, nullptr, tab);
+}
+
+int csmpn_egcl_edge_forward(const float* metric, int n, const csmpn_block_params* blocks, int n_blocks, const float* h,
+                            int32_t channels, const float* edge_attr, int32_t attr_channels, const int32_t* perm,
+                            const int32_t* src_sorted, const int32_t* dst_sorted, int64_t E, int64_t N, float* agg,
+                            float* save_inputs, void* workspace, size_t workspace_bytes, uint32_t flags, void* stream) {
+    return edge_forward(metric, n, blocks, n_blocks, h, channels, edge_attr, attr_channels, perm, src_sorted, dst_sorted, E, N, agg,
+                        save_inputs, workspace, workspace_bytes, flags, stream, nullptr);
 }
 
 static int edge_backward(const float* metric, int n, const csmpn_block_params* blocks,
@@ -301,7 +309,7 @@
                          const float* edge_attr, int32_t attr_channels, const int32_t* perm,
                          const int32_t* src_sorted, const int32_t* dst_sorted, int64_t E, int64_t N,
                          const float* g_agg, float* gh, float* g_edge_attr, const float* saved_inputs, void* workspace,
-                         size_t workspace_bytes, uint32_t flags, void* stream, SliceSet* deferred) {
+                         size_t workspace_bytes, uint32_t flags, void* stream, SliceSet* deferred, const float* tab = nullptr) {
     const AlgId id = alg_id(metric, n);
     if (id == ALG_NONE) return fail(CSMPN_ERR_UNSUPPORTED, "metric not supported by the HIP path");
     RowIO io;
@@ -313,7 +321,7 @@
     const bool need_pack = true;
     io.gy = g_agg; io.gx[0] = gh; io.gx[1] = g_edge_attr; io.saved = saved_inputs;
     io.gather_rows = N;
-    return run_rows(plan, MODE_EDGE, true, io, (hipStream_t)stream, need_pack, (flags & CSMPN_FLAG_WEIGHTS_PACKED) != 0, deferred);
+    return run_rows(plan, MODE_EDGE, true, io, (hipStream_t)stream, need_pack, (flags & CSMPN_FLAG_WEIGHTS_PACKED) != 0, deferred, tab);
 }
 
 int csmpn_egcl_edge_backward(const float* metric, int n, const csmpn_block_params* blocks,
@@ -345,10 +353,11 @@
     return CSMPN_OK;
 }
 
-int csmpn_egcl_node_forward(const float* metric, int n, const csmpn_block_params* blocks, int n_blocks, const float* h,
-                            int32_t channels, const float* agg, int32_t agg_channels, const float* node_attr,
-                            int32_t attr_channels, const int32_t* in_degree, int32_t mean_aggr, int32_t residual,
-                            int64_t N, float* out, float* save_inputs, void* workspace, size_t workspace_bytes, uint32_t flags, void* stream) {
+static int node_forward(const float* metric, int n, const csmpn_block_params* blocks, int n_blocks, const float* h,
+                        int32_t channels, const float* agg, int32_t agg_channels, const float* node_attr,
+                        int32_t attr_channels, const int32_t* in_degree, int32_t mean_aggr, int32_t residual,
+                        int64_t N, float* out, float* save_inputs, void* workspace, size_t workspace_bytes, uint32_t flags, void* stream,
+                        const float* tab) {
     const AlgId id = alg_id(metric, n);
     if (id == ALG_NONE) return fail(CSMPN_ERR_UNSUPPORTED, "metric not supported by the HIP path");
     RowIO io;
@@ -362,7 +371,15 @@
     io.y = out; io.resid = residual ? h : nullptr; io.save = save_inputs;
     io.row_store = (flags & CSMPN_FLAG_DETERMINISTIC) ? 1 : 0;
     io.save_state = (flags & CSMPN_FLAG_SAVE_STATE) ? 1 : 0;
-    return run_rows(plan, MODE_NODE, false, io, (hipStream_t)stream, need_pack);
+    return run_rows(plan, MODE_NODE, false, io, (hipStream_t)stream, need_pack, false, nullptr, tab);
+}
+
+int csmpn_egcl_node_forward(const float* metric, int n, const csmpn_block_params* blocks, int n_blocks, const float* h,
+                            int32_t channels, const float* agg, int32_t agg_channels, const float* node_attr,
+                            int32_t attr_channels, const int32_t* in_degree, int32_t mean_aggr, int32_t residual,
+                            int64_t N, float* out, float* save_inputs, void* workspace, size_t workspace_bytes, uint32_t flags, void* stream) {
+    return node_forward(metric, n, blocks, n_blocks, h, channels, agg, agg_channels, node_attr, attr_channels, in_degree, mean_aggr,
+                        residual, N, out, save_inputs, workspace, workspace_bytes, flags, stream, nullptr);
 }
 
 static int node_backward(const float* metric, int n, const csmpn_block_params* blocks,
@@ -370,7 +387,7 @@
                          const float* agg, int32_t agg_channels, const float* node_attr, int32_t attr_channels,
                          const int32_t* in_degree, int32_t mean_aggr, int32_t residual, int64_t N,
                          const float* g_out, float* gh, float* g_agg, float* g_node_attr, const float* saved_inputs, void* workspace,
-                         size_t workspace_bytes, uint32_t flags, void* stream, SliceSet* deferred) {
+                         size_t workspace_bytes, uint32_t flags, void* stream, SliceSet* deferred, const float* tab = nullptr) {
     const AlgId id = alg_id(metric, n);
     if (id == ALG_NONE) return fail(CSMPN_ERR_UNSUPPORTED, "metric not supported by the HIP path");
     RowIO io;
@@ -385,7 +402,7 @@
     io.resid_bwd = residual ? 1 : 0; io.saved = saved_inputs;
     io.row_store = (flags & CSMPN_FLAG_DETERMINISTIC) ? 1 : 0;
     io.save_state = (flags & CSMPN_FLAG_SAVE_STATE) ? 1 : 0;
-    return run_rows(plan, MODE_NODE, true, io, (hipStream_t)stream, need_pack, (flags & CSMPN_FLAG_WEIGHTS_PACKED) != 0, deferred);
+    return run_rows(plan, MODE_NODE, true, io, (hipStream_t)stream, need_pack, (flags & CSMPN_FLAG_WEIGHTS_PACKED) != 0, deferred, tab);
 }
 
 int csmpn_egcl_node_backward(const float* metric, int n, const csmpn_block_params* blocks,
@@ -397,6 +414,54 @@
     return node_backward(metric, n, blocks, grads, n_blocks, h, channels, agg, agg_channels, node_attr, attr_channels, in_degree, mean_aggr,
                          residual, N, g_out, gh, g_agg, g_node_attr, saved_inputs, workspace, workspace_bytes, flags, stream, nullptr);
 }
+
+static int egcl_backward(const float* metric, int n, const csmpn_block_params* edge_blocks, const csmpn_block_grads* edge_grads,
+                        int n_edge_blocks, const csmpn_block_params* node_blocks, const csmpn_block_grads* node_grads,
+                        int n_node_blocks, const float* h, int32_t channels, const float* agg, int32_t agg_channels,
+                        const float* edge_attr, int32_t edge_attr_channels, const float* node_attr, int32_t node_attr_channels,
+                        const int32_t* perm, const int32_t* src_sorted, const int32_t* dst_sorted, const int32_t* in_degree,
+                        int32_t mean_aggr, int32_t residual, int64_t E, int64_t N, const float* g_out, float* gh, float* g_agg,
+                        float* g_edge_attr, float* g_node_attr, float* g_edge_rows, const float* edge_saved, void* edge_workspace,
+                        size_t edge_workspace_bytes, uint32_t edge_flags, const float* node_saved, void* node_workspace,
+                        size_t node_workspace_bytes, uint32_t node_flags, void* stream, const float* images, size_t image_floats) {
+    const bool det = ((edge_flags | node_flags) & CSMPN_FLAG_DETERMINISTIC) != 0;
+    size_t img[4] = {0, 0, 0, 0};
+    if (images) {
+        const size_t need = egcl_image_floats(n, edge_blocks, n_edge_blocks, node_blocks, n_node_blocks, img);
+        if (!need) return fail(CSMPN_ERR_UNSUPPORTED, "table images: this layer has none (csmpn_egcl_image_floats is 0)");
+        if (det) return fail(CSMPN_ERR_UNSUPPORTED, "table images: not with CSMPN_FLAG_DETERMINISTIC (the per-stage entry points serve it)");
+        if (image_floats < need || (reinterpret_cast<uintptr_t>(images) & 15))
+            return fail(CSMPN_ERR_INVALID, "table images: %zu floats at a 16-byte boundary needed, got %zu", need, image_floats);
+    }
+    if ((edge_flags & CSMPN_FLAG_DETERMINISTIC) && !g_edge_rows)
+        return fail(CSMPN_ERR_INVALID, "CSMPN_FLAG_DETERMINISTIC: g_edge_rows ([E, C, D], csmpn_egcl_edge_backward's gh) is null");
+    const char *we = static_cast<const char*>(edge_workspace), *wn = static_cast<const char*>(node_workspace);
+    const bool apart = we && wn && (we + edge_workspace_bytes <= wn || wn + node_workspace_bytes <= we);
+    SliceSet node_set, edge_set;
+    node_set.unit = edge_set.unit = nullptr;
+    const bool defer = !det && apart;
+    int rc = node_backward(metric, n, node_blocks, node_grads, n_node_blocks, h, channels, agg, agg_channels, node_attr,
+                           node_attr_channels, in_degree, mean_aggr, residual, N, g_out, gh, g_agg, g_node_attr, node_saved,
+                           node_workspace, node_workspace_bytes, node_flags, stream, defer ? &node_set : nullptr,
+                           images ? images + img[3] : nullptr);
+    if (rc) return rc;
+    rc = edge_backward(metric, n, edge_blocks, edge_grads, n_edge_blocks, h, channels, edge_attr, edge_attr_channels, perm, src_sorted,
+                       dst_sorted, E, N, g_agg, (edge_flags & CSMPN_FLAG_DETERMINISTIC) ? g_edge_rows : gh, g_edge_attr, edge_saved,
+                       edge_workspace, edge_workspace_bytes, edge_flags, stream, node_set.unit ? &edge_set : nullptr,
+                       images ? images + img[1] : nullptr);
+    if (node_set.unit) {
+        const SliceSet* const other = (!rc && edge_set.unit == node_set.unit) ? &edge_set : nullptr;
+        HIP_TRY(node_set.unit->sum_slices(node_set, other, (hipStream_t)stream));
+        if (!rc && edge_set.unit && !other) HIP_TRY(edge_set.unit->sum_slices(edge_set, nullptr, (hipStream_t)stream));
+    }
+    return rc;
+}
+
+#define CSMPN_EGCL_BACKWARD_ARGS                                                                                                       \
+    metric, n, edge_blocks, edge_grads, n_edge_blocks, node_blocks, node_grads, n_node_blocks, h, channels, agg, agg_channels, edge_attr,  \
+        edge_attr_channels, node_attr, node_attr_channels, perm, src_sorted, dst_sorted, in_degree, mean_aggr, residual, E, N, g_out, gh,   \
+        g_agg, g_edge_attr, g_node_attr, g_edge_rows, edge_saved, edge_workspace, edge_workspace_bytes, edge_flags, node_saved,             \
+        node_workspace, node_workspace_bytes, node_flags, stream
 
 int csmpn_egcl_backward(const float* metric, int n, const csmpn_block_params* edge_blocks, const csmpn_block_grads* edge_grads,
                         int n_edge_blocks, const csmpn_block_params* node_blocks, const csmpn_block_grads* node_grads,
@@ -407,27 +472,66 @@
                         float* g_edge_attr, float* g_node_attr, float* g_edge_rows, const float* edge_saved, void* edge_workspace,
                         size_t edge_workspace_bytes, uint32_t edge_flags, const float* node_saved, void* node_workspace,
                         size_t node_workspace_bytes, uint32_t node_flags, void* stream) {
-    const bool det = ((edge_flags | node_flags) & CSMPN_FLAG_DETERMINISTIC) != 0;
-    if ((edge_flags & CSMPN_FLAG_DETERMINISTIC) && !g_edge_rows)
-        return fail(CSMPN_ERR_INVALID, "CSMPN_FLAG_DETERMINISTIC: g_edge_rows ([E, C, D], csmpn_egcl_edge_backward's gh) is null");
-    const char *we = static_cast<const char*>(edge_workspace), *wn = static_cast<const char*>(node_workspace);
-    const bool apart = we && wn && (we + edge_workspace_bytes <= wn || wn + node_workspace_bytes <= we);
-    SliceSet node_set, edge_set;
-    node_set.unit = edge_set.unit = nullptr;
-    const bool defer = !det && apart;
-    int rc = node_backward(metric, n, node_blocks, node_grads, n_node_blocks, h, channels, agg, agg_channels, node_attr,
-                           node_attr_channels, in_degree, mean_aggr, residual, N, g_out, gh, g_agg, g_node_attr, node_saved,
-                           node_workspace, node_workspace_bytes, node_flags, stream, defer ? &node_set : nullptr);
-    if (rc) return rc;
-    rc = edge_backward(metric, n, edge_blocks, edge_grads, n_edge_blocks, h, channels, edge_attr, edge_attr_channels, perm, src_sorted,
-                       dst_sorted, E, N, g_agg, (edge_flags & CSMPN_FLAG_DETERMINISTIC) ? g_edge_rows : gh, g_edge_attr, edge_saved,
-                       edge_workspace, edge_workspace_bytes, edge_flags, stream, node_set.unit ? &edge_set : nullptr);
-    if (node_set.unit) {
-        const SliceSet* const other = (!rc && edge_set.unit == node_set.unit) ? &edge_set : nullptr;
-        HIP_TRY(node_set.unit->sum_slices(node_set, other, (hipStream_t)stream));
-        if (!rc && edge_set.unit && !other) HIP_TRY(edge_set.unit->sum_slices(edge_set, nullptr, (hipStream_t)stream));
-    }
-    return rc;
-}
-
-}
+    return egcl_backward(CSMPN_EGCL_BACKWARD_ARGS, nullptr, 0);
+}
+
+int csmpn_egcl_backward_images(const float* metric, int n, const csmpn_block_params* edge_blocks, const csmpn_block_grads* edge_grads,
+                               int n_edge_blocks, const csmpn_block_params* node_blocks, const csmpn_block_grads* node_grads,
+                               int n_node_blocks, const float* h, int32_t channels, const float* agg, int32_t agg_channels,
+                               const float* edge_attr, int32_t edge_attr_channels, const float* node_attr, int32_t node_attr_channels,
+                               const int32_t* perm, const int32_t* src_sorted, const int32_t* dst_sorted, const int32_t* in_degree,
+                               int32_t mean_aggr, int32_t residual, int64_t E, int64_t N, const float* g_out, float* gh, float* g_agg,
+                               float* g_edge_attr, float* g_node_attr, float* g_edge_rows, const float* edge_saved, void* edge_workspace,
+                               size_t edge_workspace_bytes, uint32_t edge_flags, const float* node_saved, void* node_workspace,
+                               size_t node_workspace_bytes, uint32_t node_flags, const float* images, size_t image_floats, void* stream) {
+    if (!images) return fail(CSMPN_ERR_INVALID, "table images: images is null (csmpn_egcl_backward stages from the parameters)");
+    return egcl_backward(CSMPN_EGCL_BACKWARD_ARGS, images, image_floats);
+}
+
+size_t csmpn_egcl_image_floats(int n, const csmpn_block_params* edge_blocks, int n_edge_blocks, const csmpn_block_params* node_blocks,
+                               int n_node_blocks, size_t* offsets) {
+    if (!edge_blocks || !node_blocks || n_edge_blocks < 1 || n_edge_blocks > CSMPN_MAX_BLOCKS || n_node_blocks < 1 ||
+        n_node_blocks > CSMPN_MAX_BLOCKS)
+        return 0;
+    return egcl_image_floats(n, edge_blocks, n_edge_blocks, node_blocks, n_node_blocks, offsets);
+}
+
+int csmpn_egcl_forward(const float* metric, int n, const csmpn_block_params* edge_blocks, int n_edge_blocks,
+                       const csmpn_block_params* node_blocks, int n_node_blocks, const float* h, int32_t channels,
+                       const float* edge_attr, int32_t edge_attr_channels, const float* node_attr, int32_t node_attr_channels,
+                       const int32_t* perm, const int32_t* src_sorted, const int32_t* dst_sorted, const int32_t* in_degree,
+                       int32_t mean_aggr, int32_t residual, int64_t E, int64_t N, float* agg, int32_t agg_channels, float* out,
+                       float* edge_save, void* edge_workspace, size_t edge_workspace_bytes, uint32_t edge_flags, float* node_save,
+                       void* node_workspace, size_t node_workspace_bytes, uint32_t node_flags, float* images, size_t image_floats,
+                       float* zero, int64_t zero_floats, void* stream) {
+    const AlgId id = alg_id(metric, n);
+    if (id == ALG_NONE) return fail(CSMPN_ERR_UNSUPPORTED, "metric not supported by the HIP path");
+    if ((edge_flags | node_flags) & CSMPN_FLAG_DETERMINISTIC)
+        return fail(CSMPN_ERR_UNSUPPORTED, "csmpn_egcl_forward: not with CSMPN_FLAG_DETERMINISTIC (the per-stage entry points serve it)");
+    if (!edge_blocks || !node_blocks || n_edge_blocks < 1 || n_edge_blocks > CSMPN_MAX_BLOCKS || n_node_blocks < 1 ||
+        n_node_blocks > CSMPN_MAX_BLOCKS)
+        return fail(CSMPN_ERR_INVALID, "csmpn_egcl_forward: blocks");
+    size_t img[4];
+    const size_t need = id == ALG_N3 ? egcl_image_floats(n, edge_blocks, n_edge_blocks, node_blocks, n_node_blocks, img) : 0;
+    if (!need) return fail(CSMPN_ERR_UNSUPPORTED, "csmpn_egcl_forward: this layer has no table images (csmpn_egcl_image_floats is 0)");
+    if (!images || image_floats < need || (reinterpret_cast<uintptr_t>(images) & 15))
+        return fail(CSMPN_ERR_INVALID, "csmpn_egcl_forward: %zu image floats at a 16-byte boundary needed, got %zu", need, image_floats);
+    if (zero_floats < 0 || (zero_floats > 0 && (!zero || (reinterpret_cast<uintptr_t>(zero) & 15))))
+        return fail(CSMPN_ERR_INVALID, "csmpn_egcl_forward: the zero-fill range needs a 16-byte boundary");
+    const int64_t agg_floats = N * (int64_t)agg_channels << n;
+    if (N > 0 && (!agg || agg < zero || agg + agg_floats > zero + zero_floats))
+        return fail(CSMPN_ERR_INVALID, "csmpn_egcl_forward: agg (%lld floats) does not lie inside the zero-fill range", (long long)agg_floats);
+    Plan pe, pn;
+    int rc = make_plan(id, edge_blocks, nullptr, n_edge_blocks, edge_workspace, edge_workspace_bytes, false,
+                       edge_blocks[n_edge_blocks - 1].out_features << n, false, E, pe);
+    if (rc) return rc;
+    if ((rc = make_plan(id, node_blocks, nullptr, n_node_blocks, node_workspace, node_workspace_bytes, false, 0, false, N, pn))) return rc;
+    HIP_TRY(cl_prepare_n3(pe.C, pn.C, images, zero, (size_t)zero_floats, (hipStream_t)stream));
+    rc = edge_forward(metric, n, edge_blocks, n_edge_blocks, h, channels, edge_attr, edge_attr_channels, perm, src_sorted, dst_sorted, E,
+                      N, agg, edge_save, edge_workspace, edge_workspace_bytes, edge_flags, stream, images + img[0]);
+    if (rc) return rc;
+    return node_forward(metric, n, node_blocks, n_node_blocks, h, channels, agg, agg_channels, node_attr, node_attr_channels, in_degree,
+                        mean_aggr, residual, N, out, node_save, node_workspace, node_workspace_bytes, node_flags, stream, images + img[2]);
+}
+
+}
diff --git a/clifford-group-equivariant-simplicial-message-passing-networks_amd/csrc/cemlp_cl.hpp b/clifford-group-equivariant-simplicial-message-passing-networks_amd/csrc/cemlp_cl.hpp
--- a/clifford-group-equivariant-simplicial-message-passing-networks_amd/csrc/cemlp_cl.hpp
+++ b/clifford-group-equivariant-simplicial-message-passing-networks_amd/csrc/cemlp_cl.hpp
@@ -245,6 +245,20 @@
         if (wave == 2 && lane < C) st4(par + lane * kClParStride, f4{pb1, pbL, pla, 0.f});
     }
 };
+
+template <int FLOATS>
+CSMPN_DEV void cl_stage_image(const float* img, float* lds, int tid) {
+    static_assert(FLOATS % 4 == 0, "whole 16-byte vectors");
+    constexpr int NV = FLOATS / 4, NT = 64 * kClWaves, NIT = (NV + NT - 1) / NT;
+    const ClBuf b(img, (size_t)FLOATS * 4);
+    f4 v[NIT];
+#pragma unroll
+    for (int i = 0; i < NIT; ++i) v[i] = b.ld4(16u * (unsigned)(tid + NT * i));
+#pragma unroll
+    for (int i = 0; i < NIT; ++i) {
+        if (NT * (i + 1) <= NV || tid + NT * i < NV) st4(lds + 4 * (tid + NT * i), v[i]);
+    }
+}
 
 template <class ALG>
 CSMPN_DEV void cl_weighted_gp(float (&out)[8], const float (&z)[8], const float (&r)[8], const float* wp) {
@@ -739,7 +753,9 @@
     ClRaw<ALG, C, MODE, NA> raw;
     raw.issue(in, T);
     Tn.load(in, tile0 + tstride, r);
-    {
+    if (io.tabs) {
+        cl_stage_image<tab_floats>(io.tabs, lds, threadIdx.x);
+    } else {
         const int dir = cl_probe_dir<C>(c);
         ClStage<ALG, C, T0, false> st0;
         ClStage<ALG, C, T1, false> st1;
@@ -1206,7 +1222,9 @@
     ClBwdReq<ALG, C, MODE, NBLK, NA, SAVES> req;
     T0.load(in, blockIdx.x * kClWaves + __builtin_amdgcn_readfirstlane(threadIdx.x >> 6), ClMap<C>::row(lane));
     req.template request<NBLK - 1>(io, in, T0);
-    {
+    if (io.tabs) {
+        cl_stage_image<tabs>(io.tabs, smem, threadIdx.x);
+    } else {
         const int wave = __builtin_amdgcn_readfirstlane(threadIdx.x >> 6);
         const int dir = cl_probe_dir<C>(ClMap<C>::chan(lane));
         ClStage<ALG, C, TB0, true> st0;
@@ -1290,4 +1308,44 @@
     else cl_reduce_group<ALG, C, I0B, NBLKB>(CdB, partB, nslicesB, slice_cap, (int)blockIdx.x - groupsA, red);
 }
 
-}
+template <int C, int MODE, int NA, bool BWD>
+constexpr int cl_image_floats_of() { return ClTab<C, MODE, NA, 0, BWD>::total + ClTab<C, MODE, NA, 1, BWD>::total; }
+constexpr int kClPrepImages = 4;
+template <class ALG, int C, int MODE, int NA, bool BWD>
+CSMPN_DEV void cl_prepare_image(const DevCemlp& Cd, float* img) {
+    using T0 = ClTab<C, MODE, NA, 0, BWD>;
+    using T1 = ClTab<C, MODE, NA, 1, BWD>;
+    const int wave = __builtin_amdgcn_readfirstlane(threadIdx.x >> 6), lane = threadIdx.x & 63;
+    const int dir = cl_probe_dir<C>(ClMap<C>::chan(lane));
+    ClStage<ALG, C, T0, BWD> st0;
+    ClStage<ALG, C, T1, BWD> st1;
+    st0.load(Cd.b[0], wave, lane, dir);
+    st1.load(Cd.b[1], wave, lane, dir);
+    st0.store(img, wave, lane);
+    st1.store(img + T0::total, wave, lane);
+}
+template <class ALG, int C, int NAE, int NAT>
+__global__ void __launch_bounds__(64 * kClWaves) cl_prepare_kernel(const DevCemlp Ce_arg, const DevCemlp Cn_arg, float* images,
+                                                                    int off_edge_bwd, int off_node_fwd, int off_node_bwd, float* zero,
+                                                                    size_t n_zero) {
+    typedef const char __attribute__((address_space(4))) * KArgPtr;
+    const KArgPtr ka = (KArgPtr)__builtin_amdgcn_kernarg_segment_ptr();
+    constexpr size_t kCnOffset = (sizeof(DevCemlp) + alignof(DevCemlp) - 1) / alignof(DevCemlp) * alignof(DevCemlp);
+    const DevCemlp& Ce = *(const DevCemlp*)(const char*)ka;
+    const DevCemlp& Cn = *(const DevCemlp*)(const char*)(ka + kCnOffset);
+    (void)Ce_arg; (void)Cn_arg;
+    if (blockIdx.x < (unsigned)kClPrepImages) {
+        if (!images) return;
+        if (blockIdx.x == 0) cl_prepare_image<ALG, C, MODE_EDGE, NAE, false>(Ce, images);
+        else if (blockIdx.x == 1) cl_prepare_image<ALG, C, MODE_EDGE, NAE, true>(Ce, images + off_edge_bwd);
+        else if (blockIdx.x == 2) cl_prepare_image<ALG, C, MODE_NODE, NAT, false>(Cn, images + off_node_fwd);
+        else cl_prepare_image<ALG, C, MODE_NODE, NAT, true>(Cn, images + off_node_bwd);
+        return;
+    }
+    const size_t nv = n_zero / 4, stride = (size_t)(gridDim.x - kClPrepImages) * (64 * kClWaves);
+    for (size_t i = (size_t)(blockIdx.x - kClPrepImages) * (64 * kClWaves) + threadIdx.x; i < nv; i += stride)
+        st4(zero + 4 * i, f4{0.f, 0.f, 0.f, 0.f});
+    if (blockIdx.x == (unsigned)kClPrepImages && threadIdx.x < n_zero % 4) zero[4 * nv + threadIdx.x] = 0.f;
+}
+
+}
diff --git a/clifford-group-equivariant-simplicial-message-passing-networks_amd/csrc/dispatch.hip b/clifford-group-equivariant-simplicial-message-passing-networks_amd/csrc/dispatch.hip
--- a/clifford-group-equivariant-simplicial-message-passing-networks_amd/csrc/dispatch.hip
+++ b/clifford-group-equivariant-simplicial-message-passing-networks_amd/csrc/dispatch.hip
@@ -90,6 +90,7 @@
     SavedNeed (*saved)(const SizeKey& k);
     int handover_blocks;
     void (*kernel_label)(const Launch& x, const RowIO& io);
+    bool images;
 };
 
 bool pq_on() { return !sw().no_pq && !sw().no_cm; }
@@ -227,17 +228,17 @@
 
 const Family kFamilies[] = {
     {"pq", kChannelsAttr, pq_eligible, pq_grid, [](const AlgOps*) { return &cemlp_pq_n3(); }, pq_tail, &RowIO::slices, nullptr, n3_shape,
-     pq_saved, 1, pq_label},
+     pq_saved, 1, pq_label, false},
     {"pg", kChannelsAttr, pg_eligible, pg_grid, [](const AlgOps* A) { return A ? A->pg : nullptr; }, pg_tail, &RowIO::slices, nullptr,
-     pg_reserves, pg_saved, 1, pg_label},
+     pg_reserves, pg_saved, 1, pg_label, false},
     {"plw", kChannelsAttr, plw_eligible, plw_grid, [](const AlgOps* A) { return A ? A->plw : nullptr; }, plw_tail, &RowIO::slices, nullptr,
-     plw_reserves, plw_saved, 2, plw_label},
+     plw_reserves, plw_saved, 2, plw_label, false},
     {"pl", kI0, pl_eligible, pl_grid, [](const AlgOps* A) { return A ? A->pl : nullptr; }, pl_tail, &RowIO::slices,
-     "workspace too small for the parity-lane backward", pl_reserves, nullptr, 0, pl_label},
+     "workspace too small for the parity-lane backward", pl_reserves, nullptr, 0, pl_label, false},
     {"cl", kChannelsI0, cl_eligible, cl_grid, [](const AlgOps*) { return &cemlp_cl_n3(); }, cl_tail, &RowIO::rl_partials, nullptr, n3_shape,
-     cl_saved, 1, cl_label},
+     cl_saved, 1, cl_label, true},
     {"cm", kChannelsI0, cm_eligible, cm_grid, [](const AlgOps*) { return &cemlp_cm_n3(); }, cl_tail, &RowIO::rl_partials, nullptr, n3_shape,
-     cm_saved, 1, cm_label},
+     cm_saved, 1, cm_label, false},
 };
 
 SavedNeed family_saved(const SizeKey& k) {
@@ -258,6 +259,18 @@
             best = b > best ? b : best;
         }
     return best;
+}
+
+size_t egcl_image_floats(int n, const csmpn_block_params* edge_blocks, int n_edge, const csmpn_block_params* node_blocks, int n_node,
+                         size_t* offsets) {
+    if (sw().no_cl || n != 3) return 0;
+    const SizeKey ke = size_key(n, edge_blocks, n_edge), kn = size_key(n, node_blocks, n_node);
+    if (!n3_shape(ke) || !n3_shape(kn)) return 0;
+    const LaneShape se = shape_of(MODE_EDGE, ke), sn = shape_of(MODE_NODE, kn);
+    if (!cl_images_n3(se, sn) || !serves(cemlp_cl_n3(), se) || !serves(cemlp_cl_n3(), sn)) return 0;
+    const ClImageLayout L = cl_image_layout(se.attr, sn.attr);
+    if (offsets) { offsets[0] = L.edge_fwd; offsets[1] = L.edge_bwd; offsets[2] = L.node_fwd; offsets[3] = L.node_bwd; }
+    return L.total;
 }
 
 bool pq_plain_shape(int n, const csmpn_block_params* blocks, int nblk) { return nblk >= 1 && pq_saved(size_key(n, blocks, nblk)).claimed; }
@@ -309,7 +322,7 @@
 }
 
 int run_rows(const Plan& plan, int mode, bool bwd, const RowIO& io_in, hipStream_t st, bool need_pack, bool tables_ready,
-             SliceSet* deferred) {
+             SliceSet* deferred, const float* image) {
     if (deferred) deferred->unit = nullptr;
     if (io_in.rows <= 0) return CSMPN_OK;
     const AlgOps& A = alg_ops(plan.id);
@@ -330,6 +343,7 @@
         const unsigned grid = F.grid(x, io.rows);
         float* tabs = nullptr;
         if (t.bytes()) io.*F.slices = carve(plan, t, &tabs);
+        if (F.images) io.tabs = image;
         if (bwd && F.handover_blocks && x.S.nblk >= F.handover_blocks) io.handover = handover;
         if (sw().debug) debug_line(F, x, grid, io.rows);
         bool handled = false;
diff --git a/clifford-group-equivariant-simplicial-message-passing-networks_amd/csrc/k_cl_prep_n3.hip b/clifford-group-equivariant-simplicial-message-passing-networks_amd/csrc/k_cl_prep_n3.hip
--- /dev/null
+++ b/clifford-group-equivariant-simplicial-message-passing-networks_amd/csrc/k_cl_prep_n3.hip
@@ -0,0 +1,35 @@
+#include "cemlp_cl.hpp"
+#include "launch_unit.hpp"
+
+namespace csmpn {
+namespace {
+using ALG_T = Alg<3, 0u>;
+constexpr int kC = 8, kEdgeAttr = 6, kNodeAttr = 3;
+constexpr ClImageLayout kLayout = cl_image_layout(kEdgeAttr, kNodeAttr);
+static_assert(cl_image_floats(MODE_EDGE, kEdgeAttr, false) == (size_t)cl_image_floats_of<kC, MODE_EDGE, kEdgeAttr, false>(), "edge forward image");
+static_assert(cl_image_floats(MODE_EDGE, kEdgeAttr, true) == (size_t)cl_image_floats_of<kC, MODE_EDGE, kEdgeAttr, true>(), "edge backward image");
+static_assert(cl_image_floats(MODE_NODE, kNodeAttr, false) == (size_t)cl_image_floats_of<kC, MODE_NODE, kNodeAttr, false>(), "node forward image");
+static_assert(cl_image_floats(MODE_NODE, kNodeAttr, true) == (size_t)cl_image_floats_of<kC, MODE_NODE, kNodeAttr, true>(), "node backward image");
+static_assert(cl_image_floats(MODE_EDGE, kEdgeAttr, false) * 4 <= cl_fwd_lds_bytes<ALG_T, kC, MODE_EDGE, 2, kEdgeAttr>(), "inside the edge forward's LDS");
+static_assert(cl_image_floats(MODE_NODE, kNodeAttr, false) * 4 <= cl_fwd_lds_bytes<ALG_T, kC, MODE_NODE, 2, kNodeAttr>(), "inside the node forward's LDS");
+static_assert(cl_image_floats(MODE_EDGE, kEdgeAttr, true) * 4 <= cl_bwd_lds_bytes<ALG_T, kC, MODE_EDGE, 2, kEdgeAttr>(), "inside the edge backward's LDS");
+static_assert(cl_image_floats(MODE_NODE, kNodeAttr, true) * 4 <= cl_bwd_lds_bytes<ALG_T, kC, MODE_NODE, 2, kNodeAttr>(), "inside the node backward's LDS");
+static_assert(kLayout.edge_bwd % 4 == 0 && kLayout.node_fwd % 4 == 0 && kLayout.node_bwd % 4 == 0 && kLayout.total % kClImageAlign == 0,
+              "16-byte loads from every image");
+static_assert(kLayout.total < (1u << 30), "image offsets are ints in the kernel");
+constexpr size_t kFillGroups = 1024;
+}
+
+bool cl_images_n3(const LaneShape& edge, const LaneShape& node) {
+    return edge.mode == MODE_EDGE && edge.nblk == 2 && edge.channels == kC && edge.attr == kEdgeAttr && node.mode == MODE_NODE &&
+           node.nblk == 2 && node.channels == kC && node.attr == kNodeAttr;
+}
+
+hipError_t cl_prepare_n3(const DevCemlp& edge, const DevCemlp& node, float* images, float* zero, size_t n_zero, hipStream_t st) {
+    const size_t vecs = n_zero / 4 + (n_zero % 4 ? 1 : 0), want = (vecs + 64 * kClWaves - 1) / (64 * kClWaves);
+    const unsigned fill = (unsigned)(want < kFillGroups ? want : kFillGroups);
+    return launch_kernel<cl_prepare_kernel<ALG_T, kC, kEdgeAttr, kNodeAttr>>(kClPrepImages + fill, 64 * kClWaves, 0, st, edge, node, images,
+                                                                              (int)kLayout.edge_bwd, (int)kLayout.node_fwd,
+                                                                              (int)kLayout.node_bwd, zero, n_zero);
+}
+}
diff --git a/clifford-group-equivariant-simplicial-message-passing-networks_amd/csrc/launch.hpp b/clifford-group-equivariant-simplicial-message-passing-networks_amd/csrc/launch.hpp
--- a/clifford-group-equivariant-simplicial-message-passing-networks_amd/csrc/launch.hpp
+++ b/clifford-group-equivariant-simplicial-message-passing-networks_amd/csrc/launch.hpp
@@ -53,6 +53,28 @@
 static_assert(cl_array_fits(16711680, 64) && !cl_array_fits(16711681, 64), "8 channels of Cl(3,0): 256-byte rows, 16 711 680 of them");
 static_assert(cl_array_fits(0, 64) && !cl_array_fits(-1, 64) && !cl_array_fits(1L << 40, 64), "no wrap in the check itself");
 CSMPN_DECLARE_LANE_UNIT(cl, n3)
+constexpr size_t kClImageAlign = 64;
+constexpr size_t cl_image_floats(int mode, int attr, bool bwd) {
+    size_t rep = 1;
+    while ((int)rep < attr) rep <<= 1;
+    const size_t C = 8, mat = 4 * C * C, par = C * 36, np = (mode == MODE_EDGE ? 1 : 2) + (attr > 0 ? 1 : 0);
+    const size_t w1 = 4 * C * ((mode == MODE_EDGE ? 1 : 2) * C + (attr > 0 ? rep : 0));
+    return (w1 + 2 * mat + (bwd ? (np + 2) * mat : 0) + par) + (3 * mat + (bwd ? 3 * mat : 0) + par);
+}
+struct ClImageLayout { size_t edge_fwd, edge_bwd, node_fwd, node_bwd, total; };
+constexpr size_t cl_image_pad(size_t floats) { return (floats + kClImageAlign - 1) / kClImageAlign * kClImageAlign; }
+constexpr ClImageLayout cl_image_layout(int edge_attr, int node_attr) {
+    ClImageLayout L{0, 0, 0, 0, 0};
+    L.edge_bwd = L.edge_fwd + cl_image_pad(cl_image_floats(MODE_EDGE, edge_attr, false));
+    L.node_fwd = L.edge_bwd + cl_image_pad(cl_image_floats(MODE_EDGE, edge_attr, true));
+    L.node_bwd = L.node_fwd + cl_image_pad(cl_image_floats(MODE_NODE, node_attr, false));
+    L.total = L.node_bwd + cl_image_pad(cl_image_floats(MODE_NODE, node_attr, true));
+    return L;
+}
+static_assert(cl_image_floats(MODE_EDGE, 6, false) == 2368 && cl_image_floats(MODE_EDGE, 6, true) == 4160, "S1's edge program");
+static_assert(cl_image_floats(MODE_NODE, 3, false) == 2496 && cl_image_floats(MODE_NODE, 3, true) == 4544, "S1's node program");
+bool cl_images_n3(const LaneShape& edge, const LaneShape& node);
+hipError_t cl_prepare_n3(const DevCemlp& edge, const DevCemlp& node, float* images, float* zero, size_t n_zero, hipStream_t st);
 
 constexpr int kCmMaxFwdGroups = 768;
 constexpr int kCmMaxBwdGroups = 256;
diff --git a/clifford-group-equivariant-simplicial-message-passing-networks_amd/csrc/plan.hpp b/clifford-group-equivariant-simplicial-message-passing-networks_amd/csrc/plan.hpp
--- a/clifford-group-equivariant-simplicial-message-passing-networks_amd/csrc/plan.hpp
+++ b/clifford-group-equivariant-simplicial-message-passing-networks_amd/csrc/plan.hpp
@@ -121,9 +121,11 @@
 bool pq_plain_shape(int n, const csmpn_block_params* blocks, int nblk);
 bool general_phased_shape(int n, const csmpn_block_params* blocks, int nblk);
 size_t family_tail_bytes(int n, const csmpn_block_params* blocks, int nblk);
+size_t egcl_image_floats(int n, const csmpn_block_params* edge_blocks, int n_edge, const csmpn_block_params* node_blocks, int n_node,
+                         size_t* offsets);
 
 int run_rows(const Plan& plan, int mode, bool bwd, const RowIO& io_in, hipStream_t st, bool need_pack, bool tables_ready = false,
-             SliceSet* deferred = nullptr);
+             SliceSet* deferred = nullptr, const float* image = nullptr);
 bool plw_serves(const Plan& plan, int mode, bool bwd, const RowIO& io);
 
 }
diff --git a/include/csmpn_hip.h b/include/csmpn_hip.h
--- a/include/csmpn_hip.h
+++ b/include/csmpn_hip.h
@@ -168,6 +168,30 @@
                         size_t edge_workspace_bytes, uint32_t edge_flags, const float* node_saved_inputs, void* node_workspace,
                         size_t node_workspace_bytes, uint32_t node_flags, void* stream);
 
+size_t csmpn_egcl_image_floats(int n, const csmpn_block_params* edge_blocks, int n_edge_blocks,
+                               const csmpn_block_params* node_blocks, int n_node_blocks, size_t* offsets);
+
+int csmpn_egcl_forward(const float* metric_host, int n, const csmpn_block_params* edge_blocks, int n_edge_blocks,
+                       const csmpn_block_params* node_blocks, int n_node_blocks, const float* h, int32_t channels,
+                       const float* edge_attr, int32_t edge_attr_channels, const float* node_attr, int32_t node_attr_channels,
+                       const int32_t* perm, const int32_t* src_sorted, const int32_t* dst_sorted, const int32_t* in_degree,
+                       int32_t mean_aggr, int32_t residual, int64_t n_edges, int64_t n_nodes, float* agg, int32_t agg_channels,
+                       float* out, float* edge_save_inputs, void* edge_workspace, size_t edge_workspace_bytes, uint32_t edge_flags,
+                       float* node_save_inputs, void* node_workspace, size_t node_workspace_bytes, uint32_t node_flags,
+                       float* images, size_t image_floats, float* zero, int64_t zero_floats, void* stream);
+
+int csmpn_egcl_backward_images(const float* metric_host, int n, const csmpn_block_params* edge_blocks,
+                               const csmpn_block_grads* edge_grads, int n_edge_blocks, const csmpn_block_params* node_blocks,
+                               const csmpn_block_grads* node_grads, int n_node_blocks, const float* h, int32_t channels,
+                               const float* agg, int32_t agg_channels, const float* edge_attr, int32_t edge_attr_channels,
+                               const float* node_attr, int32_t node_attr_channels, const int32_t* perm, const int32_t* src_sorted,
+                               const int32_t* dst_sorted, const int32_t* in_degree, int32_t mean_aggr, int32_t residual,
+                               int64_t n_edges, int64_t n_nodes, const float* g_out, float* gh, float* g_agg, float* g_edge_attr,
+                               float* g_node_attr, float* g_edge_rows, const float* edge_saved_inputs, void* edge_workspace,
+                               size_t edge_workspace_bytes, uint32_t edge_flags, const float* node_saved_inputs, void* node_workspace,
+                               size_t node_workspace_bytes, uint32_t node_flags, const float* images, size_t image_floats,
+                               void* stream);
+
 typedef struct csmpn_vertex_block {
     const float* data;
     int32_t channels;
```

After: 659.4 million edges/s, median of 6. +2.1%, better.
